# jac99/Egonn

Hardware: AMD Instinct MI355X
Metric: LiDAR scans/sec (descriptor extraction), 50k-pt clouds @ 0.1m voxel (higher is better)
Workload: dtype f32

## Files before the change

### egonn_amd/_lib.py

```python
from __future__ import annotations

import ctypes as C
import os
from typing import List, Optional, Sequence

import numpy as np
import torch

_HERE = os.path.dirname(os.path.abspath(__file__))
LIB_PATH = os.path.join(_HERE, "lib", "libegonn_hip.so")

QUANT_CARTESIAN, QUANT_POLAR = 0, 1
FLAG_DISABLE_GLOBAL, FLAG_DISABLE_LOCAL, FLAG_IGNORE_KP_REGRESSOR, FLAG_BF16 = 1, 2, 4, 8
FLAG_POOL_SPOC, FLAG_POOL_MAC = 16, 32
MINKFPN_SPLIT_TOPDOWN = 1
MINKFPN_BLOCKS = {'BasicBlock': 0, 'ECABasicBlock': 1}
MINKFPN_POOLING = {None: 0, 'GeM': 1, 'MAC': 2, 'SPoC': 3}

_P = C.c_void_p
_SIGS = [
    ("egonn_ctx_create", C.c_int, [C.POINTER(_P), C.c_int, C.c_int]),
    ("egonn_ctx_destroy", None, [_P]),
    ("egonn_last_error", C.c_char_p, []),
    ("egonn_debug_set_naive_conv", C.c_int, [_P, C.c_int]),
    ("egonn_debug_set_ksplit", C.c_int, [_P, C.c_int, C.c_int, C.c_int, C.c_int, C.c_int]),
    ("egonn_debug_set_resident", C.c_int, [_P, C.c_int, C.c_int]),
    ("egonn_debug_keep_level_features", C.c_int, [_P, C.c_int]),
    ("egonn_debug_set_trace", C.c_int, [_P]),
    ("egonn_prepare_maps", C.c_int, [_P, C.c_int, _P]),
    ("egonn_debug_rowgroup_tables", C.c_int, [_P, C.c_int, C.c_int, _P, _P, C.c_int64, C.POINTER(C.c_int64), _P]),
    ("egonn_debug_rowgroup_perm", C.c_int, [_P, C.c_int, C.c_int, _P, C.c_int64, C.POINTER(C.c_int64), _P]),
    ("egonn_debug_radix_sort_scratch_bytes", C.c_int64, [C.c_int64, C.c_int]),
    ("egonn_debug_radix_sort", C.c_int, [_P, _P, _P, _P, C.c_int64, C.c_int, _P, _P, C.c_int, C.c_int, C.c_int,
                                         C.POINTER(C.c_int32), _P, C.c_int64, _P]),
    ("egonn_voxelize", C.c_int, [_P, _P, C.POINTER(C.c_int64), C.c_int, C.c_int, C.POINTER(C.c_float), _P]),
    ("egonn_ctx_reserve", C.c_int, [_P, C.c_int64, C.c_int, C.POINTER(C.c_int64)]),
    ("egonn_voxelize_device", C.c_int, [_P, _P, C.c_int64, _P, C.c_int, C.c_int, C.POINTER(C.c_float), _P]),
    ("egonn_plan_status", C.c_int, [_P, _P]),
    ("egonn_ctx_set_exact_fp32", C.c_int, [_P, C.c_int]),
    ("egonn_ctx_set_operand_autoscale", C.c_int, [_P, C.c_int]),
    ("egonn_level_capacity", C.c_int, [_P, C.c_int, C.POINTER(C.c_int64)]),
    ("egonn_graph_begin", C.c_int, [_P]),
    ("egonn_graph_end", C.c_int, [_P, C.POINTER(_P)]),
    ("egonn_graph_launch", C.c_int, [_P, _P]),
    ("egonn_graph_destroy", None, [_P]),
    ("egonn_coords_set", C.c_int, [_P, _P, C.c_int64, C.c_int, _P]),
    ("egonn_level_count", C.c_int, [_P, C.c_int, C.POINTER(C.c_int64)]),
    ("egonn_level_batch_offsets", C.c_int, [_P, C.c_int, C.POINTER(C.c_int64)]),
    ("egonn_level_coords", C.c_int, [_P, C.c_int, _P, _P]),
    ("egonn_input_index", C.c_int, [_P, _P, _P]),
    ("egonn_conv", C.c_int, [_P, C.c_int, C.c_int, C.c_int, _P, C.c_int, _P, C.c_int, _P, _P, C.c_int, _P, _P]),
    ("egonn_conv_transpose", C.c_int, [_P, C.c_int, _P, C.c_int, _P, C.c_int, _P, _P]),
    ("egonn_sparse_conv", C.c_int, [_P, C.c_int, C.c_int, _P, C.c_int, _P, C.c_int, C.c_int, _P, _P, C.c_int, _P, _P, _P]),
    ("egonn_map_groups", C.c_int, [_P, C.c_int, C.c_int, C.POINTER(C.c_int64), C.POINTER(C.c_int64), _P]),
    ("egonn_global_avg_pool", C.c_int, [_P, C.c_int, _P, C.c_int, _P, _P]),
    ("egonn_bn_fold", C.c_int, [_P, _P, _P, _P, C.c_float, C.c_int, _P, _P, _P]),
    ("egonn_block_tail", C.c_int, [_P, C.c_int, _P, _P, C.c_int, _P, C.c_int, _P, _P]),
    ("egonn_gem", C.c_int, [_P, C.c_int, _P, C.c_int, _P, _P, _P]),
    ("egonn_global_max_pool", C.c_int, [_P, C.c_int, _P, C.c_int, _P, _P]),
    ("egonn_netvlad", C.c_int, [_P, C.c_int, _P, C.c_int, _P, _P, _P, _P, _P, _P, _P, _P, _P, _P, C.c_int, C.c_int, _P, _P]),
    ("egonn_netvlad_train_forward", C.c_int, [_P, C.c_int, _P, C.c_int, C.c_int, _P, _P, _P, _P, C.c_float, C.c_float, _P, _P,
                                              _P, C.c_int, _P, _P, _P, _P, _P, _P, _P]),
    ("egonn_netvlad_train_backward", C.c_int, [_P, C.c_int, _P, C.c_int, C.c_int, _P, _P, _P, _P, C.c_int, _P, _P, _P, _P, _P,
                                               _P, _P, _P, _P, _P, _P, _P]),
    ("egonn_global_max_pool_argmax", C.c_int, [_P, C.c_int, _P, C.c_int, _P, _P, _P]),
    ("egonn_global_max_pool_backward", C.c_int, [_P, C.c_int, _P, _P, C.c_int, _P, _P]),
    ("egonn_sigmoid_gate", C.c_int, [_P, _P, _P, C.c_int64, _P, _P, _P, _P]),
    ("egonn_add", C.c_int, [_P, _P, C.c_int64, _P, _P]),
    ("egonn_gather_input", C.c_int, [_P, _P, C.c_int, _P, _P]),
    ("egonn_model_create", C.c_int, [C.POINTER(_P)]),
    ("egonn_model_destroy", None, [_P]),
    ("egonn_model_set_tensor", C.c_int, [_P, C.c_char_p, _P, C.c_int, C.POINTER(C.c_int64)]),
    ("egonn_model_finalize", C.c_int, [_P, _P]),
    ("egonn_forward", C.c_int, [_P, _P, _P, C.c_int, C.POINTER(C.c_float), C.c_int, _P, _P, _P, _P, _P]),
    ("egonn_forward_level_features", C.c_int, [_P, C.c_int, _P, C.c_int, _P]),
    ("egonn_minkfpn_finalize", C.c_int, [_P, C.c_int, C.POINTER(C.c_int), C.POINTER(C.c_int), C.c_int, C.c_int, C.c_int, C.c_int, _P]),
    ("egonn_minkfpn_out_level", C.c_int, [C.c_int, C.c_int, C.POINTER(C.c_int)]),
    ("egonn_minkfpn_forward", C.c_int, [_P, _P, C.c_int, _P, _P, _P]),
    ("egonn_topdown_step", C.c_int, [_P, C.c_int, _P, _P, _P, _P, C.c_int, C.c_int, _P, _P]),
    ("egonn_select_keypoints", C.c_int, [_P, _P, _P, _P, C.c_int, _P, _P, _P, _P, _P]),
    ("egonn_topk_rows", C.c_int, [_P, _P, C.c_int, C.c_int, _P, _P, _P]),
    ("egonn_triplet_loss_scratch_floats", C.c_int64, [C.c_int]),
    ("egonn_triplet_loss", C.c_int, [_P, C.c_int, C.c_int, _P, _P, C.c_float, _P, _P, _P, _P, _P]),
    ("egonn_nn_search", C.c_int, [_P, C.c_int64, _P, _P, C.c_int64, _P, _P, _P]),
    ("egonn_matrix_min", C.c_int, [_P, C.c_int64, C.c_int64, _P, _P, _P, _P, _P]),
    ("egonn_softmax_cross_entropy", C.c_int, [_P, C.c_int64, C.c_int64, _P, _P, _P, _P, _P]),
    ("egonn_local_loss_scratch_bytes", C.c_int64, [C.c_int, C.c_int64, C.c_int64, C.c_int]),
    ("egonn_local_loss", C.c_int, [C.c_int, C.c_int64, C.c_int64, C.c_int64, C.c_int64, C.c_int] + [_P] * 13 +
                                  [C.POINTER(C.c_float)] + [_P] * 9 + [C.c_int64, _P]),
    ("egonn_dense", C.c_int, [_P, C.c_int64, C.c_int, _P, C.c_int, _P, C.c_int, C.c_int, _P, _P]),
    ("egonn_dense_pack_fragments", C.c_int, [_P, C.c_int, C.c_int, C.c_int, _P, _P]),
    ("egonn_dense_pack_fragments_host", C.c_int, [_P, C.c_int, C.c_int, C.c_int, _P]),
    ("egonn_debug_dense", C.c_int, [_P, C.c_int, C.c_int64, _P, C.c_int, C.c_int, _P, C.c_int, _P, _P, _P, _P, C.c_int, _P, C.c_int,
                                    _P, _P, C.c_int, _P, C.c_int, C.c_int, _P]),
    ("egonn_debug_dense_route", C.c_int, [C.c_int64, C.c_int, C.c_int, C.c_int, C.c_int, C.POINTER(C.c_int32)]),
    ("egonn_dense_backward_weight", C.c_int, [_P, C.c_int, _P, C.c_int, C.c_int64, _P, _P, C.c_int64, _P]),
    ("egonn_conv_backward_weight", C.c_int, [_P, C.c_int, C.c_int, C.c_int, C.c_int, _P, C.c_int, _P, C.c_int, _P, _P,
                                             C.c_int64, _P]),
    ("egonn_col_stats", C.c_int, [C.c_int, _P, _P, _P, _P, C.c_int64, C.c_int, _P, _P, C.c_int64, _P]),
    ("egonn_bn_train_finalize", C.c_int, [_P, _P, C.c_double, C.c_int, _P, _P, C.c_float, C.c_float, _P, _P, _P, _P]),
    ("egonn_bn_backward_finalize", C.c_int, [_P, _P, C.c_double, C.c_int, _P, _P, _P, _P, _P]),
    ("egonn_affine_act", C.c_int, [_P, _P, _P, C.c_int64, C.c_int, C.c_int, _P, _P]),
    ("egonn_affine3", C.c_int, [_P, _P, _P, _P, _P, _P, C.c_int64, C.c_int, _P, _P]),
    ("egonn_relu_backward", C.c_int, [_P, _P, C.c_int64, C.c_int, _P, _P]),
    ("egonn_contrastive_loss_scratch_floats", C.c_int64, [C.c_int]),
    ("egonn_contrastive_loss", C.c_int, [_P, C.c_int, C.c_int, _P, _P, C.c_float, C.c_float, _P, _P, _P, _P, _P]),
    ("egonn_se_gate", C.c_int, [_P, _P, _P, _P, _P, C.c_int, C.c_int, C.c_int, _P, _P, _P]),
    ("egonn_se_gate_backward", C.c_int, [_P, _P, _P, _P, _P, _P, C.c_int, C.c_int, C.c_int, _P, _P, _P, _P, _P, _P]),
    ("egonn_eca_gate", C.c_int, [_P, _P, C.c_int, C.c_int, C.c_int, _P, _P]),
    ("egonn_eca_gate_backward", C.c_int, [_P, _P, _P, _P, C.c_int, C.c_int, C.c_int, _P, _P, _P]),
    ("egonn_act_backward", C.c_int, [C.c_int, _P, _P, C.c_int64, C.c_int, _P, _P]),
    ("egonn_l2_normalize", C.c_int, [_P, _P, C.c_int64, C.c_int, _P, _P]),
    ("egonn_gate_residual", C.c_int, [_P, C.c_int, _P, _P, _P, C.c_int, C.c_int, _P, _P]),
    ("egonn_gate_residual_backward", C.c_int, [_P, C.c_int, _P, _P, _P, C.c_int, _P, _P, _P]),
    ("egonn_segment_sums", C.c_int, [_P, C.c_int, C.c_int, _P, _P, _P, _P, C.c_int, _P, _P, C.c_int64, _P]),
    ("egonn_segment_broadcast", C.c_int, [_P, C.c_int, _P, C.c_int, C.c_int, _P, _P]),
    ("egonn_gem_backward", C.c_int, [_P, C.c_int, _P, _P, _P, C.c_int, _P, _P]),
    ("egonn_filter_points_scratch_ints", C.c_int64, [C.c_int64]),
    ("egonn_filter_points", C.c_int, [_P, C.c_int64, C.c_int, _P, C.c_int, C.c_int, C.c_int, C.c_float, _P, _P, _P,
                                      C.c_int64, _P]),
    ("egonn_knn", C.c_int, [_P, C.c_int64, _P, C.c_int64, C.c_int, C.c_int, _P, _P, _P, C.c_int64, _P]),
    ("egonn_recall_counts", C.c_int, [_P, _P, _P, C.c_int64, C.c_int, C.c_int, _P, C.c_int, _P, _P]),
    ("egonn_registration_scratch_bytes", C.c_int64, [C.c_int, C.c_int, C.c_int]),
    ("egonn_match_mutual_scratch_bytes", C.c_int64, [C.c_int, C.c_int]),
    ("egonn_match_mutual", C.c_int, [_P, _P, _P, _P, C.c_int, C.c_int, C.c_int, _P, _P, _P, C.c_int64, _P]),
    ("egonn_ransac_pairs", C.c_int, [_P, _P, _P, _P, _P, _P, _P, C.c_int, C.c_int, C.c_int, C.c_uint64, C.c_double, _P,
                                     C.c_int64, _P, _P, _P]),
    ("egonn_registration_finish", C.c_int, [_P, _P, _P, _P, _P, _P, _P, C.c_int, C.c_int, C.c_int, C.c_uint64, C.c_double, _P,
                                            C.c_int64, _P, C.c_double, _P, _P, _P, _P, _P, _P, _P, _P, _P, _P, _P, _P]),
    ("egonn_voxel_downsample_scratch_bytes", C.c_int64, [C.c_int64, C.c_int]),
    ("egonn_voxel_downsample", C.c_int, [_P, C.c_int64, _P, C.c_int, C.c_double, C.POINTER(C.c_float), _P, _P, _P, _P, _P,
                                         C.c_int64, _P]),
    ("egonn_icp_scratch_bytes", C.c_int64, [C.c_int64, C.c_int64, C.c_int]),
    ("egonn_icp_pairs", C.c_int, [_P, C.c_int64, _P, _P, C.c_int64, _P, C.c_int, _P, C.c_double, C.c_int, C.c_double, C.c_double,
                                  _P, _P, _P, _P, _P, _P, _P, _P, _P, C.c_int64, _P]),
    ("egonn_estimate_normals_scratch_bytes", C.c_int64, [C.c_int64, C.c_int]),
    ("egonn_estimate_normals", C.c_int, [_P, C.c_int64, _P, C.c_int, C.c_int, _P, _P, _P, _P, _P, C.c_int64, _P]),
    ("egonn_icp_plane_scratch_bytes", C.c_int64, [C.c_int64, C.c_int64, C.c_int]),
    ("egonn_icp_plane_pairs", C.c_int, [_P, C.c_int64, _P, _P, C.c_int64, _P, _P, C.c_int, _P, C.c_double, C.c_int, C.c_double,
                                        C.c_double, _P, _P, _P, _P, _P, _P, _P, _P, _P, C.c_int64, _P]),
    ("egonn_augment_scratch_bytes", C.c_int64, [C.c_int64, C.c_int]),
    ("egonn_augment_points", C.c_int, [_P, C.c_int64, _P, C.c_int, _P, _P, _P, _P, _P, _P, _P, _P, _P, C.c_int64, _P]),
    ("egonn_scan_context", C.c_int, [_P, C.c_int64, _P, C.c_int, C.c_int, C.c_int, C.c_double, C.c_double, _P, _P, _P]),
    ("egonn_scan_context_ringkey", C.c_int, [_P, C.c_int64, C.c_int, C.c_int, _P, _P]),
    ("egonn_scan_context_distance", C.c_int, [_P, C.c_int64, _P, C.c_int64, C.c_int, C.c_int, _P, C.c_int, _P, _P, _P]),
    ("egonn_scan_context_rerank", C.c_int, [_P, _P, _P, C.c_int64, C.c_int, _P, _P, _P, _P]),
    ("egonn_radius_count", C.c_int, [_P, C.c_int64, _P, C.c_int64, C.POINTER(C.c_double), C.c_int, C.c_int, _P, _P]),
    ("egonn_radius_fill", C.c_int, [_P, C.c_int64, _P, C.c_int64, C.c_double, C.c_int, _P, _P, C.c_int64, _P, _P]),
    ("egonn_pair_masks", C.c_int, [_P, C.c_int, _P, _P, C.c_int64, _P, _P, C.c_int64, C.c_int64, _P, _P, _P, _P]),
    ("egonn_relative_poses", C.c_int, [_P, C.c_int64, _P, _P, C.c_int64, C.c_int, _P, _P, _P]),
    ("egonn_gather_clouds", C.c_int, [_P, C.c_int64, _P, C.c_int64, _P, C.c_int, _P, C.c_int64, _P, _P, _P]),
    ("egonn_match_candidates_scratch_bytes", C.c_int64, [C.c_int, C.c_int, C.c_int]),
    ("egonn_match_candidates", C.c_int, [_P, _P, _P, _P, _P, C.c_int, C.c_int, C.c_int, C.c_int, C.c_int, _P, _P, _P, _P,
                                         C.c_int64, _P]),
    ("egonn_gather_candidates", C.c_int, [_P, _P, _P, _P, _P, _P, C.c_int, C.c_int, C.c_int, C.c_int, _P, _P, _P, _P, _P, _P]),
    ("egonn_pick_candidates", C.c_int, [_P, C.c_int, C.c_int, C.c_int, _P, _P, _P, _P, _P, _P, _P, _P, C.c_int] + [_P] * 12),
    ("egonn_profile_enable", C.c_int, [_P, C.c_int, C.c_char_p]),
    ("egonn_profile_fetch", C.c_int, [_P, C.c_int, C.POINTER(C.c_int), C.c_char_p, C.POINTER(C.c_float),
                                      C.POINTER(C.c_double), C.POINTER(C.c_double), _P]),
]
EXPORTED_SYMBOLS = [s[0] for s in _SIGS]

_lib = None


def load() -> C.CDLL:
    global _lib
    if _lib is not None:
        return _lib
    if not os.path.exists(LIB_PATH):
        raise RuntimeError(
            f"egonn_amd: HIP library not found at {LIB_PATH}. Build it with "
            f"`python -c 'import __graft_entry__ as g; g.build()'` (hipcc --offload-arch=gfx950). "
            f"There is no CPU fallback.")
    lib = C.CDLL(LIB_PATH)
    for name, res, args in _SIGS:
        fn = getattr(lib, name)
        fn.restype = res
        fn.argtypes = args
    _lib = lib
    return lib


def _err(lib) -> str:
    msg = lib.egonn_last_error()
    return msg.decode() if msg else "unknown error"


class EgonnError(RuntimeError):

    def __init__(self, msg: str, code: int):
        super().__init__(msg)
        self.code = int(code)


class CapacityError(EgonnError):
    """status 5: the batch did not fit the capacities of egonn_ctx_reserve (the exact-size eager path still works)"""


class Fp16RangeError(EgonnError):
    """status 6: a kernel on the fp16-split pipe (fp32 sparse convolution or local heads) met an operand fp16 cannot hold
    (|x| >= 65520) or a non-finite input: the batch's outputs are invalid; Context.set_exact_fp32(True) and run it again
    (on the same plan: every forward clears this flag)"""


def check(rc: int):
    if rc != 0:
        cls = CapacityError if rc == 5 else (Fp16RangeError if rc == 6 else EgonnError)
        raise cls(f"libegonn_hip: {_err(load())} (code {rc})", rc)


def _stream() -> int:
    return torch.cuda.current_stream().cuda_stream


def _ptr(t: Optional[torch.Tensor]) -> Optional[int]:
    return None if t is None else t.data_ptr()


def call(device: torch.device, fn, *args):
    idx = device.index
    if idx is None or torch.cuda.current_device() == idx:
        rc = fn(*args, _stream())
    else:
        with torch.cuda.device(device):
            rc = fn(*args, _stream())
    if rc != 0:
        check(rc)


def _dev_f32(t: torch.Tensor, device) -> torch.Tensor:
    return t.to(device=device, dtype=torch.float32).contiguous()

# ... 425 lines not shown
            self._call(self.lib.egonn_sigmoid_gate, y.data_ptr(), t.data_ptr(), None, y.numel(), out.data_ptr(), None, None)
            return out
        g = _dev_f32(grad_out, self.device)
        dy, dt = torch.empty_like(y), torch.empty_like(y)
        self._call(self.lib.egonn_sigmoid_gate, y.data_ptr(), t.data_ptr(), g.data_ptr(), y.numel(), None, dy.data_ptr(),
                   dt.data_ptr())
        return dy, dt

    def dense_backward_weight(self, a, b):
        a, b = _dev_f32(a, self.device), _dev_f32(b, self.device)
        assert a.shape[0] == b.shape[0]
        ca, cb = a.shape[1], b.shape[1]
        out = torch.empty((ca, cb), dtype=torch.float32, device=self.device)
        sc = self.scratch(64 * ca * cb)
        self._call(self.lib.egonn_dense_backward_weight, a.data_ptr(), ca, b.data_ptr(), cb, a.shape[0], out.data_ptr(),
                   sc.data_ptr(), sc.numel())
        return out

    def conv_backward_weight(self, level_in, level_out, kernel_size, transposed, x, grad_out, kernel_shape):
        g = _dev_f32(grad_out, self.device)
        xx = None if x is None else _dev_f32(x, self.device)
        cin, cout = kernel_shape[-2], kernel_shape[-1]
        out = torch.empty(tuple(kernel_shape), dtype=torch.float32, device=self.device)
        sc = self.scratch(16 * out.numel())
        self._call(self.lib.egonn_conv_backward_weight, self.h, level_in, level_out, kernel_size, int(transposed), _ptr(xx),
                   cin, g.data_ptr(), cout, out.data_ptr(), sc.data_ptr(), sc.numel())
        return out

    def col_stats(self, mode: int, a, b=None, mask=None, mean=None):
        a = _dev_f32(a, self.device)
        n, c = a.shape
        out = torch.empty((2, c), dtype=torch.float64, device=self.device)
        sc = self.scratch(4 * c * max(1024, n // 512 + 2))
        self._call(self.lib.egonn_col_stats, mode, a.data_ptr(), _ptr(b), _ptr(mask), _ptr(mean), n, c, out.data_ptr(),
                   sc.data_ptr(), sc.numel())
        return out

    def affine_act(self, x, scale, shift, relu: bool):
        x = _dev_f32(x, self.device)
        out = torch.empty_like(x)
        self._call(self.lib.egonn_affine_act, x.data_ptr(), scale.data_ptr(), shift.data_ptr(), x.shape[0], x.shape[1],
                   int(relu), out.data_ptr())
        return out

    def affine3(self, g, mask, x, A, B, Cc):
        g, x = _dev_f32(g, self.device), _dev_f32(x, self.device)
        out = torch.empty_like(x)
        self._call(self.lib.egonn_affine3, g.data_ptr(), _ptr(mask), x.data_ptr(), A.data_ptr(), B.data_ptr(),
                   Cc.data_ptr(), x.shape[0], x.shape[1], out.data_ptr())
        return out

    def relu_backward(self, grad_out, out):
        g = _dev_f32(grad_out, self.device)
        dx = torch.empty_like(g)
        self._call(self.lib.egonn_relu_backward, g.data_ptr(), out.data_ptr(), g.shape[0], g.shape[1], dx.data_ptr())
        return dx

    def act_backward(self, act: int, grad_out, out):
        g = _dev_f32(grad_out, self.device)
        dx = torch.empty_like(g)
        self._call(self.lib.egonn_act_backward, act, g.data_ptr(), out.data_ptr(), g.shape[0], g.shape[1], dx.data_ptr())
        return dx

    def l2_normalize(self, x, grad_out=None):
        x = _dev_f32(x, self.device)
        g = None if grad_out is None else _dev_f32(grad_out, self.device)
        out = torch.empty_like(x)
        self._call(self.lib.egonn_l2_normalize, x.data_ptr(), _ptr(g), x.shape[0], x.shape[1], out.data_ptr())
        return out

    def gate_residual(self, level, x, gate, residual, relu: bool = True):
        x = _dev_f32(x, self.device)
        assert x.shape[0] == self.level_count(level)
        out = torch.empty_like(x)
        self._call(self.lib.egonn_gate_residual, self.h, level, x.data_ptr(), _ptr(gate), _ptr(residual), x.shape[1],
                   int(relu), out.data_ptr())
        return out

    def gate_residual_backward(self, level, grad_out, out, gate, want_residual: bool = True):
        g = _dev_f32(grad_out, self.device)
        dx = torch.empty_like(g)
        dres = torch.empty_like(g) if want_residual else None
        self._call(self.lib.egonn_gate_residual_backward, self.h, level, g.data_ptr(), _ptr(out), _ptr(gate), g.shape[1],
                   dx.data_ptr(), _ptr(dres))
        return dx, dres

    def segment_sums(self, level, mode, a, b=None, x2=None, p=None):
        a = _dev_f32(a, self.device)
        c = a.shape[1]
        out = torch.empty((self.batch_size, c), dtype=torch.float32, device=self.device)
        sc = self.scratch(32 * self.batch_size * c)
        self._call(self.lib.egonn_segment_sums, self.h, level, mode, a.data_ptr(), _ptr(b), _ptr(x2), _ptr(p), c,
                   out.data_ptr(), sc.data_ptr(), sc.numel())
        return out

    def segment_broadcast(self, level, v, mean: bool):
        v = _dev_f32(v, self.device)
        out = torch.empty((self.level_count(level), v.shape[1]), dtype=torch.float32, device=self.device)
        self._call(self.lib.egonn_segment_broadcast, self.h, level, v.data_ptr(), v.shape[1], int(mean), out.data_ptr())
        return out

    def gem_backward(self, level, x, coef, p):
        x, coef = _dev_f32(x, self.device), _dev_f32(coef, self.device)
        dx = torch.empty_like(x)
        self._call(self.lib.egonn_gem_backward, self.h, level, x.data_ptr(), coef.data_ptr(), p.data_ptr(), x.shape[1],
                   dx.data_ptr())
        return dx

    def eca_gate(self, mean, w):
        B, c = mean.shape
        gate = torch.empty_like(mean)
        self._call(self.lib.egonn_eca_gate, mean.data_ptr(), w.data_ptr(), w.numel(), B, c, gate.data_ptr())
        return gate

    def eca_gate_backward(self, grad_out, gate, mean, w):
        B, c = mean.shape
        dmean = torch.empty_like(mean)
        dw = torch.empty(w.numel(), dtype=torch.float32, device=mean.device)
        self._call(self.lib.egonn_eca_gate_backward, grad_out.data_ptr(), gate.data_ptr(), mean.data_ptr(), w.data_ptr(),
                   w.numel(), B, c, dmean.data_ptr(), dw.data_ptr())
        return dmean, dw

    def se_gate_backward(self, grad_out, gate, hid, mean, w1, w2):
        B, c = mean.shape
        h = w1.shape[0]
        dmean, dw1, dw2 = torch.empty_like(mean), torch.empty_like(w1), torch.empty_like(w2)
        db1 = torch.empty(h, dtype=torch.float32, device=mean.device)
        db2 = torch.empty(c, dtype=torch.float32, device=mean.device)
        self._call(self.lib.egonn_se_gate_backward, grad_out.data_ptr(), gate.data_ptr(), hid.data_ptr(), mean.data_ptr(),
                   w1.data_ptr(), w2.data_ptr(), B, c, h, dmean.data_ptr(), dw1.data_ptr(), db1.data_ptr(), dw2.data_ptr(),
                   db2.data_ptr())
        return dmean, dw1, db1, dw2, db2

    def bn_train_finalize(self, sums, shift, total: float, weight, bias, eps: float, momentum: float, running_mean=None,
                          running_var=None):
        c = weight.numel()
        out4 = torch.empty((4, c), dtype=torch.float32, device=sums.device)
        self._call(self.lib.egonn_bn_train_finalize, sums.data_ptr(), shift.data_ptr(), total, c, weight.data_ptr(),
                   bias.data_ptr(), float(eps), float(momentum), _ptr(running_mean), _ptr(running_var), out4.data_ptr())
        return out4

    def bn_backward_finalize(self, sums, sums_all, total: float, weight, mean, invstd):
        c = weight.numel()
        out5 = torch.empty((5, c), dtype=torch.float32, device=sums.device)
        self._call(self.lib.egonn_bn_backward_finalize, sums.data_ptr(), sums_all.data_ptr(), total, c, weight.data_ptr(),
                   mean.data_ptr(), invstd.data_ptr(), out5.data_ptr())
        return out5

    def forward_level_features(self, level: int, channels: int) -> torch.Tensor:
        out = torch.empty((self.level_count(level), channels), dtype=torch.float32, device=self.device)
        self._call(self.lib.egonn_forward_level_features, self.h, level, out.data_ptr(), channels)
        return out

    def select_keypoints(self, sigma: torch.Tensor, keypoints: torch.Tensor, descriptors: torch.Tensor, n_k: int):
        B = self.batch_size
        dev = self.device
        sel_kp = torch.empty((B, n_k, 3), dtype=torch.float32, device=dev)
        sel_desc = torch.empty((B, n_k, descriptors.shape[1]), dtype=torch.float32, device=dev)
        sel_rows = torch.empty((B, n_k), dtype=torch.int32, device=dev)
        sel_count = torch.empty((B,), dtype=torch.int32, device=dev)
        self._call(self.lib.egonn_select_keypoints, self.h, sigma.data_ptr(), keypoints.data_ptr(), descriptors.data_ptr(), n_k,
                   sel_kp.data_ptr(), sel_desc.data_ptr(), sel_rows.data_ptr(), sel_count.data_ptr())
        return sel_kp, sel_desc, sel_rows, sel_count

    def profile_enable(self, mode: int, filt: str = ""):
        check(self.lib.egonn_profile_enable(self.h, mode, filt.encode()))

    def profile_fetch(self, cap: int = 4096):
        n = C.c_int()
        names = C.create_string_buffer(cap * 64)
        ms = (C.c_float * cap)()
        by = (C.c_double * cap)()
        fl = (C.c_double * cap)()
        self._call(self.lib.egonn_profile_fetch, self.h, cap, C.byref(n), names, ms, by, fl)
        out = []
        for i in range(n.value):
            nm = names.raw[i * 64:(i + 1) * 64].split(b"\0", 1)[0].decode()
            out.append((nm, float(ms[i]), float(by[i]), float(fl[i])))
        return out


class ModelHandle:

    def __init__(self):
        self.lib = load()
        h = _P()
        check(self.lib.egonn_model_create(C.byref(h)))
        self.h = h
        self._keep = {}

    def __del__(self):
        try:
            if getattr(self, "h", None):
                self.lib.egonn_model_destroy(self.h)
                self.h = None
        except Exception:
            pass

    def set_tensor(self, key: str, t: torch.Tensor):
        assert t.is_cuda and t.dtype == torch.float32 and t.is_contiguous(), key
        shape = (C.c_int64 * max(t.dim(), 1))(*t.shape)
        check(self.lib.egonn_model_set_tensor(self.h, key.encode(), t.data_ptr(), t.dim(), shape))
        self._keep[key] = t

    def finalize(self):
        check(self.lib.egonn_model_finalize(self.h, _stream()))

    def finalize_minkfpn(self, planes: Sequence[int], layers: Sequence[int], num_top_down: int, feature_size: int, block: int,
                         pooling: int):
        n = len(planes)
        assert len(layers) == n
        check(self.lib.egonn_minkfpn_finalize(self.h, n, (C.c_int * max(n, 1))(*planes), (C.c_int * max(n, 1))(*layers),
                                              int(num_top_down), int(feature_size), int(block), int(pooling), _stream()))


def minkfpn_out_level(n_levels: int, num_top_down: int) -> int:
    lv = C.c_int()
    check(load().egonn_minkfpn_out_level(int(n_levels), int(num_top_down), C.byref(lv)))
    return lv.value
```

### egonn_amd/csrc/common.h

```cpp
#pragma once
#include <hip/hip_runtime.h>
#include <atomic>
#include <stdint.h>
#include <stdio.h>
#include <string.h>
#include <string>
#include <vector>

#define EGONN_MAX_LEVELS 10
#define EGONN_NUM_LEVELS 8
#define EGONN_MAX_BATCH 4096

#define API extern "C" __attribute__((visibility("default")))

namespace egonn {

void set_error(const char* fmt, ...);
#define EGONN_OK 0
#define EGONN_ERR_INVALID 1
#define EGONN_ERR_HIP 2
#define EGONN_ERR_RANGE 3
#define EGONN_ERR_STATE 4
#define EGONN_ERR_CAPACITY 5
#define EGONN_ERR_FP16_RANGE 6
// ... 27 lines not shown
__host__ __device__ static inline int64_t clipi(int64_t v, int64_t hi) { return v < 0 ? 0 : (v > hi ? hi : v); }

struct AttrOnce {
  std::atomic<uint64_t> done{0};
  static int dev() { int d = 0; (void)hipGetDevice(&d); return d & 63; }
  bool need() const { return !((done.load(std::memory_order_acquire) >> dev()) & 1ull); }
  void mark() { done.fetch_or(1ull << dev(), std::memory_order_release); }
};
static inline size_t align_up(size_t v, size_t a) { return (v + a - 1) / a * a; }

struct Arena {
  char* base = nullptr;
  size_t cap = 0;
  size_t off = 0;
  bool borrowed = false;
  static Arena view(void* span, size_t bytes) {
    Arena a;
    a.base = static_cast<char*>(span);
    a.cap = bytes;
    a.borrowed = true;
    return a;
  }
  int ensure(size_t bytes) {
    if (bytes <= cap) return EGONN_OK;
    EGONN_REQUIRE(!borrowed, EGONN_ERR_INVALID, "scratch span of %zu bytes is %zu bytes short of the %zu needed", cap, bytes - cap,
                  bytes);
    size_t want = align_up(bytes + bytes / 4, size_t(1) << 20);
    if (base) {
      HIP_CHECK(hipDeviceSynchronize());
      HIP_CHECK(hipFree(base));
      base = nullptr;
      cap = 0;
    }
    HIP_CHECK(hipMalloc(reinterpret_cast<void**>(&base), want));
    cap = want;
    off = 0;
    return EGONN_OK;
  }
  void reset() { off = 0; }
  template <typename T>
  T* alloc(size_t n) {
    size_t o = align_up(off, 256);
    size_t end = o + n * sizeof(T);
    if (end > cap) return nullptr;
    off = end;
    return reinterpret_cast<T*>(base + o);
  }
  void release() {
    if (borrowed) return;
    if (base) (void)hipFree(base);
    base = nullptr;
    cap = off = 0;
  }
};

__host__ __device__ static inline uint64_t part1by2(uint32_t v) {
  uint64_t x = v & 0xFFFFull;
  x = (x | (x << 16)) & 0x0000FF0000FFull;
  x = (x | (x << 8)) & 0x00F00F00F00Full;
  x = (x | (x << 4)) & 0x0C30C30C30C3ull;
  x = (x | (x << 2)) & 0x249249249249ull;
  return x;
}
__host__ __device__ static inline uint32_t compact1by2(uint64_t x) {
  x &= 0x249249249249ull;
  x = (x | (x >> 2)) & 0x0C30C30C30C3ull;
  x = (x | (x >> 4)) & 0x00F00F00F00Full;
  x = (x | (x >> 8)) & 0x0000FF0000FFull;
  x = (x | (x >> 16)) & 0xFFFFull;
  return (uint32_t)x;
}
__host__ __device__ static inline uint64_t morton3(uint32_t x, uint32_t y, uint32_t z) {
  return part1by2(x) | (part1by2(y) << 1) | (part1by2(z) << 2);
}

static constexpr int RG_MAX_JOBS = 24;
static constexpr int RG_MAX_WIN = 512;
struct RowGroups {
  int K = 0;
  int win = 0;
  int cap_groups = 0;
  int32_t* perm = nullptr;
  int32_t* snbr = nullptr;
  uint32_t* gmask = nullptr;
  int32_t* meta = nullptr;
  int32_t* order4 = nullptr;
  bool built = false;
};
struct RGBuild {
  RowGroups* rg;
  const int32_t* nbr;
  const int32_t* n_dev;
  const int32_t* boff;
  int32_t cap_rows = 0;
};
int rowgroup_build(const RGBuild* jobs, int njobs, int B, hipStream_t stream);

struct Level {
  int64_t n = 0;
  uint64_t* keys = nullptr;
  int32_t* parent = nullptr;
  int32_t* cstart = nullptr;
  uint64_t* mask = nullptr;
  int32_t* bstart = nullptr;
  int32_t* boff = nullptr;
  int32_t* nbr27 = nullptr;
  int32_t* nbr8 = nullptr;
  int32_t* nbrT = nullptr;
  RowGroups rg27, rg8, rgT;
};

struct Plan {
  bool valid = false;
  bool built_reserved = false;
  bool exact = false;
  int64_t cap_points = 0;
  int64_t* scan_off = nullptr;
  int batch = 0;
  int coord_bits = 16;
  int64_t n_input = 0;
  Level lv[EGONN_MAX_LEVELS];
  int64_t cap[EGONN_MAX_LEVELS] = {};
  int32_t* perm0 = nullptr;
  int32_t* g0 = nullptr;
  uint64_t* t2m = nullptr;
  int32_t* t2s = nullptr;
  std::vector<int32_t> boff_host[EGONN_NUM_LEVELS];
};

enum ProfKind { PK_CONV0 = 0, PK_K3 = 1, PK_K2S2 = 2, PK_TCONV = 3, PK_OTHER = 4 };
struct ProfRec {
  char name[64];
  int kind, level, K, cin, cout;
  int es;
  hipEvent_t e0, e1;
};
struct Profiler {
  int mode = 0;
  char filter[64] = "";
  std::vector<ProfRec> recs;
  std::vector<ProfRec> graph_recs;
  std::vector<hipEvent_t> pool;
  hipEvent_t get();
};

struct Switches {
  bool debug_sync;
  bool no_presplit;
  bool no_fused_down;
  bool no_fused_lateral;
  bool no_gated_k2s2;
  bool no_fused_ghead;
  bool no_split_heads;
  bool no_tail_split;
  bool no_task_order;
  bool flat_sort, sort_pairs;
  bool no_search67;
  bool no_dense_stream;
  int split_max_level;
  int split_max_level_k8;
  int split_cfg;
  int rg_first_pass;
  const char* ksplit[5];
};
const Switches& switches();

struct KsRule {
  int8_t kparts[2][EGONN_NUM_LEVELS];
  int8_t kw[2][EGONN_NUM_LEVELS];
  int8_t col_parts[EGONN_NUM_LEVELS];
};

static constexpr int SCONV_RESIDENT_DEFAULT = 6;

struct Ctx {
  Profiler prof;
  KsRule ks_rule;
  uint16_t* conv0_lut = nullptr;
  unsigned long long* dev_pairs = nullptr;
  int device = 0;
  int coord_bits = 16;
  int split_max_level = 5;
  float* ks_part = nullptr;
  size_t ks_part_floats = 0;
  const void* sort_prezeroed = nullptr;
  int resident_mask = SCONV_RESIDENT_DEFAULT;
  int resident_wgs = 0;
  int keep_level_features = 0;
  int operand_autoscale = 0;
  int conv_variant = 0;
  Arena plan_arena;
  Arena work_arena;
  Arena sort_arena;
  Plan plan;
  int32_t* host_counts = nullptr;
  int32_t* dev_counts = nullptr;
  int32_t* dev_flags = nullptr;
  int32_t* dev_fp16_flag = nullptr;
  bool reserved = false;
  int64_t reserve_points = 0;
  int reserve_batch = 0;
  int64_t reserve_cap[EGONN_MAX_LEVELS] = {};
  hipEvent_t ev0 = nullptr, ev1 = nullptr;
};

hipEvent_t* prof_kernel_events();
struct ProfScope {
  Ctx* ctx;
  hipStream_t st;
  int idx = -1;
  bool exact = false;
  bool in_graph = false;
  ProfScope(Ctx* c, hipStream_t s, const char* name, int kind, int level, int K, int cin, int cout, int es);
  ~ProfScope();
};

int ensure_level0_parent_table(Ctx* ctx, hipStream_t stream);
int ensure_rowgroups(Ctx* ctx, const int* kinds, const int* levels, int count, hipStream_t stream);
int rowgroup_cap_groups(const Plan& P, int level);

static constexpr int KP_MAX_N = 256;
static constexpr int KP_MAX_D = 256;
static constexpr int KP_MAX_PAIRS = 1 << 20;
static constexpr int REL_MAX_K = 1024;
int reg_check_shape(const char* who, int P, int n_max);
int rel_check_shape(const char* who, int Q, int k, int M, int n_max);

int radix_sort_pairs(Arena& ws, uint64_t* keys_in, uint32_t* vals_in, uint64_t* keys_out, uint32_t* vals_out,
                     int64_t n, int nbits, hipStream_t stream, const int64_t* n_dev = nullptr, uint64_t** keys_res = nullptr,
                     uint32_t** vals_res = nullptr);
size_t radix_sort_scratch_bytes(int64_t n);
int radix_sort_segments(Arena& ws, uint64_t* keys_in, uint32_t* vals_in, uint64_t* keys_out, uint32_t* vals_out, int64_t n,
                        const int64_t* off_dev, int B, int nbits, hipStream_t stream, uint64_t** keys_res, uint32_t** vals_res,
                        int idx_bits = 0, const void* prezeroed = nullptr);
size_t radix_sort_segments_scratch_bytes(int64_t n, int B);
int radix_sort_segments_layout(Arena& ws, int64_t n, int B, int32_t** tilehist, int32_t** scanhist);
int radix_sort_segments_passes(int nbits);
int radix_sort_segments_digits();

int plan_from_points(Ctx* ctx, const float* points, const int64_t* scan_offsets, int64_t n_cap, int offsets_on_device,
                     int B, int mode, const float* step, hipStream_t stream);
int plan_reserve(Ctx* ctx, int64_t max_points, int B, const int64_t* level_caps);
int plan_sync(Ctx* ctx, hipStream_t stream);
int plan_from_coords(Ctx* ctx, const int32_t* coords, int64_t n, int B, hipStream_t stream);
int plan_level_coords(Ctx* ctx, int level, int32_t* out, hipStream_t stream);
int count_map_pairs(Ctx* ctx, hipStream_t stream);

}
```

### egonn_amd/csrc/coords.hip

```cpp
#include "common.h"

#include <algorithm>
#include <stdarg.h>

namespace egonn {

static thread_local char g_err[1024] = "";
void set_error(const char* fmt, ...) {
  va_list ap;
  va_start(ap, fmt);
  vsnprintf(g_err, sizeof(g_err), fmt, ap);
  va_end(ap);
}
const char* last_error() { return g_err; }

const Switches& switches() {
  static const Switches sw = [] {
    auto on = [](const char* name) { return getenv(name) != nullptr; };
    auto num = [](const char* name, int unset) { const char* e = getenv(name); return e ? atoi(e) : unset; };
    const char* ds = getenv("EGONN_DEBUG_SYNC");
    return Switches{.debug_sync = ds && ds[0] == '1', .no_presplit = on("EGONN_NO_PRESPLIT"), .no_fused_down = on("EGONN_NO_FUSED_DOWN"),
                    .no_fused_lateral = on("EGONN_NO_FUSED_LATERAL"), .no_gated_k2s2 = on("EGONN_NO_GATED_K2S2"),
                    .no_fused_ghead = on("EGONN_NO_FUSED_GHEAD"), .no_split_heads = on("EGONN_NO_SPLIT_HEADS"),
                    .no_tail_split = on("EGONN_NO_TAIL_SPLIT"), .no_task_order = on("EGONN_NO_TASK_ORDER"),
                    .flat_sort = on("EGONN_FLAT_SORT"), .sort_pairs = on("EGONN_SORT_PAIRS"), .no_search67 = on("EGONN_NO_SEARCH67"),
                    .no_dense_stream = on("EGONN_NO_DENSE_STREAM"),
                    .split_max_level = num("EGONN_SPLIT_MAX_LEVEL", -1), .split_max_level_k8 = num("EGONN_SPLIT_MAX_LEVEL_K8", -1),
                    .split_cfg = num("EGONN_SPLIT_CFG", 0), .rg_first_pass = num("EGONN_RG_FIRST_PASS", 0),
                    .ksplit = {getenv("EGONN_KSPLIT"), getenv("EGONN_KSPLIT8"), getenv("EGONN_KSPLIT_KW"), getenv("EGONN_KSPLIT_KW8"),
                               getenv("EGONN_KSPLIT_PARTS")}};
  }();
  return sw;
}

hipEvent_t Profiler::get() {
  if (!pool.empty()) {
    hipEvent_t e = pool.back();
    pool.pop_back();
    return e;
  }
  hipEvent_t e = nullptr;
  (void)hipEventCreate(&e);
  return e;
}
ProfScope::ProfScope(Ctx* c, hipStream_t s, const char* name, int kind, int level, int K, int cin, int cout, int es)
    : ctx(c), st(s) {
  if (!c || c->prof.mode == 0) return;
  if (c->prof.mode >= 2 && !strstr(name, c->prof.filter)) return;
  hipStreamCaptureStatus cs = hipStreamCaptureStatusNone;
  (void)hipStreamIsCapturing(s, &cs);
  in_graph = cs == hipStreamCaptureStatusActive;
  if (in_graph && c->prof.mode != 3) return;
  ProfRec r;
  snprintf(r.name, sizeof(r.name), "%s", name);
  r.kind = kind; r.level = level; r.K = K; r.cin = cin; r.cout = cout; r.es = es;
  r.e0 = c->prof.get();
  r.e1 = c->prof.get();
  exact = c->prof.mode == 2 && (kind == PK_K3 || kind == PK_K2S2 || kind == PK_TCONV);
  if (exact) {
    prof_kernel_events()[0] = r.e0;
    prof_kernel_events()[1] = r.e1;
  } else {
    (void)hipEventRecord(r.e0, s);
  }
  std::vector<ProfRec>& dst = in_graph ? c->prof.graph_recs : c->prof.recs;
  idx = (int)dst.size();
  dst.push_back(r);
}
ProfScope::~ProfScope() {
  if (idx < 0) return;
  if (exact) {
    prof_kernel_events()[0] = prof_kernel_events()[1] = nullptr;
  } else {
    (void)hipEventRecord((in_graph ? ctx->prof.graph_recs : ctx->prof.recs)[idx].e1, st);
  }
}
hipEvent_t* prof_kernel_events() {
  static thread_local hipEvent_t ev[2] = {nullptr, nullptr};
  return ev;
}

struct QuantParams {
  int mode;
  float s0, s1, s2;
};

__device__ static inline void quantize_point(const QuantParams& qp, float x, float y, float z, int32_t& cx,
                                             int32_t& cy, int32_t& cz) {
  if (qp.mode == 0) {
    cx = (int32_t)floorf(qp.s0 == 1.0f ? x : __fdiv_rn(x, qp.s0));
    cy = (int32_t)floorf(qp.s0 == 1.0f ? y : __fdiv_rn(y, qp.s0));
    cz = (int32_t)floorf(qp.s0 == 1.0f ? z : __fdiv_rn(z, qp.s0));
  } else {
    const float at = (float)atan2((double)y, (double)x);
    const float theta = __fadd_rn(180.0f, __fdiv_rn(__fmul_rn(at, 180.0f), 3.14159265358979323846f));
    const float dist = sqrtf(__fadd_rn(__fmul_rn(x, x), __fmul_rn(y, y)));
    cx = (int32_t)floorf(__fdiv_rn(theta, qp.s0));
    cy = (int32_t)floorf(__fdiv_rn(dist, qp.s1));
    cz = (int32_t)floorf(__fdiv_rn(z, qp.s2));
  }
}

__device__ static inline bool encode_key(int32_t b, int32_t cx, int32_t cy, int32_t cz, int cb, uint64_t& key) {
  const int32_t bias = 1 << (cb - 1);
  const int32_t lim = 1 << cb;
  const int32_t ux = cx + bias, uy = cy + bias, uz = cz + bias;
  const bool ok = (ux >= 0) & (ux < lim) & (uy >= 0) & (uy < lim) & (uz >= 0) & (uz < lim) & (b >= 0);
  key = ((uint64_t)(uint32_t)b << (3 * cb)) | morton3((uint32_t)ux, (uint32_t)uy, (uint32_t)uz);
  return ok;
}

__global__ void points_to_keys_kernel(const float* __restrict__ pts, int64_t n_cap, const int64_t* __restrict__ scan_off,
                                      int B, QuantParams qp, int cb, uint64_t* __restrict__ keys,
                                      uint32_t* __restrict__ vals, int32_t* __restrict__ flags, int idx_bits,
                                      int64_t* __restrict__ off_copy, int32_t* __restrict__ zero_ptr, int zero_words) {
  const int64_t i = (int64_t)blockIdx.x * blockDim.x + threadIdx.x;
  const int64_t stride = (int64_t)gridDim.x * blockDim.x;
  if (off_copy)
    for (int64_t b = i; b <= B; b += stride) off_copy[b] = scan_off[b];
  for (int64_t w = i; w < zero_words; w += stride) zero_ptr[w] = 0;
  const int64_t nn = scan_off[B];
  if (i == 0 && nn > n_cap) atomicOr(flags, 2);
  for (int64_t b = i; b <= B; b += stride)
    if ((b == 0 && scan_off[0] != 0) || (b > 0 && scan_off[b] < scan_off[b - 1])) atomicOr(flags, 1);
  if (i >= (nn < n_cap ? nn : n_cap)) return;
  int lo = 0, hi = B;
  while (hi - lo > 1) {
    const int mid = (lo + hi) >> 1;
    if (scan_off[mid] <= i) lo = mid; else hi = mid;
  }
  const float x = pts[3 * i + 0], y = pts[3 * i + 1], z = pts[3 * i + 2];
  int32_t cx, cy, cz;
  quantize_point(qp, x, y, z, cx, cy, cz);
  uint64_t key;
  const bool finite = isfinite(x) & isfinite(y) & isfinite(z);
  if (!encode_key(lo, cx, cy, cz, cb, key) || !finite) {
    atomicOr(flags, 1);
    const int32_t hi = (1 << (cb - 1)) - 1, lo_c = -(1 << (cb - 1));
    const int32_t qx = finite ? min(max(cx, lo_c), hi) : 0, qy = finite ? min(max(cy, lo_c), hi) : 0,
                  qz = finite ? min(max(cz, lo_c), hi) : 0;
    encode_key(lo, qx, qy, qz, cb, key);
  }
  if (idx_bits > 0) {
    keys[i] = ((key & ((1ull << (3 * cb)) - 1)) << idx_bits) | (uint64_t)(i - scan_off[lo]);
  } else {
    keys[i] = key;
    vals[i] = (uint32_t)i;
  }
}

__global__ void coords_to_keys_kernel(const int32_t* __restrict__ c4, int64_t n, int cb, int Bmax,
                                      uint64_t* __restrict__ keys, uint32_t* __restrict__ vals,
                                      int32_t* __restrict__ flags) {
  const int64_t i = (int64_t)blockIdx.x * blockDim.x + threadIdx.x;
  if (i >= n) return;
  const int4 c = reinterpret_cast<const int4*>(c4)[i];
  uint64_t key;
  if (!encode_key(c.x, c.y, c.z, c.w, cb, key) || c.x >= Bmax) {
    atomicOr(flags, 1);
    key = ~0ull >> 1;
  }
  keys[i] = key;
  vals[i] = (uint32_t)i;
}

static constexpr int PYR_BLOCK = 256;
static constexpr int PYR_ROUNDS = 4;
static constexpr int PYR_TILE = PYR_BLOCK * PYR_ROUNDS;
static constexpr int NL = EGONN_MAX_LEVELS;

__device__ static inline int head_levels(const uint64_t* __restrict__ keys, int64_t i) {
  if (i == 0) return NL;
  const uint64_t d = keys[i] ^ keys[i - 1];
  if (d == 0) return 0;
  const int t = (63 - __clzll(d)) / 3;
  return (t >= NL - 1) ? NL : t + 1;
// ... 902 lines not shown
```

### egonn_amd/csrc/heads.hip

```cpp
#include <algorithm>

#include "common.h"
#include "kernels.h"
#include "rowmath.h"

namespace egonn {

__device__ static inline void keypoint_position(uint64_t key, int level, int cb, float ox, float oy, float oz, int mode,
                                                float s0, float s1, float s2, float* __restrict__ out3) {
  const int cbL = cb - level;
  const uint64_t mort = key & ((1ull << (3 * cbL)) - 1);
  const int32_t bias = 1 << (cb - 1);
  const float cx = (float)(((int32_t)compact1by2(mort) << level) - bias);
  const float cy = (float)(((int32_t)compact1by2(mort >> 1) << level) - bias);
  const float cz = (float)(((int32_t)compact1by2(mort >> 2) << level) - bias);
  const float stride = (float)(1 << level);
  const float px = __fadd_rn(__fmul_rn(__fadd_rn(cx, 0.5f), s0), __fdiv_rn(__fmul_rn(ox, __fmul_rn(stride, s0)), 2.f));
  const float py = __fadd_rn(__fmul_rn(__fadd_rn(cy, 0.5f), s1), __fdiv_rn(__fmul_rn(oy, __fmul_rn(stride, s1)), 2.f));
  const float pz = __fadd_rn(__fmul_rn(__fadd_rn(cz, 0.5f), s2), __fdiv_rn(__fmul_rn(oz, __fmul_rn(stride, s2)), 2.f));
  if (mode == 0) {
    out3[0] = px; out3[1] = py; out3[2] = pz;
  } else {
    const float theta = __fdiv_rn(__fmul_rn(3.14159265358979323846f, __fadd_rn(px, -180.f)), 180.f);
    out3[0] = cosf(theta) * py;
    out3[1] = sinf(theta) * py;
    out3[2] = pz;
  }
}

__global__ void keypoint_kernel(const uint64_t* __restrict__ keys, int64_t n, int level, int cb,
                                const float* __restrict__ offs, int mode, float s0, float s1, float s2, int ignore,
                                float* __restrict__ out, const int32_t* __restrict__ n_dev) {
  const int64_t i = (int64_t)blockIdx.x * blockDim.x + threadIdx.x;
  if (n_dev) n = min((int64_t)*n_dev, n);
  if (i >= n) return;
  const float kox = ignore ? 0.f : offs[3 * i + 0], koy = ignore ? 0.f : offs[3 * i + 1],
              koz = ignore ? 0.f : offs[3 * i + 2];
  keypoint_position(keys[i], level, cb, kox, koy, koz, mode, s0, s1, s2, out + 3 * i);
}
int keypoint_positions(const uint64_t* keys, int64_t n, int level, int cb, const float* offsets, int mode,
                       const float* step, int ignore_offsets, float* out, hipStream_t stream, const int32_t* n_dev) {
  if (n == 0) return EGONN_OK;
  const float s0 = step[0], s1 = mode ? step[1] : step[0], s2 = mode ? step[2] : step[0];
  hipLaunchKernelGGL(keypoint_kernel, dim3((unsigned)cdiv(n, 256)), dim3(256), 0, stream, keys, n, level, cb, offsets,
                     mode, s0, s1, s2, ignore_offsets, out, n_dev);
  HIP_CHECK(hipGetLastError());
  return EGONN_OK;
}

struct LocalHeadsArgs {
  const float* x;
  const float *lw, *lres;
  const float *dw0, *db0, *dw1, *db1;
  const float *kw0, *kb0, *kw1, *kb1;
  const float *sw0, *sb0, *sw1, *sb1;
  const uint64_t* keys;
  const int32_t* n_dev;
  float *out_desc, *out_kp, *out_sigma;
  int64_t n;
  int level, cb, mode, ignore_offsets;
  int in_bf16;
  float s0, s1, s2;
};
template <int CIN, int NT>
__device__ static inline void stage_frags(const float* __restrict__ W, int rows_w, f32x4* __restrict__ dst, int tid, int nthreads) {
  constexpr int T = CIN / 16;
  for (int i = tid; i < NT * T * 64; i += nthreads) {
    const int lane = i & 63, ft = i >> 6;
    const int nt = ft / T, t = ft - nt * T;
    const int unit = 16 * nt + (lane & 15);
    f32x4 v = {0.f, 0.f, 0.f, 0.f};
    if (unit < rows_w) v = *reinterpret_cast<const f32x4*>(W + (int64_t)unit * CIN + 16 * t + 4 * (lane >> 4));
    dst[i] = v;
  }
}
template <int CIN, int NT>
__device__ static inline void mlp_layer(const f32x4* __restrict__ frags, const f32x4* __restrict__ in, int lane,
                                        f32x4* __restrict__ out) {
  constexpr int T = CIN / 16;
#pragma unroll
  for (int nt = 0; nt < NT; ++nt) {
    f32x4 acc = {0.f, 0.f, 0.f, 0.f};
#pragma unroll
    for (int t = 0; t < T; ++t) {
      const f32x4 wf = frags[(nt * T + t) * 64 + lane];
#pragma unroll
      for (int u = 0; u < 4; ++u) acc = __builtin_amdgcn_mfma_f32_16x16x4f32(wf[u], in[t][u], acc, 0, 0, 0);
    }
    out[nt] = acc;
    __builtin_amdgcn_sched_barrier(0);
  }
}
template <int CIN, int NT>
__device__ static inline void stage_frags_t(const float* __restrict__ W, int cout, f32x4* __restrict__ dst, int tid, int nthreads) {
  constexpr int T = CIN / 16;
  for (int i = tid; i < NT * T * 64; i += nthreads) {
    const int lane = i & 63, ft = i >> 6;
    const int nt = ft / T, t = ft - nt * T;
    const float* wp = W + (int64_t)(16 * t + 4 * (lane >> 4)) * cout + 16 * nt + (lane & 15);
    dst[i] = (f32x4){wp[0], wp[cout], wp[2 * (int64_t)cout], wp[3 * (int64_t)cout]};
  }
}
constexpr int LH_F_DW0 = 0, LH_F_DW1 = LH_F_DW0 + 6 * 4, LH_F_KW0 = LH_F_DW1 + 8 * 6, LH_F_KW1 = LH_F_KW0 + 2 * 4,
              LH_F_SW0 = LH_F_KW1 + 1 * 2, LH_F_SW1 = LH_F_SW0 + 2 * 4, LH_FRAGS = LH_F_SW1 + 1 * 2;
__global__ __launch_bounds__(LH_WAVES * 64) void local_heads_kernel(const LocalHeadsArgs p) {
  extern __shared__ __attribute__((aligned(16))) f32x4 lh_frags[];
  const int tid = threadIdx.x, lane = tid & 63, wave = tid >> 6;
  const int l15 = lane & 15, g4 = lane >> 4;
  stage_frags<64, 6>(p.dw0, 96, lh_frags + LH_F_DW0 * 64, tid, LH_WAVES * 64);
  stage_frags<96, 8>(p.dw1, 128, lh_frags + LH_F_DW1 * 64, tid, LH_WAVES * 64);
  stage_frags<64, 2>(p.kw0, 32, lh_frags + LH_F_KW0 * 64, tid, LH_WAVES * 64);
  stage_frags<32, 1>(p.kw1, 3, lh_frags + LH_F_KW1 * 64, tid, LH_WAVES * 64);
  stage_frags<64, 2>(p.sw0, 32, lh_frags + LH_F_SW0 * 64, tid, LH_WAVES * 64);
  stage_frags<32, 1>(p.sw1, 1, lh_frags + LH_F_SW1 * 64, tid, LH_WAVES * 64);
  if (p.lw) stage_frags_t<64, 4>(p.lw, 64, lh_frags + LH_FRAGS * 64, tid, LH_WAVES * 64);
  __syncthreads();
  int64_t n = p.n;
  if (p.n_dev) n = min((int64_t)*p.n_dev, n);
  const int64_t ntiles = (n + 15) >> 4;
  for (int64_t tile = (int64_t)blockIdx.x * LH_WAVES + wave; tile < ntiles; tile += (int64_t)gridDim.x * LH_WAVES) {
    const int64_t row = tile * 16 + l15;
    const bool ok = row < n;
    f32x4 x[4];
    auto load4 = [&](const float* base, int t) -> f32x4 {
      if (!ok) return (f32x4){0.f, 0.f, 0.f, 0.f};
      if (p.in_bf16) {
        const uint2 h = *reinterpret_cast<const uint2*>(reinterpret_cast<const uint16_t*>(base) + row * 64 + 16 * t + 4 * g4);
        return (f32x4){bf2f(h.x & 0xFFFFu), bf2f(h.x >> 16), bf2f(h.y & 0xFFFFu), bf2f(h.y >> 16)};
      }
      return *reinterpret_cast<const f32x4*>(base + row * 64 + 16 * t + 4 * g4);
    };
#pragma unroll
    for (int t = 0; t < 4; ++t) x[t] = load4(p.x, t);
    if (p.lw) {
      f32x4 r[4], l[4];
#pragma unroll
      for (int t = 0; t < 4; ++t) r[t] = load4(p.lres, t);
      mlp_layer<64, 4>(lh_frags + LH_FRAGS * 64, x, lane, l);
#pragma unroll
      for (int t = 0; t < 4; ++t) x[t] = l[t] + r[t];
    }
    {
      f32x4 h[6], o[8];
      mlp_layer<64, 6>(lh_frags + LH_F_DW0 * 64, x, lane, h);
#pragma unroll
      for (int nt = 0; nt < 6; ++nt) {
        const f32x4 b = *reinterpret_cast<const f32x4*>(p.db0 + 16 * nt + 4 * g4);
#pragma unroll
        for (int r = 0; r < 4; ++r) h[nt][r] = fmaxf(h[nt][r] + b[r], 0.f);
      }
      mlp_layer<96, 8>(lh_frags + LH_F_DW1 * 64, h, lane, o);
      float ss = 0.f;
#pragma unroll
      for (int nt = 0; nt < 8; ++nt) {
        const f32x4 b = *reinterpret_cast<const f32x4*>(p.db1 + 16 * nt + 4 * g4);
#pragma unroll
        for (int r = 0; r < 4; ++r) {
          o[nt][r] += b[r];
          ss += o[nt][r] * o[nt][r];
        }
      }
      ss += __shfl_xor(ss, 16, 64);
      ss += __shfl_xor(ss, 32, 64);
      const float inv = 1.f / fmaxf(sqrtf(ss), 1e-12f);
      if (ok) {
#pragma unroll
        for (int nt = 0; nt < 8; ++nt)
          *reinterpret_cast<f32x4*>(p.out_desc + row * 128 + 16 * nt + 4 * g4) = o[nt] * inv;
      }
    }
    {
      f32x4 h[2], o[1];
      mlp_layer<64, 2>(lh_frags + LH_F_KW0 * 64, x, lane, h);
#pragma unroll
      for (int nt = 0; nt < 2; ++nt) {
        const f32x4 b = *reinterpret_cast<const f32x4*>(p.kb0 + 16 * nt + 4 * g4);
#pragma unroll
        for (int r = 0; r < 4; ++r) h[nt][r] = fmaxf(h[nt][r] + b[r], 0.f);
      }
      mlp_layer<32, 1>(lh_frags + LH_F_KW1 * 64, h, lane, o);
      if (ok && g4 == 0) {
        const float ox = p.ignore_offsets ? 0.f : tanhf(o[0][0] + p.kb1[0]);
        const float oy = p.ignore_offsets ? 0.f : tanhf(o[0][1] + p.kb1[1]);
        const float oz = p.ignore_offsets ? 0.f : tanhf(o[0][2] + p.kb1[2]);
        keypoint_position(p.keys[row], p.level, p.cb, ox, oy, oz, p.mode, p.s0, p.s1, p.s2, p.out_kp + row * 3);
      }
    }
    {
      f32x4 h[2], o[1];
      mlp_layer<64, 2>(lh_frags + LH_F_SW0 * 64, x, lane, h);
#pragma unroll
      for (int nt = 0; nt < 2; ++nt) {
        const f32x4 b = *reinterpret_cast<const f32x4*>(p.sb0 + 16 * nt + 4 * g4);
#pragma unroll
        for (int r = 0; r < 4; ++r) h[nt][r] = fmaxf(h[nt][r] + b[r], 0.f);
      }
      mlp_layer<32, 1>(lh_frags + LH_F_SW1 * 64, h, lane, o);
      if (ok && g4 == 0) p.out_sigma[row] = apply_act(o[0][0] + p.sb1[0], ACT_SOFTPLUS);
    }
  }
}
typedef _Float16 lh_f16x8 __attribute__((ext_vector_type(8)));
typedef _Float16 lh_f16x2 __attribute__((ext_vector_type(2)));
typedef float lh_f32x2 __attribute__((ext_vector_type(2)));
__host__ __device__ static inline int lh_chan(int g, int e) { return e < 4 ? 4 * g + e : 16 + 4 * g + (e - 4); }
constexpr int LHS_DW0 = 0, LHS_DW1 = LHS_DW0 + 6 * 2, LHS_KW0 = LHS_DW1 + 8 * 3, LHS_KW1 = LHS_KW0 + 2 * 2, LHS_SW0 = LHS_KW1 + 1 * 1,
              LHS_SW1 = LHS_SW0 + 2 * 2, LHS_FRAGS = LHS_SW1 + 1 * 1;
struct LhsMat { int cin, nout, nt, first; };
__constant__ LhsMat lhs_mats[6] = {{64, 96, 6, LHS_DW0}, {96, 128, 8, LHS_DW1}, {64, 32, 2, LHS_KW0}, {32, 3, 1, LHS_KW1},
                                   {64, 32, 2, LHS_SW0}, {32, 1, 1, LHS_SW1}};
__global__ void lhs_absmax_kernel(const float* const* __restrict__ W, uint32_t* __restrict__ trailer) {
  const int mi = blockIdx.x;
  const LhsMat M = lhs_mats[mi];
  const float* w = W[mi];
  float m = 0.f;
  for (int i = threadIdx.x; i < M.cin * M.nout; i += blockDim.x) {
    const float v = fabsf(w[i]);
    m = (v == v && v < INFINITY) ? fmaxf(m, v) : m;
  }
#pragma unroll
  for (int o = 32; o > 0; o >>= 1) m = fmaxf(m, __shfl_xor(m, o, 64));
  if ((threadIdx.x & 63) == 0) atomicMax(trailer + 8 + mi, __float_as_uint(m));
}
__device__ static inline float lhs_scale_of(uint32_t maxbits) {
  const int e = (int)(maxbits >> 23) - 127;
  const int se = min(max(13 - e, -100), 100);
  return __uint_as_float((uint32_t)(se + 127) << 23);
}
__global__ void lhs_pack_kernel(const float* const* __restrict__ W, uint16_t* __restrict__ out, uint32_t* __restrict__ trailer) {
  const int mi = blockIdx.y;
  const LhsMat M = lhs_mats[mi];
  const int KB = M.cin / 32;
  const int t = blockIdx.x * blockDim.x + threadIdx.x;
  const float sc = lhs_scale_of(trailer[8 + mi]);
  if (t == 0) reinterpret_cast<float*>(trailer)[mi] = 1.f / sc;
  if (t >= M.nt * KB * 2 * 64 * 8) return;
  int r = t;
  const int e = r & 7; r >>= 3;
  const int lane = r & 63; r >>= 6;
  const int part = r & 1; r >>= 1;
  const int kb = r % KB, nt = r / KB;
  const int unit = 16 * nt + (lane & 15), k = 32 * kb + lh_chan(lane >> 4, e);
  const float v = unit < M.nout ? sc * W[mi][(int64_t)unit * M.cin + k] : 0.f;
  const _Float16 hi = (_Float16)v;
  const _Float16 lo = (_Float16)(v - (float)hi);
  out[(int64_t)M.first * 2 * 512 + t] = __builtin_bit_cast(uint16_t, part == 0 ? hi : lo);
}
size_t local_heads_pack_bytes() { return (size_t)LHS_FRAGS * 2048 + 64; }
int local_heads_pack(const float* const* w6_dev , void* out, hipStream_t stream) {
  uint32_t* trailer = reinterpret_cast<uint32_t*>(reinterpret_cast<char*>(out) + (size_t)LHS_FRAGS * 2048);
  HIP_CHECK(hipMemsetAsync(trailer, 0, 64, stream));
  hipLaunchKernelGGL(lhs_absmax_kernel, dim3(6), dim3(256), 0, stream, w6_dev, trailer);
  hipLaunchKernelGGL(lhs_pack_kernel, dim3((8 * 3 * 2 * 64 * 8 + 255) / 256, 6), dim3(256), 0, stream, w6_dev,
                     reinterpret_cast<uint16_t*>(out), trailer);
  HIP_CHECK(hipGetLastError());
  return EGONN_OK;
}
__device__ static inline void lhs_split8(const f32x4& a0, const f32x4& a1, lh_f16x8& hi, lh_f16x8& lo) {
#pragma unroll
  for (int q = 0; q < 4; ++q) {
    const float x0 = q < 2 ? a0[2 * q] : a1[2 * q - 4], x1 = q < 2 ? a0[2 * q + 1] : a1[2 * q - 3];
    const lh_f16x2 h = __builtin_convertvector((lh_f32x2){x0, x1}, lh_f16x2);
    const lh_f32x2 hf = __builtin_convertvector(h, lh_f32x2);
    const lh_f16x2 l = __builtin_convertvector((lh_f32x2){x0 - hf[0], x1 - hf[1]}, lh_f16x2);
    hi[2 * q] = h[0]; hi[2 * q + 1] = h[1];
    lo[2 * q] = l[0]; lo[2 * q + 1] = l[1];
  }
}
template <int CIN, int NT>
__device__ static inline void lhs_layer(const f32x4* __restrict__ frags , const f32x4* __restrict__ in, int lane,
                                        float winv, f32x4* __restrict__ out) {
  constexpr int KB = CIN / 32;
  lh_f16x8 ah[KB], al[KB];
#pragma unroll
  for (int kb = 0; kb < KB; ++kb) lhs_split8(in[2 * kb], in[2 * kb + 1], ah[kb], al[kb]);
#pragma unroll
  for (int nt = 0; nt < NT; ++nt) {
    f32x4 acc = {0.f, 0.f, 0.f, 0.f};
#pragma unroll
    for (int kb = 0; kb < KB; ++kb) {
      const lh_f16x8 wh = __builtin_bit_cast(lh_f16x8, frags[((nt * KB + kb) * 2) * 64 + lane]);
      const lh_f16x8 wl = __builtin_bit_cast(lh_f16x8, frags[((nt * KB + kb) * 2 + 1) * 64 + lane]);
      acc = __builtin_amdgcn_mfma_f32_16x16x32_f16(wl, ah[kb], acc, 0, 0, 0);
      acc = __builtin_amdgcn_mfma_f32_16x16x32_f16(wh, al[kb], acc, 0, 0, 0);
      acc = __builtin_amdgcn_mfma_f32_16x16x32_f16(wh, ah[kb], acc, 0, 0, 0);
    }
    out[nt] = acc * winv;
    __builtin_amdgcn_sched_barrier(0);
  }
}
struct LocalHeadsSplitArgs {
  LocalHeadsArgs a;
  const void* pack;
  int32_t* flags;
};
__global__ __launch_bounds__(LH_WAVES * 64) void local_heads_split_kernel(const LocalHeadsSplitArgs q) {
  const LocalHeadsArgs& p = q.a;
  extern __shared__ __attribute__((aligned(16))) f32x4 lh_frags[];
  const int tid = threadIdx.x, lane = tid & 63, wave = tid >> 6;
  const int l15 = lane & 15, g4 = lane >> 4;
  {
    const f32x4* src = reinterpret_cast<const f32x4*>(q.pack);
    for (int i = tid; i < LHS_FRAGS * 2 * 64; i += LH_WAVES * 64) lh_frags[i] = src[i];
  }
  f32x4* const lat = lh_frags + LHS_FRAGS * 2 * 64;
  if (p.lw) stage_frags_t<64, 4>(p.lw, 64, lat, tid, LH_WAVES * 64);
  const float* winv = reinterpret_cast<const float*>(reinterpret_cast<const char*>(q.pack) + (size_t)LHS_FRAGS * 2048);
  const float wi0 = winv[0], wi1 = winv[1], wi2 = winv[2], wi3 = winv[3], wi4 = winv[4], wi5 = winv[5];
  __syncthreads();
  int64_t n = p.n;
  if (p.n_dev) n = min((int64_t)*p.n_dev, n);
  const int64_t ntiles = (n + 15) >> 4;
  for (int64_t tile = (int64_t)blockIdx.x * LH_WAVES + wave; tile < ntiles; tile += (int64_t)gridDim.x * LH_WAVES) {
    const int64_t row = tile * 16 + l15;
    const bool ok = row < n;
    f32x4 x[4];
    auto load4 = [&](const float* base, int t) -> f32x4 {
      if (!ok) return (f32x4){0.f, 0.f, 0.f, 0.f};
      if (p.in_bf16) {
        const uint2 h = *reinterpret_cast<const uint2*>(reinterpret_cast<const uint16_t*>(base) + row * 64 + 16 * t + 4 * g4);
        return (f32x4){bf2f(h.x & 0xFFFFu), bf2f(h.x >> 16), bf2f(h.y & 0xFFFFu), bf2f(h.y >> 16)};
      }
      return *reinterpret_cast<const f32x4*>(base + row * 64 + 16 * t + 4 * g4);
    };
#pragma unroll
    for (int t = 0; t < 4; ++t) x[t] = load4(p.x, t);
    if (p.lw) {
      f32x4 r[4], l[4];
#pragma unroll
      for (int t = 0; t < 4; ++t) r[t] = load4(p.lres, t);
      mlp_layer<64, 4>(lat, x, lane, l);
#pragma unroll
      for (int t = 0; t < 4; ++t) x[t] = l[t] + r[t];
    }
    float guard = 0.f;
    bool outside = false;
#pragma unroll
    for (int t = 0; t < 4; ++t)
#pragma unroll
      for (int r = 0; r < 4; ++r) outside |= !(fabsf(x[t][r]) < 65520.f);
    {
      f32x4 h[6], o[8];
      lhs_layer<64, 6>(lh_frags + LHS_DW0 * 2 * 64, x, lane, wi0, h);
#pragma unroll
      for (int nt = 0; nt < 6; ++nt) {
        const f32x4 b = *reinterpret_cast<const f32x4*>(p.db0 + 16 * nt + 4 * g4);
#pragma unroll
        for (int r = 0; r < 4; ++r) h[nt][r] = fmaxf(h[nt][r] + b[r], 0.f);
      }
      lhs_layer<96, 8>(lh_frags + LHS_DW1 * 2 * 64, h, lane, wi1, o);
      float ss = 0.f;
#pragma unroll
      for (int nt = 0; nt < 8; ++nt) {
        const f32x4 b = *reinterpret_cast<const f32x4*>(p.db1 + 16 * nt + 4 * g4);
#pragma unroll
        for (int r = 0; r < 4; ++r) {
          o[nt][r] += b[r];
          ss += o[nt][r] * o[nt][r];
        }
      }
      ss += __shfl_xor(ss, 16, 64);
      ss += __shfl_xor(ss, 32, 64);
      guard += ss - ss;
      const float inv = 1.f / fmaxf(sqrtf(ss), 1e-12f);
      if (ok) {
#pragma unroll
        for (int nt = 0; nt < 8; ++nt)
          *reinterpret_cast<f32x4*>(p.out_desc + row * 128 + 16 * nt + 4 * g4) = o[nt] * inv;
      }
    }
    {
      f32x4 h[2], o[1];
      lhs_layer<64, 2>(lh_frags + LHS_KW0 * 2 * 64, x, lane, wi2, h);
#pragma unroll
      for (int nt = 0; nt < 2; ++nt) {
        const f32x4 b = *reinterpret_cast<const f32x4*>(p.kb0 + 16 * nt + 4 * g4);
#pragma unroll
        for (int r = 0; r < 4; ++r) h[nt][r] = fmaxf(h[nt][r] + b[r], 0.f);
      }
      lhs_layer<32, 1>(lh_frags + LHS_KW1 * 2 * 64, h, lane, wi3, o);
      if (ok && g4 == 0) {
        guard += (o[0][0] - o[0][0]) + (o[0][1] - o[0][1]) + (o[0][2] - o[0][2]);
        const float ox = p.ignore_offsets ? 0.f : tanhf(o[0][0] + p.kb1[0]);
        const float oy = p.ignore_offsets ? 0.f : tanhf(o[0][1] + p.kb1[1]);
        const float oz = p.ignore_offsets ? 0.f : tanhf(o[0][2] + p.kb1[2]);
        keypoint_position(p.keys[row], p.level, p.cb, ox, oy, oz, p.mode, p.s0, p.s1, p.s2, p.out_kp + row * 3);
      }
    }
    {
      f32x4 h[2], o[1];
      lhs_layer<64, 2>(lh_frags + LHS_SW0 * 2 * 64, x, lane, wi4, h);
#pragma unroll
      for (int nt = 0; nt < 2; ++nt) {
        const f32x4 b = *reinterpret_cast<const f32x4*>(p.sb0 + 16 * nt + 4 * g4);
#pragma unroll
        for (int r = 0; r < 4; ++r) h[nt][r] = fmaxf(h[nt][r] + b[r], 0.f);
      }
      lhs_layer<32, 1>(lh_frags + LHS_SW1 * 2 * 64, h, lane, wi5, o);
      if (ok && g4 == 0) {
        guard += o[0][0] - o[0][0];
        p.out_sigma[row] = apply_act(o[0][0] + p.sb1[0], ACT_SOFTPLUS);
      }
    }
    if (ok && (outside || guard != 0.f) && q.flags) atomicOr(q.flags, 8);
  }
}

int local_heads_forward(const float* x, int64_t n, const int32_t* n_dev, const float* const* w ,
                        const uint64_t* keys, int level, int cb, int mode, const float* step, int ignore_offsets,
                        float* out_desc, float* out_kp, float* out_sigma, hipStream_t stream, const float* lateral_w,
                        const float* lateral_res, int in_bf16, const void* split_pack, int32_t* flags) {
  if (n == 0) return EGONN_OK;
  EGONN_REQUIRE((lateral_w == nullptr) == (lateral_res == nullptr), EGONN_ERR_INVALID, "local heads: lateral kernel and residual go together");
  LocalHeadsArgs a;
  a.x = x; a.n = n; a.n_dev = n_dev;
  a.lw = lateral_w; a.lres = lateral_res;
  a.in_bf16 = in_bf16 ? 1 : 0;
  EGONN_REQUIRE(!in_bf16 || lateral_w, EGONN_ERR_INVALID, "local heads: bf16 input rows only through the fused lateral");
  a.dw0 = w[0]; a.db0 = w[1]; a.dw1 = w[2]; a.db1 = w[3];
  a.kw0 = w[4]; a.kb0 = w[5]; a.kw1 = w[6]; a.kb1 = w[7];
  a.sw0 = w[8]; a.sb0 = w[9]; a.sw1 = w[10]; a.sb1 = w[11];
  a.keys = keys; a.level = level; a.cb = cb; a.mode = mode; a.ignore_offsets = ignore_offsets;
  a.s0 = step[0]; a.s1 = mode ? step[1] : step[0]; a.s2 = mode ? step[2] : step[0];
  a.out_desc = out_desc; a.out_kp = out_kp; a.out_sigma = out_sigma;
  const int64_t tiles = cdiv(n, 16);
  const size_t lds = (size_t)(LH_FRAGS + (lateral_w ? 16 : 0)) * 64 * sizeof(f32x4);
  static AttrOnce attr_done;
  if (attr_done.need()) {
    HIP_CHECK(hipFuncSetAttribute(reinterpret_cast<const void*>(&local_heads_kernel), hipFuncAttributeMaxDynamicSharedMemorySize, 160 * 1024));
    attr_done.mark(); 
  }
  const unsigned grid = (unsigned)std::min<int64_t>(cdiv(tiles, LH_WAVES), 256);
  if (split_pack) {
    static AttrOnce attr2;
    if (attr2.need()) {
      HIP_CHECK(hipFuncSetAttribute(reinterpret_cast<const void*>(&local_heads_split_kernel), hipFuncAttributeMaxDynamicSharedMemorySize, 160 * 1024));
      attr2.mark();
    }
    LocalHeadsSplitArgs q;
    q.a = a; q.pack = split_pack; q.flags = flags;
    const size_t lds2 = (size_t)(LHS_FRAGS * 2 + (lateral_w ? 16 : 0)) * 64 * sizeof(f32x4);
    hipLaunchKernelGGL(local_heads_split_kernel, dim3(grid), dim3(LH_WAVES * 64), lds2, stream, q);
    HIP_CHECK(hipGetLastError());
    return EGONN_OK;
  }
  hipLaunchKernelGGL(local_heads_kernel, dim3(grid), dim3(LH_WAVES * 64), lds, stream, a);
  HIP_CHECK(hipGetLastError());
  return EGONN_OK;
}

__device__ static inline uint32_t sigma_bits(float v) {
  const uint32_t u = __float_as_uint(v);
  return (u & 0x80000000u) ? ~u : (u | 0x80000000u);
}
constexpr int TK_THREADS = 1024, TK_BINS = 2048, TK_CACHE = 8;
__global__ __launch_bounds__(TK_THREADS) void select_topk_kernel(const float* __restrict__ sigma, const int32_t* __restrict__ boff,
                                                                 int k, int S, const float* __restrict__ kp,
                                                                 const float* __restrict__ desc, int dc,
                                                                 int32_t* __restrict__ sel_rows, int32_t* __restrict__ sel_count,
                                                                 float* __restrict__ out_kp, float* __restrict__ out_desc) {
  extern __shared__ __attribute__((aligned(16))) unsigned long long skeys[];
  __shared__ uint32_t s_hist[TK_BINS];
  __shared__ uint32_t s_wave[TK_THREADS / 64];
  __shared__ uint32_t s_pick[3];
  __shared__ uint32_t s_n;
  const int b = blockIdx.x, tid = threadIdx.x, lane = tid & 63, wave = tid >> 6;
  const int32_t r0 = boff[b], nb = boff[b + 1] - r0;
  const int kk = min(k, nb);
  uint32_t sb[TK_CACHE];
#pragma unroll
  for (int i = 0; i < TK_CACHE; ++i) {
    const int r = i * TK_THREADS + tid;
    sb[i] = r < nb ? sigma_bits(sigma[r0 + r]) : 0xFFFFFFFFu;
  }
  auto key_of = [&](uint32_t bits, int r) { return ((unsigned long long)bits << 32) | (unsigned)r; };
  unsigned long long T = 0;
  if (kk > 0) {
    unsigned long long prefix = 0;
    uint32_t need = (uint32_t)kk;
    const int shifts[6] = {53, 42, 31, 20, 9, 0};
#pragma unroll 1
    for (int p = 0; p < 6; ++p) {
      const int sh = shifts[p], bits = p == 5 ? 9 : 11;
      const uint32_t dmask = (1u << bits) - 1;
      for (int i = tid; i < TK_BINS; i += TK_THREADS) s_hist[i] = 0;
      __syncthreads();
      auto count = [&](uint32_t sbits, int r) {
        const unsigned long long key = key_of(sbits, r);
        if (p == 0 || (key >> (sh + bits)) == prefix) atomicAdd(&s_hist[(uint32_t)(key >> sh) & dmask], 1u);
      };
#pragma unroll
      for (int i = 0; i < TK_CACHE; ++i) {
        const int r = i * TK_THREADS + tid;
        if (r < nb) count(sb[i], r);
      }
      for (int r = TK_CACHE * TK_THREADS + tid; r < nb; r += TK_THREADS) count(sigma_bits(sigma[r0 + r]), r);
      __syncthreads();
      const uint32_t h0 = s_hist[2 * tid], h1 = s_hist[2 * tid + 1];
      uint32_t inc = h0 + h1;
#pragma unroll
      for (int d = 1; d < 64; d <<= 1) {
        const uint32_t o = __shfl_up(inc, d, 64);
        if (lane >= d) inc += o;
      }
      if (lane == 63) s_wave[wave] = inc;
      __syncthreads();
      uint32_t ex = inc - (h0 + h1);
      for (int w = 0; w < wave; ++w) ex += s_wave[w];
      if (ex < need && need <= ex + h0) {
        s_pick[0] = 2 * tid; s_pick[1] = ex; s_pick[2] = h0;
      } else if (ex + h0 < need && need <= ex + h0 + h1) {
        s_pick[0] = 2 * tid + 1; s_pick[1] = ex + h0; s_pick[2] = h1;
      }
      __syncthreads();
      const uint32_t digit = s_pick[0], below = s_pick[1], inbin = s_pick[2];
      prefix = (prefix << bits) | digit;
      need -= below;
      if (inbin == need || sh == 0) {
        T = sh ? ((prefix << sh) | ((1ull << sh) - 1)) : prefix;
        break;
      }
    }
  }
  if (tid == 0) s_n = 0;
  for (int i = tid; i < S; i += TK_THREADS) skeys[i] = ~0ull;
  __syncthreads();
  if (kk > 0) {
    auto take = [&](uint32_t sbits, int r) {
      const unsigned long long key = key_of(sbits, r);
      if (key <= T) skeys[atomicAdd(&s_n, 1u)] = key;
    };
#pragma unroll
    for (int i = 0; i < TK_CACHE; ++i) {
      const int r = i * TK_THREADS + tid;
      if (r < nb) take(sb[i], r);
    }
    for (int r = TK_CACHE * TK_THREADS + tid; r < nb; r += TK_THREADS) take(sigma_bits(sigma[r0 + r]), r);
  }
  __syncthreads();
  if (k <= 512) {
    unsigned long long* sorted = skeys + S;
    if (tid < kk) {
      const unsigned long long mine = skeys[tid];
      int rank = 0;
      for (int j = 0; j < kk; ++j) rank += skeys[j] < mine ? 1 : 0;
      sorted[rank] = mine;
    }
    __syncthreads();
    if (tid < kk) skeys[tid] = sorted[tid];
    __syncthreads();
  } else {
    for (int k2 = 2; k2 <= S; k2 <<= 1)
      for (int j2 = k2 >> 1; j2 > 0; j2 >>= 1) {
        for (int e = tid; e < S / 2; e += TK_THREADS) {
          const int i = ((e & ~(j2 - 1)) << 1) | (e & (j2 - 1));
          const int q = i | j2;
          const bool up = (i & k2) == 0;
          const unsigned long long x = skeys[i], y = skeys[q];
          if ((x > y) == up) { skeys[i] = y; skeys[q] = x; }
        }
        __syncthreads();
      }
  }
  for (int i = tid; i < k; i += TK_THREADS) sel_rows[(int64_t)b * k + i] = (i < kk) ? r0 + (int32_t)(skeys[i] & 0xFFFFFFFFu) : -1;
  if (tid == 0) sel_count[b] = kk;
  if (out_desc) {
    if ((dc & 3) == 0) {
      const int q4 = dc >> 2;
      for (int t = tid; t < k * q4; t += TK_THREADS) {
        const int i = t / q4, c = t - i * q4;
        float4 v = make_float4(0.f, 0.f, 0.f, 0.f);
        if (i < kk) v = *reinterpret_cast<const float4*>(desc + (int64_t)(r0 + (int32_t)(skeys[i] & 0xFFFFFFFFu)) * dc + 4 * c);
        *reinterpret_cast<float4*>(out_desc + ((int64_t)b * k + i) * dc + 4 * c) = v;
      }
    } else {
      for (int64_t t = tid; t < (int64_t)k * dc; t += TK_THREADS) {
        const int i = (int)(t / dc), c = (int)(t - (int64_t)i * dc);
        out_desc[((int64_t)b * k + i) * dc + c] = (i < kk) ? desc[(int64_t)(r0 + (int32_t)(skeys[i] & 0xFFFFFFFFu)) * dc + c] : 0.f;
      }
    }
    for (int t = tid; t < k * 3; t += TK_THREADS) {
      const int i = t / 3, c = t - i * 3;
      out_kp[((int64_t)b * k + i) * 3 + c] = (i < kk) ? kp[(int64_t)(r0 + (int32_t)(skeys[i] & 0xFFFFFFFFu)) * 3 + c] : 0.f;
    }
  }
}
int select_topk(const float* sigma, const int32_t* boff_dev, int B, int k, const float* kp, const float* desc, int dc,
                int32_t* sel_rows, int32_t* sel_count, float* out_kp, float* out_desc, hipStream_t stream) {
  EGONN_REQUIRE(k >= 1 && k <= 8192, EGONN_ERR_INVALID, "select_keypoints: n_k=%d outside [1, 8192]", k);
  int S = 64;
  while (S < k) S <<= 1;
  const size_t lds = (size_t)(S + (k <= 512 ? k : 0)) * sizeof(unsigned long long);
  static AttrOnce attr_done;
  if (attr_done.need()) {
    HIP_CHECK(hipFuncSetAttribute(reinterpret_cast<const void*>(&select_topk_kernel), hipFuncAttributeMaxDynamicSharedMemorySize,
                                  128 * 1024));
    attr_done.mark(); 
  }
  hipLaunchKernelGGL(select_topk_kernel, dim3(B), dim3(TK_THREADS), lds, stream, sigma, boff_dev, k, S, kp, desc, dc, sel_rows,
// ... 7 lines not shown
```

### egonn_amd/csrc/kernels.h

```cpp
#pragma once
#include "common.h"

namespace egonn {

const char* last_error();

bool sconv_rg_supported(int cin, int cout);
int pack_rg_weights(const float* W, int K, int cin, int cout, int bf16, int flip, int transpose, void* out,
                    hipStream_t stream);
extern unsigned long long* g_sconv_trace;
struct PackedKernel {
  const void* rg32 = nullptr;
  const void* rg16 = nullptr;
  const void* split = nullptr;
};
struct ConvCall {
  int kind = 0, level = 0;
  const void* in = nullptr; void* out = nullptr;
  int cin = 0, cout = 0, bf16 = 0;
  const float *scale = nullptr, *shift = nullptr;
  int relu = 0;
  float* psum = nullptr;
  const PackedKernel* packed = nullptr;
  const float* W = nullptr; float* scratch = nullptr; size_t scratch_floats = 0;
  int split_io = 0;
  const float *in2 = nullptr, *gate = nullptr;
  const float* residual = nullptr;
};
enum SconvRoute {
  ROUTE_PLAIN,
  ROUTE_SPLIT,
  ROUTE_TAIL_SPLIT,
  ROUTE_WG,
  ROUTE_DMA,
  ROUTE_RG
};
SconvRoute sconv_route(const Ctx* ctx, int kind, int level, int cin, int cout, int bf16);
bool sconv_split_arithmetic(const Ctx* ctx);
const char* sconv_kernel_name(const Ctx* ctx, int kind, int level, int cin, int cout, int bf16);
struct SconvLaunch {
  SconvRoute route = ROUTE_RG;
  const RowGroups* rg = nullptr;
  int64_t n_in_cap = 0;
  int64_t groups_hint = 0;
  const void* Wp = nullptr;
  int variant = 0;
  bool small = false;
  int32_t* flags = nullptr;
  int B = 0;
  int kparts = 1, kw = 0, col_parts = 0;
  int resident = 0, resident_wgs = 0;
  float* part = nullptr; size_t part_floats = 0;
  uint32_t* in_absmax = nullptr; int64_t in_elems = 0;
};
int sconv_rg_forward(const ConvCall& c, const SconvLaunch& l, hipStream_t stream);
int sconv_map(Ctx* ctx, const ConvCall& c, hipStream_t stream);
bool sconv_split_supported(int cin, int cout);
int pack_split_weights(const float* W, int K, int cin, int cout, int flip, int transpose, void* out, hipStream_t stream);
size_t split_weights_bytes(int K, int cin, int cout);
int sconv_split_forward(const ConvCall& c, const SconvLaunch& l, hipStream_t stream);
size_t sconv_split_part_floats(const RowGroups& rg, int cout, int kparts);
void sconv_ksplit_rule(const Ctx* ctx, int kind, int level, int* kparts, int* col_parts, int* kw);
void sconv_ksplit_defaults(KsRule* r);
size_t sconv_ksplit_scratch_floats(const Ctx* ctx);
int sconv_resident_bit(int kind, int level, int cin, int cout, bool gated);
static constexpr size_t SCONV_SCRATCH_FLOATS = (size_t)2 << 20;
int sconv_naive(const float* in, const int32_t* nbr, const float* W, const float* scale, const float* shift, int relu,
                float* out, int64_t n_out, int K, int cin, int cout, hipStream_t stream);
int conv0_lut_init(Ctx* ctx);
int conv0_k5_forward(Ctx* ctx, const float* feat, const float* W, int cout, const float* scale,
                     const float* shift, int relu, void* out, int out_bf16, hipStream_t stream, const void* wpk = nullptr);
int conv0_pack_unit(const float* W, void* wpk, hipStream_t stream);

enum Act { ACT_NONE = 0, ACT_RELU = 1, ACT_TANH = 2, ACT_SOFTPLUS = 3, ACT_SIGMOID = 4 };
struct DenseCall {
  const void* in = nullptr; int in_bf16 = 0;
  int64_t n = 0;
  const int32_t* n_dev = nullptr;
  int cin = 0, cout = 0;
  const float* W = nullptr;
  int w_out_in = 0;
  const float* wfrag = nullptr;
  const float* bias = nullptr;
  const float *scale = nullptr, *shift = nullptr;
  int act = 0;
  const void* residual = nullptr; int res_bf16 = 0;
  const float* gate = nullptr;
  const int32_t* boff = nullptr;
  int B = 0;
  void* out = nullptr; int out_bf16 = 0;
  int form = -1;
};
enum DenseRoute {
  DENSE_INVALID = -1,
  DENSE_NONE = 0,
  DENSE_STREAM,
  DENSE_LDS,
  DENSE_SMALL,
  DENSE_TILE,
  DENSE_PLAIN
};
struct DenseLaunch {
  DenseRoute route = DENSE_NONE;
  unsigned gx = 0, gy = 0;
  size_t lds = 0;
  int colblk = 0;
};
DenseRoute dense_route(int64_t n, int cin, int cout, int form);
DenseLaunch dense_launch(int64_t n, int cin, int cout, int form, int gate_scans);
int dense_forward(const DenseCall& c, hipStream_t stream);
bool dense_gate_fusable(int64_t n, int cin, int cout);
bool dense_group3_rows(int64_t n);
int dense_small_group3(const float* const* in, const int64_t* n, const int32_t* const* n_dev, const float* const* W, float* const* out,
                       hipStream_t stream);
int dense_pack_frags(const float* W, int w_out_in, int cin, int cout, float* out, hipStream_t stream);

int bn_fold(const float* w, const float* b, const float* rm, const float* rv, float eps, int c, float* scale,
            float* shift, hipStream_t stream);
int gather_rows(const float* in, const int32_t* perm, int64_t n, int c, float* out, hipStream_t stream,
                const int32_t* n_dev = nullptr);
static constexpr int SEG_CHUNKS = 32;
int segment_partial_sums(const float* in, const int32_t* boff, int B, int c, int pow_mode, const float* p,
                         float* partial, hipStream_t stream);
int eca_apply(const float* x, const float* res, const float* partial, const int32_t* boff, int B, int64_t n, int c,
              const float* wconv, int ksize, float* out, hipStream_t stream);
int eca_gate_groups(const float* psum, const RowGroups& rg, const int32_t* boff, int B, int c, const float* wconv, int ksize,
                    float* gate, hipStream_t stream);
int eca_apply_gate(const void* x, const void* res, const float* gate, const int32_t* boff, int B, int64_t n, int c,
                   void* out, int bf16, hipStream_t stream);
int convert_bf16_to_f32(const void* in, int64_t n, float* out, hipStream_t stream);
int gem_finish(const float* partial, const int32_t* boff, int B, int c, const float* p, float* out,
               hipStream_t stream);
int pool_finish(const float* partial, const int32_t* boff, int B, int c, int mode, float* out, hipStream_t stream);
int l2_normalize_rows(float* x, int64_t n, int c, hipStream_t stream, const int32_t* n_dev = nullptr);
int add_act(const float* a, const float* b, int64_t n, int relu, float* out, hipStream_t stream);

constexpr int LH_WAVES = 8;
int keypoint_positions(const uint64_t* keys, int64_t n, int level, int cb, const float* offsets, int mode,
                       const float* step, int ignore_offsets, float* out, hipStream_t stream, const int32_t* n_dev = nullptr);
int local_heads_forward(const float* x, int64_t n, const int32_t* n_dev, const float* const* w, const uint64_t* keys,
                        int level, int cb, int mode, const float* step, int ignore_offsets, float* out_desc, float* out_kp,
                        float* out_sigma, hipStream_t stream, const float* lateral_w = nullptr, const float* lateral_res = nullptr,
                        int in_bf16 = 0, const void* split_pack = nullptr, int32_t* flags = nullptr);
size_t local_heads_pack_bytes();
int local_heads_pack(const float* const* w6_dev, void* out, hipStream_t stream);
int select_topk(const float* sigma, const int32_t* boff_dev, int B, int k, const float* kp, const float* desc, int dc,
                int32_t* sel_rows , int32_t* sel_count , float* out_kp, float* out_desc, hipStream_t stream);

static constexpr int NV_K = 64;
static constexpr int NV_MAX_CHUNKS = 32;
static constexpr int NV_CHUNK_ROWS = 128;
__host__ __device__ static inline int nv_chunks(int32_t len) {
  if (len <= 0) return 0;
  const int n = (len + NV_CHUNK_ROWS - 1) / NV_CHUNK_ROWS;
  return n < NV_MAX_CHUNKS ? n : NV_MAX_CHUNKS;
}
size_t netvlad_workspace_floats(int B, int C, int D);
void netvlad_workspace_carve(float* ws, int B, int C, float** part, float** vraw, float** sq, float** pp);
int netvlad_forward(const float* x, const int32_t* boff, int B, int C, const float* wc, const float* w2, const float* sc1,
                    const float* sh1, const float* H, int D, const float* sc2, const float* sh2, const float* wg,
                    const float* scg, const float* shg, int gating, float* out, float* ws, hipStream_t stream);

constexpr int LL_CLOUD_CHUNK = 1024;
constexpr int LL_STATS = 16;

}
```

### egonn_amd/csrc/model.h

```cpp
#pragma once
#include <map>
#include <string>
#include <vector>

#include "../../include/egonn_hip.h"
#include "common.h"
#include "kernels.h"

struct egonn_ctx : public egonn::Ctx {
  hipStream_t plan_stream = nullptr;

  void* level_feat[EGONN_NUM_LEVELS] = {};
  int level_ch[EGONN_NUM_LEVELS] = {};
  int level_bf16 = 0;
  bool from_points = false;
};

#define REQUIRE_PLAN(c)                                                                               \
  EGONN_REQUIRE((c) && (c)->plan.valid, EGONN_ERR_STATE, "no coordinate plan (call egonn_voxelize / " \
                                                         "egonn_coords_set first)")
#define REQUIRE_LEVEL(c, level)                                                                              \
  REQUIRE_PLAN(c);                                                                                           \
  HIP_CHECK(hipSetDevice((c)->device));                                                                      \
  EGONN_REQUIRE((level) >= 0 && (level) < EGONN_NUM_LEVELS, EGONN_ERR_INVALID, "level %d out of range", (level))

#define DBG_SYNC(...)                                                 \
  do {                                                                \
    if (switches().debug_sync) {                                      \
      fprintf(stderr, "[egonn] " __VA_ARGS__);                        \
      fprintf(stderr, "\n");                                          \
      fflush(stderr);                                                 \
      HIP_CHECK(hipStreamSynchronize(st));                            \
    }                                                                 \
  } while (0)

#define WALLOC(T, var, count)                                                      \
  T* var = A->alloc<T>((size_t)(count));                                           \
  EGONN_REQUIRE(var != nullptr, EGONN_ERR_STATE, "work arena too small (" #var ")")

namespace egonn {

int claim_work(egonn_ctx* c, size_t bytes, bool with_ksplit, Arena** A);

struct TensorRef {
  const float* p = nullptr;
  std::vector<int64_t> shape;
};

struct BnRef {
  const float *w = nullptr, *b = nullptr, *rm = nullptr, *rv = nullptr;
  float *scale = nullptr, *shift = nullptr;
  int c = 0;
};

struct BlockRef {
  const float *conv1 = nullptr, *conv2 = nullptr, *down = nullptr, *eca = nullptr;
  BnRef n1, n2, dn;
  int cin = 0, cout = 0, eca_k = 0;
};

struct MlpRef {
  const float *w0 = nullptr, *b0 = nullptr, *w1 = nullptr, *b1 = nullptr;
  int cin = 0, mid = 0, cout = 0;
};

struct ModelStore {
  enum Form { RG32, RG16, SPLIT, DENSE };
  struct Pack { Form form; const float* w; int K, ci, co; size_t off; const void** dst; };
  std::vector<BnRef*> bns;
  std::vector<Pack> packs;
  size_t bn_bytes = 0, pack_bytes = 0;
  char *folded = nullptr, *packed = nullptr;
  size_t folded_cap = 0, packed_cap = 0;

  void begin();
  void add_bn(BnRef* bn);
  void add_pack(Form form, const float* w, int K, int ci, int co, const void** dst);
  void add_kernel(const float* w, int K, int ci, int co, bool bf16, PackedKernel* dst);
  int commit(hipStream_t st);
  void release();
};

struct MinkFpnModel;
void minkfpn_model_free(MinkFpnModel* f);
void minkfpn_model_invalidate(MinkFpnModel* f);

}

struct egonn_model {
  std::map<std::string, egonn::TensorRef> t;
  bool ready = false;
  egonn::ModelStore store;
  const float* conv0 = nullptr;
  egonn::BnRef bn[8];
  const float* convs[8] = {};
  egonn::BlockRef blk[8];
  const float *g1x1[8] = {}, *gt[8] = {}, *l1x1[8] = {}, *lt[8] = {};
  const float* gem_p = nullptr;
  egonn::MlpRef gdec, ldec, kp, sg;
  void* conv0_unit = nullptr;
  void* lh_pack = nullptr;
  const float** lh_ptrs = nullptr;
  egonn::PackedKernel pk_convs[8], pk_c1[8], pk_c2[8], pk_gt[8], pk_lt[8];
  const void *pk_down[8] = {}, *pk_l1x1[8] = {};
  egonn::MinkFpnModel* fpn = nullptr;
};

namespace egonn {

int get_tensor(egonn_model* m, const std::string& key, std::initializer_list<int64_t> want, const float** out);
int get_bn(egonn_model* m, const std::string& prefix, int c, BnRef* bn, ModelStore* store);
int get_block(egonn_model* m, const std::string& prefix, int ci, int co, bool eca, BlockRef* b, ModelStore* store);
int eca_ksize(int c);
int conv_layer(egonn_ctx* c, hipStream_t st, const ConvCall& cc, const char* what);
ConvCall conv_call(int kind, int level, const void* in, const PackedKernel& pk, int cin, int cout, int bf16, const BnRef* bn, int relu,
                   void* out);
int ensure_graph_rowgroups(egonn_ctx* c, int L, const int* tlevels, int nt, hipStream_t st);
int block_convs(egonn_ctx* c, hipStream_t st, Arena* A, int level, const BlockRef& b, const PackedKernel& pk1, const PackedKernel& pk2,
                int bf16, const void* in, float* psum, void** t2);
DenseCall down_call(const BlockRef& b, const void* in, int bf16, int64_t n, const int32_t* n_dev, const void* wfrag);
int block_tail(const float* x, const float* res, const int32_t* boff, int B, int64_t n, int ch, const float* eca, int eca_k,
               float* partial, float* out, hipStream_t st);
enum Pooling { POOL_GEM = 1, POOL_MAC = 2, POOL_SPOC = 3 };
int global_pool(Pooling method, const float* x, const int32_t* boff, int B, int C, const float* p, float* partial, float* out,
                hipStream_t st);

bool topdown_split_supported(int C, int Cl);
int topdown_split_forward(Ctx* ctx, int level_out, const float* x_coarse, const void* sp_tconv, const float* x_lateral,
                          const void* sp_lateral, int C, int Cl, float* out, hipStream_t stream);

}
```

### egonn_amd/csrc/model.hip

```cpp
#include "model.h"

using namespace egonn;

namespace {

const int PLANES[7] = {32, 64, 64, 128, 128, 128, 128};
const int GLOBAL_CH = 128, GLOBAL_DIM = 256, LOCAL_CH = 64, LOCAL_DIM = 128;

}

API const char* egonn_last_error(void) { return last_error(); }

API int egonn_debug_set_naive_conv(egonn_ctx* c, int on) {
  EGONN_REQUIRE(c, EGONN_ERR_INVALID, "debug_set_naive_conv: null context");
  if (on >= 1000) { c->conv_variant = on; return EGONN_OK; }
  c->conv_variant = (on == 1) ? 3 : (on == 2 ? 1 : (on == 4 ? 2 : (on == 8 ? 4 : (on == 16 ? 5 : (on == 32 ? 6 : (on == 128 ? 9 : 0))))));
  return EGONN_OK;
}

API int egonn_debug_set_ksplit(egonn_ctx* c, int map_class, int level, int kparts, int kw, int col_parts) {
  EGONN_REQUIRE(c && (map_class == 0 || map_class == 1) && level >= 0 && level < EGONN_NUM_LEVELS, EGONN_ERR_INVALID,
                "debug_set_ksplit: bad argument");
  EGONN_REQUIRE(kparts <= 27 && kw <= 4 && col_parts <= 4, EGONN_ERR_INVALID, "debug_set_ksplit: kparts <= 27, kw <= 4, col_parts <= 4");
  if (kparts >= 0) c->ks_rule.kparts[map_class][level] = (int8_t)std::max(kparts, 1);
// ... 597 lines not shown
  auto dense = [&](const float* w, int ci, int co, const void** dst) {
    *dst = nullptr;
    if (ci % 16 == 0 && co % 16 == 0) S.add_pack(ModelStore::DENSE, w, 1, ci, co, dst);
  };
  EGONN_TRY(get_tensor(m, "trunk.convs.0.kernel", {125, 1, 32}, &m->conv0));
  EGONN_TRY(get_bn(m, "trunk.bn.0", 32, &m->bn[0], &S));
  int inpl = PLANES[0];
  for (int i = 1; i <= 7; ++i) {
    const std::string si = std::to_string(i);
    const int cout = PLANES[i - 1];
    EGONN_TRY(get_tensor(m, "trunk.convs." + si + ".kernel", {8, inpl, inpl}, &m->convs[i]));
    EGONN_TRY(get_bn(m, "trunk.bn." + si, inpl, &m->bn[i], &S));
    BlockRef& b = m->blk[i];
    EGONN_TRY(get_block(m, "trunk.blocks." + si + ".0", inpl, cout, true, &b, &S));
    S.add_kernel(m->convs[i], 8, inpl, inpl, true, &m->pk_convs[i]);
    S.add_kernel(b.conv1, 27, inpl, cout, true, &m->pk_c1[i]);
    S.add_kernel(b.conv2, 27, cout, cout, true, &m->pk_c2[i]);
    m->pk_down[i] = nullptr;
    if (b.down) dense(b.down, inpl, cout, &m->pk_down[i]);
    inpl = cout;
  }
  for (int l : {5, 6, 7})
    EGONN_TRY(get_tensor(m, "global_head.conv1x1." + std::to_string(l) + ".kernel", {PLANES[l - 1], GLOBAL_CH}, &m->g1x1[l]));
  for (int l : {6, 7}) {
    EGONN_TRY(get_tensor(m, "global_head.tconv." + std::to_string(l) + ".kernel", {8, GLOBAL_CH, GLOBAL_CH}, &m->gt[l]));
    S.add_kernel(m->gt[l], 8, GLOBAL_CH, GLOBAL_CH, true, &m->pk_gt[l]);
  }
  for (int l : {3, 4}) {
    EGONN_TRY(get_tensor(m, "local_head.conv1x1." + std::to_string(l) + ".kernel", {PLANES[l - 1], LOCAL_CH}, &m->l1x1[l]));
    dense(m->l1x1[l], PLANES[l - 1], LOCAL_CH, &m->pk_l1x1[l]);
  }
  EGONN_TRY(get_tensor(m, "local_head.tconv.4.kernel", {8, LOCAL_CH, LOCAL_CH}, &m->lt[4]));
  S.add_kernel(m->lt[4], 8, LOCAL_CH, LOCAL_CH, true, &m->pk_lt[4]);
  m->gem_p = nullptr;
  if (m->t.count("global_pooling.pooling.p")) EGONN_TRY(get_tensor(m, "global_pooling.pooling.p", {1}, &m->gem_p));
  EGONN_TRY(get_mlp(m, "global_descriptor_decoder", GLOBAL_CH, GLOBAL_DIM + (GLOBAL_CH - GLOBAL_DIM) / 2, GLOBAL_DIM, &m->gdec));
  EGONN_TRY(get_mlp(m, "local_descriptor_decoder", LOCAL_CH, LOCAL_DIM + (LOCAL_CH - LOCAL_DIM) / 2, LOCAL_DIM, &m->ldec));
  EGONN_TRY(get_mlp(m, "local_keypoint_regressor", LOCAL_CH, LOCAL_CH / 2, 3, &m->kp));
  EGONN_TRY(get_mlp(m, "local_sigma_regressor", LOCAL_CH, LOCAL_CH / 2, 1, &m->sg));

  EGONN_TRY(S.commit(st));
  if (!m->conv0_unit) HIP_CHECK(hipMalloc(&m->conv0_unit, 2 * 4 * 3 * 64 * 16));
  EGONN_TRY(conv0_pack_unit(m->conv0, m->conv0_unit, st));
  if (m->ldec.cin == 64 && m->ldec.mid == 96 && m->ldec.cout == 128 && m->kp.mid == 32 && m->sg.mid == 32 && m->kp.cin == 64 &&
      m->sg.cin == 64) {
    if (!m->lh_pack) HIP_CHECK(hipMalloc(&m->lh_pack, local_heads_pack_bytes()));
    if (!m->lh_ptrs) HIP_CHECK(hipMalloc(reinterpret_cast<void**>(&m->lh_ptrs), 6 * sizeof(float*)));
    const float* hp[6] = {m->ldec.w0, m->ldec.w1, m->kp.w0, m->kp.w1, m->sg.w0, m->sg.w1};
    HIP_CHECK(hipMemcpyAsync(m->lh_ptrs, hp, sizeof(hp), hipMemcpyHostToDevice, st));
    HIP_CHECK(hipStreamSynchronize(st));
    EGONN_TRY(local_heads_pack(m->lh_ptrs, m->lh_pack, st));
  }
  m->ready = true;
  return EGONN_OK;
}

namespace {

int run_mlp(const MlpRef& r, const float* x, int64_t n, int act_out, float* hidden, float* out, hipStream_t st,
            const int32_t* n_dev) {
  EGONN_TRY(dense_forward({.in = x, .n = n, .n_dev = n_dev, .cin = r.cin, .cout = r.mid, .W = r.w0, .w_out_in = 1, .bias = r.b0,
                           .act = ACT_RELU, .out = hidden},
                          st));
  return dense_forward({.in = hidden, .n = n, .n_dev = n_dev, .cin = r.mid, .cout = r.cout, .W = r.w1, .w_out_in = 1, .bias = r.b1,
                        .act = act_out, .out = out},
                       st);
}

}

namespace egonn {

int claim_work(egonn_ctx* c, size_t bytes, bool with_ksplit, Arena** A) {
  for (int l = 0; l < EGONN_NUM_LEVELS; ++l) c->level_feat[l] = nullptr;
  c->ks_part = nullptr;
  c->ks_part_floats = 0;
  EGONN_TRY(c->work_arena.ensure(bytes));
  c->work_arena.reset();
  *A = &c->work_arena;
  const size_t ks = with_ksplit ? sconv_ksplit_scratch_floats(c) : 0;
  if (ks) {
    c->ks_part = (*A)->alloc<float>(ks);
    EGONN_REQUIRE(c->ks_part, EGONN_ERR_STATE, "work arena too small (ks_part)");
    c->ks_part_floats = ks;
  }
  return EGONN_OK;
}

int conv_layer(egonn_ctx* c, hipStream_t st, const ConvCall& cc, const char* what) {
  static const int pk[3] = {PK_K3, PK_K2S2, PK_TCONV};
  char tag[64];
  snprintf(tag, sizeof(tag), "%s<%d,%d>/L%d/%s", sconv_kernel_name(c, cc.kind, cc.level, cc.cin, cc.cout, cc.bf16), cc.cin, cc.cout,
           cc.level, what);
  ProfScope ps(c, st, tag, pk[cc.kind], cc.level, cc.kind == 0 ? 27 : 8, cc.cin, cc.cout, cc.bf16 ? 2 : 4);
  return sconv_map(c, cc, st);
}
ConvCall conv_call(int kind, int level, const void* in, const PackedKernel& pk, int cin, int cout, int bf16, const BnRef* bn, int relu,
                   void* out) {
  return ConvCall{.kind = kind, .level = level, .in = in, .out = out, .cin = cin, .cout = cout, .bf16 = bf16,
                  .scale = bn ? bn->scale : nullptr, .shift = bn ? bn->shift : nullptr, .relu = relu, .packed = &pk};
}

int ensure_graph_rowgroups(egonn_ctx* c, int L, const int* tlevels, int nt, hipStream_t st) {
  int kinds[RG_MAX_JOBS], levels[RG_MAX_JOBS], n = 0;
  for (int l = 1; l <= L; ++l) { kinds[n] = 0; levels[n++] = l; }
  for (int l = 1; l <= L; ++l) { kinds[n] = 1; levels[n++] = l; }
  for (int i = 0; i < nt; ++i) { kinds[n] = 2; levels[n++] = tlevels[i]; }
  return ensure_rowgroups(c, kinds, levels, n, st);
}

int block_convs(egonn_ctx* c, hipStream_t st, Arena* A, int level, const BlockRef& b, const PackedKernel& pk1, const PackedKernel& pk2,
                int bf16, const void* in, float* psum, void** t2_out) {
  const size_t bytes = (size_t)c->plan.cap[level] * b.cout * (bf16 ? 2 : 4);
  WALLOC(char, t1, bytes);
  WALLOC(char, t2, bytes);
  const bool t1_split = !switches().no_presplit && sconv_route(c, 0, level, b.cin, b.cout, bf16) == ROUTE_SPLIT &&
                        sconv_route(c, 0, level, b.cout, b.cout, bf16) == ROUTE_SPLIT;
  ConvCall c1 = conv_call(0, level, in, pk1, b.cin, b.cout, bf16, &b.n1, 1, t1);
  c1.split_io = t1_split ? 2 : 0;
  EGONN_TRY(conv_layer(c, st, c1, "k3.conv1"));
  ConvCall c2 = conv_call(0, level, t1, pk2, b.cout, b.cout, bf16, &b.n2, 0, t2);
  c2.split_io = t1_split ? 1 : 0;
  c2.psum = psum;
  EGONN_TRY(conv_layer(c, st, c2, "k3.conv2"));
  *t2_out = t2;
  return EGONN_OK;
}

DenseCall down_call(const BlockRef& b, const void* in, int bf16, int64_t n, const int32_t* n_dev, const void* wfrag) {
  return DenseCall{.in = in, .in_bf16 = bf16, .n = n, .n_dev = n_dev, .cin = b.cin, .cout = b.cout, .W = b.down,
                   .wfrag = static_cast<const float*>(wfrag), .scale = b.dn.scale, .shift = b.dn.shift, .out_bf16 = bf16};
}

int global_pool(Pooling method, const float* x, const int32_t* boff, int B, int C, const float* p, float* partial, float* out,
                hipStream_t st) {
  if (method == POOL_GEM) {
    EGONN_TRY(segment_partial_sums(x, boff, B, C, 1, p, partial, st));
    return gem_finish(partial, boff, B, C, p, out, st);
  }
  const int mode = method == POOL_MAC ? 2 : 0;
  EGONN_TRY(segment_partial_sums(x, boff, B, C, mode, nullptr, partial, st));
  return pool_finish(partial, boff, B, C, mode, out, st);
}

int block_tail(const float* x, const float* res, const int32_t* boff, int B, int64_t n, int ch, const float* eca, int eca_k,
               float* partial, float* out, hipStream_t st) {
  if (!eca) return add_act(x, res, n * ch, 1, out, st);
  EGONN_TRY(segment_partial_sums(x, boff, B, ch, 0, nullptr, partial, st));
  return eca_apply(x, res, partial, boff, B, n, ch, eca, eca_k, out, st);
}

}

API int egonn_forward(egonn_ctx* c, egonn_model* m, const float* features, int quant_mode, const float* step, int flags,
                      float* out_global, float* out_desc, float* out_kp, float* out_sigma, void* stream) {
  REQUIRE_PLAN(c);
  EGONN_REQUIRE(m && m->ready, EGONN_ERR_STATE, "model not finalized (call egonn_model_finalize)");
  EGONN_REQUIRE(step, EGONN_ERR_INVALID, "forward: null argument");
  HIP_CHECK(hipSetDevice(c->device));
  hipStream_t st = (hipStream_t)stream;
  Plan& P = c->plan;
  const int B = P.batch;
  const int32_t* cnt = c->dev_counts;
  const int bf16 = (flags & EGONN_FLAG_BF16) ? 1 : 0;
  const size_t es = bf16 ? 2 : 4;
  const bool do_global = !(flags & EGONN_FLAG_DISABLE_GLOBAL);
  const bool do_local = !(flags & EGONN_FLAG_DISABLE_LOCAL);
  EGONN_REQUIRE(!do_global || out_global, EGONN_ERR_INVALID, "forward: out_global is null");
  EGONN_REQUIRE(!do_local || (out_desc && out_kp && out_sigma), EGONN_ERR_INVALID, "forward: local outputs are null");
  HIP_CHECK(hipMemsetAsync(c->dev_fp16_flag, 0, sizeof(int32_t), st));

  {
    const int tlevels[3] = {6, 5, 3};
    EGONN_TRY(ensure_graph_rowgroups(c, 7, tlevels + (do_global ? 0 : 2), (do_global ? 2 : 0) + (do_local ? 1 : 0), st));
    DBG_SYNC("row groups");
  }

  size_t need = (size_t)P.cap[0] * (1 + 32) * 4;
  for (int i = 1; i <= 7; ++i) need += (size_t)P.cap[i] * 128 * 4 * 6 + (size_t)P.lv[i].rg27.cap_groups * 128 * 4;
  need += (size_t)P.cap[5] * (192 + 256 + 128 * 2) * 4 + (size_t)P.cap[3] * (96 + 32 + 32 + 3 + 64 * 2) * 4;
  need += (size_t)B * SEG_CHUNKS * 256 * 4 * 10 + (size_t)P.cap[3] * 32 + (4u << 20);
  need += sconv_ksplit_scratch_floats(c) * 4 + 4096;
  Arena* A;
  EGONN_TRY(claim_work(c, need, true, &A));

  const int64_t n0 = P.cap[0];
  const float* f0 = features;
  if (features && !c->from_points) {
    WALLOC(float, fg, n0);
    EGONN_TRY(gather_rows(features, P.perm0, n0, 1, fg, st, cnt));
    f0 = fg;
  }
  WALLOC(char, x0, n0 * 32 * es);
  {
    ProfScope ps(c, st, "conv0_k5_kernel/L0", PK_CONV0, 0, 125, 1, 32, (int)es);
    EGONN_TRY(conv0_k5_forward(c, f0, m->conv0, 32, m->bn[0].scale, m->bn[0].shift, 1, x0, bf16, st, m->conv0_unit));
  }
  DBG_SYNC("conv0");
  const void* x[8] = {x0};
  c->level_feat[0] = x0;
  c->level_ch[0] = 32;
  c->level_bf16 = bf16;
  auto local_head = [&](hipStream_t st) -> int {
    const int64_t n3 = P.cap[3], n4 = P.cap[4];
    WALLOC(char, l4, n4 * LOCAL_CH * es);
    EGONN_TRY(dense_forward({.in = x[4], .in_bf16 = bf16, .n = n4, .n_dev = cnt + 4, .cin = 128, .cout = LOCAL_CH, .W = m->l1x1[4],
                             .wfrag = static_cast<const float*>(m->pk_l1x1[4]), .out = l4, .out_bf16 = bf16},
                            st));
    WALLOC(char, u3, n3 * LOCAL_CH * es);
    EGONN_TRY(conv_layer(c, st, conv_call(2, 3, l4, m->pk_lt[4], LOCAL_CH, LOCAL_CH, bf16, nullptr, 0, u3), "tconv"));
    EGONN_REQUIRE(m->ldec.cin == 64 && m->ldec.mid == 96 && m->ldec.cout == 128 && m->kp.mid == 32 && m->sg.mid == 32,
                  EGONN_ERR_STATE, "local heads: unexpected layer sizes");
    const float* hw[12] = {m->ldec.w0, m->ldec.b0, m->ldec.w1, m->ldec.b1, m->kp.w0, m->kp.b0, m->kp.w1, m->kp.b1,
                           m->sg.w0, m->sg.b0, m->sg.w1, m->sg.b1};
    const void* lh_pack = (!switches().no_split_heads && sconv_split_arithmetic(c)) ? m->lh_pack : nullptr;
    if (!switches().no_fused_lateral && LOCAL_CH == 64) {
      EGONN_TRY(local_heads_forward(reinterpret_cast<const float*>(x[3]), n3, cnt + 3, hw, P.lv[3].keys, 3, P.coord_bits, quant_mode,
                                    step, (flags & EGONN_FLAG_IGNORE_KP_REGRESSOR) ? 1 : 0, out_desc, out_kp, out_sigma, st,
                                    m->l1x1[3], reinterpret_cast<const float*>(u3), bf16, lh_pack, c->dev_fp16_flag));
      return EGONN_OK;
    }
    WALLOC(float, l3, n3 * LOCAL_CH);
    EGONN_TRY(dense_forward({.in = x[3], .in_bf16 = bf16, .n = n3, .n_dev = cnt + 3, .cin = 64, .cout = LOCAL_CH, .W = m->l1x1[3],
                             .wfrag = static_cast<const float*>(m->pk_l1x1[3]), .residual = u3, .res_bf16 = bf16, .out = l3},
                            st));
    EGONN_TRY(local_heads_forward(l3, n3, cnt + 3, hw, P.lv[3].keys, 3, P.coord_bits, quant_mode, step,
                                  (flags & EGONN_FLAG_IGNORE_KP_REGRESSOR) ? 1 : 0, out_desc, out_kp, out_sigma, st, nullptr, nullptr, 0,
                                  lh_pack, c->dev_fp16_flag));
    return EGONN_OK;
  };
  const float *gated_t2 = nullptr, *gated_res = nullptr, *gated_gate = nullptr;
  for (int i = 1; i <= 7; ++i) {
    const BlockRef& b = m->blk[i];
    const Level& L = P.lv[i];
    const int64_t n = P.cap[i];
    WALLOC(char, y, n * b.cin * es);
    {
      ConvCall cc = conv_call(1, i, x[i - 1], m->pk_convs[i], b.cin, b.cin, bf16, &m->bn[i], 1, y);
      if (gated_t2 && i == 2) {
        cc.in = gated_t2;
        cc.in2 = gated_res;
        cc.gate = gated_gate;
      }
      EGONN_TRY(conv_layer(c, st, cc, "k2s2"));
    }
    DBG_SYNC("L%d k2s2", i);
    WALLOC(float, psum, (size_t)L.rg27.cap_groups * b.cout);
    void* t2 = nullptr;
    EGONN_TRY(block_convs(c, st, A, i, b, m->pk_c1[i], m->pk_c2[i], bf16, y, psum, &t2));
    WALLOC(float, gate, (size_t)B * b.cout);
    DBG_SYNC("L%d convs", i);
    EGONN_TRY(eca_gate_groups(psum, L.rg27, L.boff, B, b.cout, b.eca, b.eca_k, gate, st));
    DBG_SYNC("L%d eca gate", i);
    const void* res = y;
    if (i == 1 && !switches().no_gated_k2s2 && !c->keep_level_features && !bf16 && !b.down && c->conv_variant == 0 && b.cout == 32 &&
        m->blk[2].cin == 32 && sconv_route(c, 1, 2, 32, 32, 0) == ROUTE_SPLIT) {
      gated_t2 = reinterpret_cast<const float*>(t2);
      gated_res = reinterpret_cast<const float*>(y);
      gated_gate = gate;
      x[i] = nullptr;
      c->level_feat[i] = nullptr;
      c->level_ch[i] = b.cout;
      continue;
    }
    WALLOC(char, xo, n * b.cout * es);
    const DenseCall down = down_call(b, y, bf16, n, cnt + i, m->pk_down[i]);
    if (b.down && !switches().no_fused_down && dense_gate_fusable(n, b.cin, b.cout)) {
      DenseCall dc = down;
      dc.residual = t2; dc.res_bf16 = bf16;
      dc.gate = gate; dc.boff = L.boff; dc.B = B;
      dc.out = xo;
      EGONN_TRY(dense_forward(dc, st));
    } else {
      if (b.down) {
        WALLOC(char, rd, n * b.cout * es);
        DenseCall dc = down;
        dc.out = rd;
        EGONN_TRY(dense_forward(dc, st));
        res = rd;
      }
      EGONN_TRY(eca_apply_gate(t2, res, gate, L.boff, B, n, b.cout, xo, bf16, st));
    }
    DBG_SYNC("L%d eca apply", i);
    x[i] = xo;
    c->level_feat[i] = xo;
    c->level_ch[i] = b.cout;
  }
  if (do_local) EGONN_TRY(local_head(st));
  DBG_SYNC("local head");

  void* g5_fused = nullptr;
  if (do_global && !switches().no_fused_ghead && !bf16 && c->conv_variant == 0 && dense_group3_rows(P.cap[5]) &&
      dense_group3_rows(P.cap[6]) && dense_group3_rows(P.cap[7])) {
    WALLOC(float, l7, P.cap[7] * GLOBAL_CH);
    WALLOC(float, l6, P.cap[6] * GLOBAL_CH);
    WALLOC(float, l5, P.cap[5] * GLOBAL_CH);
    WALLOC(float, g6f, P.cap[6] * GLOBAL_CH);
    WALLOC(float, g5f, P.cap[5] * GLOBAL_CH);
    const float* gin[3] = {reinterpret_cast<const float*>(x[7]), reinterpret_cast<const float*>(x[6]), reinterpret_cast<const float*>(x[5])};
    const int64_t gn[3] = {P.cap[7], P.cap[6], P.cap[5]};
    const int32_t* gnd[3] = {cnt + 7, cnt + 6, cnt + 5};
    const float* gw[3] = {m->g1x1[7], m->g1x1[6], m->g1x1[5]};
    float* gout[3] = {l7, l6, l5};
    EGONN_TRY(dense_small_group3(gin, gn, gnd, gw, gout, st));
    for (int lv = 6; lv >= 5; --lv) {
      ConvCall cc = conv_call(2, lv, lv == 6 ? l7 : g6f, m->pk_gt[lv + 1], GLOBAL_CH, GLOBAL_CH, 0, nullptr, 0, lv == 6 ? g6f : g5f);
      cc.residual = lv == 6 ? l6 : l5;
      EGONN_TRY(conv_layer(c, st, cc, "tconv"));
    }
    g5_fused = g5f;
    DBG_SYNC("global head (fused)");
  }
  if (do_global) {
    const float* g5 = reinterpret_cast<const float*>(g5_fused);
    if (!g5) {
    auto lateral = [&](int l, const void* up, void* out, int out_bf16) {
      return dense_forward({.in = x[l], .in_bf16 = bf16, .n = P.cap[l], .n_dev = cnt + l, .cin = 128, .cout = GLOBAL_CH, .W = m->g1x1[l],
                            .residual = up, .res_bf16 = up ? bf16 : 0, .out = out, .out_bf16 = out_bf16},
                           st);
    };
    WALLOC(char, g7, P.cap[7] * GLOBAL_CH * es);
    EGONN_TRY(lateral(7, nullptr, g7, bf16));
    WALLOC(char, u6, P.cap[6] * GLOBAL_CH * es);
    EGONN_TRY(conv_layer(c, st, conv_call(2, 6, g7, m->pk_gt[7], GLOBAL_CH, GLOBAL_CH, bf16, nullptr, 0, u6), "tconv"));
    WALLOC(char, g6, P.cap[6] * GLOBAL_CH * es);
    EGONN_TRY(lateral(6, u6, g6, bf16));
    WALLOC(char, u5, P.cap[5] * GLOBAL_CH * es);
    EGONN_TRY(conv_layer(c, st, conv_call(2, 5, g6, m->pk_gt[6], GLOBAL_CH, GLOBAL_CH, bf16, nullptr, 0, u5), "tconv"));
    WALLOC(float, g5u, P.cap[5] * GLOBAL_CH);
    EGONN_TRY(lateral(5, u5, g5u, 0));
    g5 = g5u;
    DBG_SYNC("global head");
    }
    WALLOC(float, gh, P.cap[5] * m->gdec.mid);
    WALLOC(float, gd, P.cap[5] * GLOBAL_DIM);
    EGONN_TRY(run_mlp(m->gdec, g5, P.cap[5], ACT_NONE, gh, gd, st, cnt + 5));
    WALLOC(float, gp, (size_t)B * SEG_CHUNKS * GLOBAL_DIM);
    const Pooling pool = (flags & EGONN_FLAG_POOL_MAC) ? POOL_MAC : (flags & EGONN_FLAG_POOL_SPOC) ? POOL_SPOC : POOL_GEM;
    EGONN_REQUIRE(pool != POOL_GEM || m->gem_p, EGONN_ERR_STATE, "forward: GeM pooling needs the tensor 'global_pooling.pooling.p'");
    EGONN_TRY(global_pool(pool, gd, P.lv[5].boff, B, GLOBAL_DIM, m->gem_p, gp, out_global, st));
  }

  DBG_SYNC("global decoder + pooling");
  return EGONN_OK;
}

API int egonn_forward_level_features(egonn_ctx* c, int level, float* out, int channels, void* stream) {
  REQUIRE_PLAN(c);
  EGONN_REQUIRE(level >= 0 && level < EGONN_NUM_LEVELS && c->level_feat[level], EGONN_ERR_STATE,
                "no features for level %d (run egonn_forward first; level 1 of fp32 maps is materialised only after "
                "egonn_debug_keep_level_features(ctx, 1))", level);
  EGONN_REQUIRE(channels == c->level_ch[level], EGONN_ERR_INVALID, "level %d has %d channels, caller expects %d", level,
                c->level_ch[level], channels);
  const int64_t cnt = c->plan.lv[level].n * channels;
  if (c->level_bf16) return convert_bf16_to_f32(c->level_feat[level], cnt, out, (hipStream_t)stream);
  HIP_CHECK(hipMemcpyAsync(out, c->level_feat[level], sizeof(float) * cnt, hipMemcpyDeviceToDevice, (hipStream_t)stream));
  return EGONN_OK;
}

API int egonn_select_keypoints(egonn_ctx* c, const float* sigma, const float* keypoints, const float* descriptors,
                               int n_k, float* sel_kp, float* sel_desc, int32_t* sel_rows, int32_t* sel_count,
                               void* stream) {
  REQUIRE_PLAN(c);
  EGONN_REQUIRE(sigma && keypoints && descriptors && sel_kp && sel_desc && sel_rows && sel_count, EGONN_ERR_INVALID,
                "select_keypoints: null argument");
  HIP_CHECK(hipSetDevice(c->device));
  return select_topk(sigma, c->plan.lv[3].boff, c->plan.batch, n_k, keypoints, descriptors, LOCAL_DIM, sel_rows, sel_count,
                     sel_kp, sel_desc, (hipStream_t)stream);
}


API int egonn_topk_rows(const float* sigma, const int32_t* row_offsets, int batch_size, int n_k, int32_t* sel_rows,
                        int32_t* sel_count, void* stream) {
  EGONN_REQUIRE(sigma && row_offsets && sel_rows && sel_count && batch_size >= 1, EGONN_ERR_INVALID, "topk_rows: bad argument");
  return select_topk(sigma, row_offsets, batch_size, n_k, nullptr, nullptr, 0, sel_rows, sel_count, nullptr, nullptr,
                     (hipStream_t)stream);
}

API int egonn_profile_enable(egonn_ctx* c, int mode, const char* filter) {
  EGONN_REQUIRE(c && mode >= 0 && mode <= 3, EGONN_ERR_INVALID, "profile_enable: bad argument");
  c->prof.mode = mode;
  snprintf(c->prof.filter, sizeof(c->prof.filter), "%s", filter ? filter : "");
  return EGONN_OK;
}

API int egonn_profile_fetch(egonn_ctx* c, int cap, int* n, char* names, float* ms, double* bytes, double* flops,
                            void* stream) {
  EGONN_REQUIRE(c && n && names && ms && bytes && flops, EGONN_ERR_INVALID, "profile_fetch: null argument");
  HIP_CHECK(hipSetDevice(c->device));
  Plan& P = c->plan;
  if (P.valid) {
    if (P.built_reserved) P.exact = false;
    EGONN_TRY(plan_sync(c, (hipStream_t)stream));
    EGONN_TRY(count_map_pairs(c, (hipStream_t)stream));
  }
  HIP_CHECK(hipStreamSynchronize((hipStream_t)stream));
  unsigned long long pairs[16];
  HIP_CHECK(hipMemcpy(pairs, c->dev_pairs, sizeof(pairs), hipMemcpyDeviceToHost));
  int w = 0;
  std::vector<ProfRec> all(c->prof.recs);
  all.insert(all.end(), c->prof.graph_recs.begin(), c->prof.graph_recs.end());
  const size_t n_plain = c->prof.recs.size();
  size_t ri = 0;
  for (auto& r : all) {
    const bool plain = ri++ < n_plain;
    float t = 0.f;
    if (hipEventSynchronize(r.e1) != hipSuccess || hipEventElapsedTime(&t, r.e0, r.e1) != hipSuccess) {
      (void)hipGetLastError();
      if (plain) { c->prof.pool.push_back(r.e0); c->prof.pool.push_back(r.e1); }
      continue;
    }
    if (w < cap) {
      const double n_out = (double)P.lv[r.level].n;
      double Pn = 0;
      switch (r.kind) {
        case PK_CONV0: Pn = (double)pairs[0]; break;
        case PK_K3: Pn = (double)pairs[r.level]; break;
        case PK_K2S2: Pn = (double)P.lv[r.level - 1].n; break;
        case PK_TCONV: Pn = n_out; break;
        default: Pn = n_out; break;
      }
      snprintf(names + (size_t)w * 64, 64, "%s", r.name);
      ms[w] = t;
      bytes[w] = Pn * r.cin * r.es + n_out * r.cout * r.es + (double)r.K * r.cin * r.cout * r.es + 8.0 * Pn;
      flops[w] = 2.0 * Pn * r.cin * r.cout;
      ++w;
    }
    if (plain) { c->prof.pool.push_back(r.e0); c->prof.pool.push_back(r.e1); }
  }
  c->prof.recs.clear();
  *n = w;
  return EGONN_OK;
}
```

### egonn_amd/evaluator.py

```python
from __future__ import annotations

from typing import Dict, List, Sequence

import numpy as np
import torch

from . import _lib
from .model import MinkGL
from .minkloc import _MinkLocBase


class DescriptorExtractor:
    def __init__(self, model: MinkGL, n_k: int = 128, ignore_keypoint_saliency: bool = False):
        self.model = model
        self.n_k = n_k
        self.quantizer = model.quantizer
        self.ignore_keypoint_saliency = ignore_keypoint_saliency

    @torch.no_grad()
    def compute_embedding(self, pc, model: MinkGL = None):
        model = model or self.model
        pc = pc if isinstance(pc, torch.Tensor) else torch.as_tensor(np.asarray(pc), dtype=torch.float32)
        out = self.extract([pc], model=model)
        n = int(out['count'][0].item())
        global_embedding = out['global'].cpu().numpy()
        return global_embedding, out['keypoints'][0, :n].cpu(), out['descriptors'][0, :n].cpu()

    def get_keypoints_idxes(self, sigmas: torch.Tensor, n_k: int):
        n = sigmas.shape[0]
        if self.ignore_keypoint_saliency:
            return torch.randperm(n)[:min(n_k, n)]
        ctx = self.model.context()
        dev = ctx.device
        sg = sigmas.detach().to(device=dev, dtype=torch.float32).reshape(-1).contiguous()
        rows = torch.empty((1, n_k), dtype=torch.int32, device=dev)
        cnt = torch.empty((1,), dtype=torch.int32, device=dev)
        boff = torch.tensor([0, n], dtype=torch.int32, device=dev)
        _lib.call(dev, ctx.lib.egonn_topk_rows, sg.data_ptr(), boff.data_ptr(), 1, n_k, rows.data_ptr(), cnt.data_ptr())
        return rows[0, :int(cnt[0].item())].long().cpu()

    @torch.no_grad()
    def extract(self, scans: Sequence[torch.Tensor], model: MinkGL = None) -> Dict[str, torch.Tensor]:
        model = model or self.model
        ctx = model.context()
        dev = ctx.device
        pts = [torch.as_tensor(s, dtype=torch.float32).to(dev) for s in scans]
        offsets = [0]
        for p in pts:
            offsets.append(offsets[-1] + p.shape[0])
        allpts = pts[0].contiguous() if len(pts) == 1 else torch.cat(pts, dim=0)
        out = self.extract_packed(allpts, offsets, model)
        try:
            ctx.plan_status()
        except _lib.Fp16RangeError:
            ctx.set_exact_fp32(True)
            try:
                y = model._forward_on_plan(ctx, None)
                d, k, s = model._last_local
                if self.ignore_keypoint_saliency:
                    s = torch.rand_like(s)
                sel_kp, sel_desc, rows, cnt = ctx.select_keypoints(s, k, d, self.n_k)
                ctx.plan_status()
            finally:
                ctx.set_exact_fp32(False)
            out = {'global': y['global'], 'keypoints': sel_kp, 'descriptors': sel_desc, 'count': cnt, 'rows': rows}
        return out

    @torch.no_grad()
    def extract_packed(self, points: torch.Tensor, offsets: List[int], model: MinkGL = None, slot: int = 0):
        model = model or self.model
        ctx = model.context(slot)
        q = self.quantizer
        ctx.voxelize(points, offsets, q.mode, q.step)
        y = model._forward_on_plan(ctx, None)
        d, k, s = model._last_local
        if self.ignore_keypoint_saliency:
            s = torch.rand_like(s)
        sel_kp, sel_desc, rows, cnt = ctx.select_keypoints(s, k, d, self.n_k)
        return {'global': y['global'], 'keypoints': sel_kp, 'descriptors': sel_desc, 'count': cnt, 'rows': rows}

    @torch.no_grad()
    def calibrate(self, points: torch.Tensor, offsets: List[int], margin: float = 1.3):
        ctx = self.model.context(0)
        q = self.quantizer
        ctx.voxelize(points, offsets, q.mode, q.step)
        return [int(ctx.level_count(l) * margin) + 1024 for l in range(8)]

    def graph(self, batch_size: int, max_points: int, level_capacity=None, slot: int = 0, stream=None):
        return GraphExtractor(self, batch_size, max_points, level_capacity, slot, stream)

    @torch.no_grad()
    def extract_stream(self, batches, n_streams: int = 2, model: MinkGL = None):
        model = model or self.model
        dev = model.context(0).device
        model._sync_weights()
        if getattr(self, '_streams', None) is None or len(self._streams) != n_streams:
            self._streams = [torch.cuda.Stream(device=dev) for _ in range(n_streams)]
        torch.cuda.current_stream(dev).synchronize()
        for i, (points, offsets) in enumerate(batches):
            slot = i % n_streams
            with torch.cuda.stream(self._streams[slot]):
                yield self.extract_packed(points, offsets, model, slot=slot)

    def _ones(self, n, dev):
        buf = getattr(self, '_ones_buf', None)
        if buf is None or buf.shape[0] < n or buf.device != dev:
            buf = torch.ones((max(n, 1) * 5 // 4 + 1024, 1), dtype=torch.float32, device=dev)
            torch.cuda.synchronize(dev)
            self._ones_buf = buf
        return buf[:n]


class GraphExtractor:

    def __init__(self, extractor: DescriptorExtractor, batch_size: int, max_points: int, level_capacity=None, slot: int = 0,
                 stream=None):
        self.ex = extractor
        model = extractor.model
        self.model = model
        self.ctx = model.context(slot)
        self.B = int(batch_size)
        self.max_points = int(max_points)
        ctx, dev = self.ctx, self.ctx.device
        model._sync_weights()
        ctx.reserve(self.max_points, self.B, level_capacity)
        self.points = torch.zeros((self.max_points, 3), dtype=torch.float32, device=dev)
        self.offsets = torch.zeros((self.B + 1,), dtype=torch.int64, device=dev)
        self._host_off = torch.zeros((self.B + 1,), dtype=torch.int64).pin_memory()
        self._off_copied = None
        self.stream = stream if stream is not None else torch.cuda.Stream(device=dev)
        self.graph = None
        self.out = None

    def _enqueue(self):
        ctx, model, q = self.ctx, self.model, self.ex.quantizer
        ctx.voxelize_device(self.points, self.offsets, self.B, q.mode, q.step)
        if self.out is None:
            dev = ctx.device
            cap3 = ctx.level_capacity(3)
            n_k = self.ex.n_k
            self.out = {
                'global': torch.zeros((self.B, model.global_descriptor_size), dtype=torch.float32, device=dev),
                'all_descriptors': torch.zeros((cap3, model.local_descriptor_size), dtype=torch.float32, device=dev),
                'all_keypoints': torch.zeros((cap3, 3), dtype=torch.float32, device=dev),
                'all_sigma': torch.zeros((cap3, 1), dtype=torch.float32, device=dev),
                'keypoints': torch.zeros((self.B, n_k, 3), dtype=torch.float32, device=dev),
                'descriptors': torch.zeros((self.B, n_k, model.local_descriptor_size), dtype=torch.float32, device=dev),
                'rows': torch.zeros((self.B, n_k), dtype=torch.int32, device=dev),
                'count': torch.zeros((self.B,), dtype=torch.int32, device=dev),
            }
        o = self.out
        model._forward_on_plan(ctx, None, outputs=(o['global'], o['all_descriptors'], o['all_keypoints'], o['all_sigma']))
        _lib.call(ctx.device, ctx.lib.egonn_select_keypoints, ctx.h, o['all_sigma'].data_ptr(), o['all_keypoints'].data_ptr(),
                  o['all_descriptors'].data_ptr(), self.ex.n_k, o['keypoints'].data_ptr(), o['descriptors'].data_ptr(),
                  o['rows'].data_ptr(), o['count'].data_ptr())

    def _load(self, points: torch.Tensor, offsets):
        n = int(offsets[-1])
        if n > self.max_points or len(offsets) != self.B + 1:
            raise ValueError(f"batch of {n} points / {len(offsets) - 1} scans does not fit the reservation "
                             f"({self.max_points} points, {self.B} scans)")
        if self._off_copied is not None:
            self._off_copied.synchronize()
        cur = torch.cuda.current_stream(self.ctx.device) if not hasattr(self, "_caller_stream") else self._caller_stream
        if cur != self.stream:
            self.stream.wait_stream(cur)
            if points.is_cuda:
                points.record_stream(self.stream)
        self._host_off.copy_(torch.as_tensor(list(offsets), dtype=torch.int64))
        self.points[:n].copy_(points[:n], non_blocking=True)
        self.offsets.copy_(self._host_off, non_blocking=True)
        self._off_copied = torch.cuda.Event()
        self._off_copied.record(self.stream)

    @torch.no_grad()
    def run(self, points: torch.Tensor, offsets):
        ctx = self.ctx
        self._caller_stream = torch.cuda.current_stream(ctx.device)
        with torch.cuda.stream(self.stream):
            self._load(points, offsets)
            if self.graph is None:
                self._enqueue()
                self.stream.synchronize()
                ctx.plan_status()
                g = _lib._P()
                _lib.check(ctx.lib.egonn_graph_begin(self.stream.cuda_stream))
                try:
                    self._enqueue()
                finally:
                    rc = ctx.lib.egonn_graph_end(self.stream.cuda_stream, _lib.C.byref(g))
                _lib.check(rc)
                self.graph = g
            _lib.check(ctx.lib.egonn_graph_launch(self.graph, self.stream.cuda_stream))
        return self.out

    def replay(self):
        _lib.check(self.ctx.lib.egonn_graph_launch(self.graph, self.stream.cuda_stream))
        return self.out

    def status(self):
        with torch.cuda.stream(self.stream):
            self.ctx.plan_status()

    def __del__(self):
        try:
            if getattr(self, 'graph', None):
                self.ctx.lib.egonn_graph_destroy(self.graph)
                self.graph = None
        except Exception:
            pass


class GlobalExtractor:

    def __init__(self, model, quantizer=None):
        if isinstance(model, _MinkLocBase):
            model.minkfpn_spec()
            self.dim = model.feature_size
        elif isinstance(model, MinkGL):
            self.dim = model.global_descriptor_size
        else:
            raise NotImplementedError(f"GlobalExtractor: {type(model).__name__} is neither a MinkLoc-type model nor MinkGL")
        self.model = model
        self.quantizer = quantizer if quantizer is not None else getattr(model, 'quantizer', None)
        if self.quantizer is None:
            raise ValueError("GlobalExtractor: the model carries no quantizer (model_factory attaches one): pass quantizer=")

    def _forward(self, ctx: _lib.Context, out: Dict[str, torch.Tensor]):
        m = self.model
        if isinstance(m, MinkGL):
            if 'map' in out:
                raise NotImplementedError("GlobalExtractor: the feature map is an output of the MinkLoc-type models only")
            m._forward_on_plan(ctx, None, disable_local_head=True, outputs=(out['global'], None, None, None))
        else:
            m.forward_on_plan(ctx, outputs=(out['global'], out.get('map')))
        return out

    def _outputs(self, ctx: _lib.Context, batch_size: int, want_map: bool):
        out = {'global': torch.empty((batch_size, self.dim), dtype=torch.float32, device=ctx.device)}
        if want_map:
            if isinstance(self.model, MinkGL):
                raise NotImplementedError("GlobalExtractor: the feature map is an output of the MinkLoc-type models only")
            out['map'] = torch.empty((ctx.level_capacity(self.model.out_level), self.dim), dtype=torch.float32, device=ctx.device)
        return out

    @torch.no_grad()
    def extract(self, scans: Sequence[torch.Tensor], want_map: bool = False) -> Dict[str, torch.Tensor]:
        dev = self.model.context().device
        pts = [torch.as_tensor(s, dtype=torch.float32).to(dev) for s in scans]
        offsets = [0]
        for p in pts:
            offsets.append(offsets[-1] + p.shape[0])
        allpts = pts[0].contiguous() if len(pts) == 1 else torch.cat(pts, dim=0)
        return self.extract_checked(allpts, offsets, want_map=want_map)

    @torch.no_grad()
    def extract_checked(self, points: torch.Tensor, offsets: List[int], slot: int = 0, want_map: bool = False):
        ctx = self.model.context(slot)
        out = self.extract_packed(points, offsets, slot, want_map=want_map)
        try:
            ctx.plan_status()
        except _lib.Fp16RangeError:
            ctx.set_exact_fp32(True)
            try:
                out = self._forward(ctx, out)
                ctx.plan_status()
            finally:
                ctx.set_exact_fp32(False)
        return out

    @torch.no_grad()
    def extract_packed(self, points: torch.Tensor, offsets: List[int], slot: int = 0, want_map: bool = False):
        ctx = self.model.context(slot)
        q = self.quantizer
        ctx.voxelize(points, offsets, q.mode, q.step)
        return self._forward(ctx, self._outputs(ctx, len(offsets) - 1, want_map))

    @torch.no_grad()
    def calibrate(self, points: torch.Tensor, offsets: List[int], margin: float = 1.3):
        ctx = self.model.context(0)
        q = self.quantizer
        ctx.voxelize(points, offsets, q.mode, q.step)
        return [int(ctx.level_count(l) * margin) + 1024 for l in range(8)]

    def graph(self, batch_size: int, max_points: int, level_capacity=None, slot: int = 0, stream=None, want_map: bool = False):
        return GlobalGraphExtractor(self, batch_size, max_points, level_capacity, slot, stream, want_map)

    @torch.no_grad()
    def extract_stream(self, batches, n_streams: int = 2):
        dev = self.model.context(0).device
        self.model._sync_weights()
        if getattr(self, '_streams', None) is None or len(self._streams) != n_streams:
            self._streams = [torch.cuda.Stream(device=dev) for _ in range(n_streams)]
        torch.cuda.current_stream(dev).synchronize()
        for i, (points, offsets) in enumerate(batches):
            slot = i % n_streams
            with torch.cuda.stream(self._streams[slot]):
                yield self.extract_packed(points, offsets, slot=slot)


class GlobalGraphExtractor(GraphExtractor):

    def __init__(self, extractor: GlobalExtractor, batch_size: int, max_points: int, level_capacity=None, slot: int = 0,
                 stream=None, want_map: bool = False):
        super().__init__(extractor, batch_size, max_points, level_capacity, slot, stream)
        self.want_map = want_map

    def _enqueue(self):
# ... 6 lines not shown
```

### egonn_amd/model.py

```python
from __future__ import annotations

from typing import Dict, List

import numpy as np
import torch
import torch.nn as nn

from . import _lib
from .quantization import Quantizer

PLANES = [32, 64, 64, 128, 128, 128, 128]
GLOBAL_LEVELS, GLOBAL_CH, GLOBAL_DIM = [5, 6, 7], 128, 256
LOCAL_LEVELS, LOCAL_CH, LOCAL_DIM = [3, 4], 64, 128


class SparseConv(nn.Module):

    def __init__(self, cin, cout, kernel_size, transpose=False):
        super().__init__()
        kv = kernel_size ** 3
        self.kernel_size, self.transpose = kernel_size, transpose
        shape = (cin, cout) if kv == 1 else (kv, cin, cout)
        self.kernel = nn.Parameter(torch.empty(*shape))
        with torch.no_grad():
# ... 232 lines not shown
        assert coords.dim() == 2 and coords.shape[1] == 4 and feats.shape[0] == coords.shape[0]
        bs = batch.get('batch_size', None)
        if bs is None:
            bs = int(coords[:, 0].max().item()) + 1
        ctx.coords_set(coords, bs)
        return ctx, feats


class MinkGL(PlanModule):

    def __init__(self, trunk: MinkTrunk, local_head: MinkHead = None, local_descriptor_size: int = None,
                 local_normalize: bool = True, global_head: MinkHead = None, global_descriptor_size: int = None,
                 global_pool_method: str = 'GeM', global_normalize: bool = False, quantizer: Quantizer = None):
        assert quantizer is not None
        super().__init__()
        self.trunk = trunk
        self.global_head = global_head
        if global_pool_method not in ('GeM', 'MAC', 'SPoC'):
            raise NotImplementedError(f'global pooling method {global_pool_method!r}: the MinkGL (egonn) path implements '
                                      f'GeM, MAC and SPoC; NetVLAD pooling is available in MinkLoc only')
        self.global_pool_method = global_pool_method
        self.global_channels = global_head.out_channels
        self.global_pooling = PoolingWrapper(global_pool_method, self.global_channels, self.global_channels)
        self.global_normalize = global_normalize
        self.global_descriptor_size = global_descriptor_size
        self.global_descriptor_decoder = DescriptorDecoder(self.global_channels, global_descriptor_size,
                                                           normalize=False)
        self.local_head = local_head
        if local_head is not None:
            self.local_descriptor_size = local_descriptor_size
            self.local_normalize = local_normalize
            n = local_head.out_channels
            self.local_keypoint_regressor = KeypointRegressor(n, reduction=2)
            self.local_sigma_regressor = SigmaRegressor(n, reduction=2)
            self.local_descriptor_decoder = DescriptorDecoder(n, local_descriptor_size, normalize=local_normalize)
        self.quantizer = quantizer
        self.ignore_keypoint_regressor = False
        if global_normalize or (local_head is not None and not local_normalize) or local_head is None:
            raise NotImplementedError("the MI355X path implements the 'egonn' configuration "
                                      "(global_normalize=False, local_normalize=True, with local head)")
        self._handle = None
        self._registered = None

    def _float_state(self):
        for k, v in self.state_dict(keep_vars=True).items():
            if v.dtype == torch.float32:
                yield k, v

    def _sync_weights(self):
        sig = tuple((k, v.data_ptr(), v._version) for k, v in self.state_dict(keep_vars=True).items())
        if self._handle is not None and sig == self._registered:
            return
        if self._handle is None:
            self._handle = _lib.ModelHandle()
        for k, v in self._float_state():
            t = v.detach()
            if not t.is_contiguous():
                raise RuntimeError(f"parameter {k} is not contiguous")
            self._handle.set_tensor(k, t)
        self._handle.finalize()
        self._registered = sig

    def forward(self, batch: Dict[str, torch.Tensor], disable_global_head: bool = False,
                disable_local_head: bool = False, context_slot: int = 0):
        assert batch['features'].dim() == 2 and batch['features'].shape[1] == 1
        ctx, feats = self._plan(batch, context_slot)
        if self.training:
            return self._forward_train(ctx, feats, disable_global_head, disable_local_head)
        return self._forward_on_plan(ctx, feats, disable_global_head, disable_local_head)

    precision = 'fp32'

    sync_bn_group = None

    def _forward_train(self, ctx: _lib.Context, feats: torch.Tensor, disable_global_head: bool,
                       disable_local_head: bool = False):
        from . import train
        if not bool((feats == 1).all()):
            raise NotImplementedError("train mode supports the reference's all-ones input features only")
        y = {}
        ctx.prepare_maps(with_level0_transpose=True)
        levels = train.trunk_forward(self, ctx, self.sync_bn_group)
        if not disable_global_head:
            g = train.global_branch(self, ctx, self.sync_bn_group, levels)
            assert g.dim() == 2 and g.shape[1] == self.global_descriptor_size
            y['global'] = g
        if self.local_head is not None and not disable_local_head:
            lvl, desc, kp_off, sigma = train.local_branch(self, ctx, levels)
            coords = ctx.level_coords(lvl)
            stride = [2 ** lvl] * 3
            if self.ignore_keypoint_regressor:
                kp_off = torch.zeros_like(kp_off)
            kp_pos = self.quantizer.keypoint_position(coords[:, 1:], stride, kp_off)
            off = ctx.level_batch_offsets(lvl)
            B = ctx.batch_size
            y['descriptors'] = [desc[off[b]:off[b + 1]] for b in range(B)]
            y['keypoints'] = [kp_pos[off[b]:off[b + 1]] for b in range(B)]
            y['sigma'] = [sigma[off[b]:off[b + 1]] for b in range(B)]
        return y

    def _forward_on_plan(self, ctx: _lib.Context, feats: torch.Tensor, disable_global_head=False,
                         disable_local_head=False, outputs=None):
        self._sync_weights()
        dev = ctx.device
        B = ctx.batch_size
        lvl = min(LOCAL_LEVELS)
        if outputs is not None:
            out_g, out_d, out_k, out_s = outputs
            self._egonn_forward(ctx, feats, disable_global_head, disable_local_head, outputs)
            self._last_local = (out_d, out_k, out_s)
            return {'global': out_g, 'descriptors': out_d, 'keypoints': out_k, 'sigma': out_s}
        n3 = ctx.level_count(lvl)
        out_g = out_d = out_k = out_s = None
        if not disable_global_head:
            out_g = torch.empty((B, self.global_descriptor_size), dtype=torch.float32, device=dev)
        if not disable_local_head:
            out_d = torch.empty((n3, self.local_descriptor_size), dtype=torch.float32, device=dev)
            out_k = torch.empty((n3, 3), dtype=torch.float32, device=dev)
            out_s = torch.empty((n3, 1), dtype=torch.float32, device=dev)
        self._egonn_forward(ctx, feats, disable_global_head, disable_local_head, (out_g, out_d, out_k, out_s))
        y = {}
        if out_g is not None:
            assert out_g.dim() == 2 and out_g.shape[1] == self.global_descriptor_size
            y['global'] = out_g
        if out_d is not None:
            off = ctx.level_batch_offsets(lvl)
            y['descriptors'] = [out_d[off[b]:off[b + 1]] for b in range(B)]
            y['keypoints'] = [out_k[off[b]:off[b + 1]] for b in range(B)]
            y['sigma'] = [out_s[off[b]:off[b + 1]] for b in range(B)]
            self._last_local = (out_d, out_k, out_s)
        return y

    def _flags(self, disable_global_head, disable_local_head):
        flags = 0
        if disable_global_head:
            flags |= _lib.FLAG_DISABLE_GLOBAL
        if disable_local_head:
            flags |= _lib.FLAG_DISABLE_LOCAL
        if self.ignore_keypoint_regressor:
            flags |= _lib.FLAG_IGNORE_KP_REGRESSOR
        if self.precision == 'bf16':
            flags |= _lib.FLAG_BF16
        elif self.precision != 'fp32':
            raise ValueError(f"precision {self.precision!r}: 'fp32' or 'bf16'")
        flags |= {'GeM': 0, 'SPoC': _lib.FLAG_POOL_SPOC, 'MAC': _lib.FLAG_POOL_MAC}[self.global_pool_method]
        return flags

    def _egonn_forward(self, ctx, feats, disable_global_head, disable_local_head, outputs):
        q = self.quantizer
        step = (_lib.C.c_float * 3)(*([float(s) for s in q.step] + [0.0, 0.0])[:3])
        _lib.call(ctx.device, ctx.lib.egonn_forward, ctx.h, self._handle.h, _lib._ptr(feats), q.mode, step,
                  self._flags(disable_global_head, disable_local_head), *[_lib._ptr(t) for t in outputs])

    def keypoint_coords(self) -> List[torch.Tensor]:
        ctx = self.context()
        lvl = min(LOCAL_LEVELS)
        c = ctx.level_coords(lvl)
        off = ctx.level_batch_offsets(lvl)
        return [c[off[b]:off[b + 1]] for b in range(ctx.batch_size)]

    def print_info(self):
        print(f'Model class: {type(self).__name__}')
        n_params = sum(p.nelement() for p in self.parameters())
        n_trunk = sum(p.nelement() for p in self.trunk.parameters())
        print(f"# parameters - total: {n_params/1000:.1f}   trunk: {n_trunk/1000:.1f} [k]")
        if self.local_head is not None:
            n_local_head = sum(p.nelement() for p in self.local_head.parameters())
            n_kr = sum(p.nelement() for p in self.local_keypoint_regressor.parameters())
            n_kd = sum(p.nelement() for p in self.local_descriptor_decoder.parameters())
            n_sr = sum(p.nelement() for p in self.local_sigma_regressor.parameters())
            print(f'kp. head: {n_local_head/1000:.1f}   kp. regressor {n_kr/1000:.1f}   '
                  f'kp. descriptor {n_kd / 1000:.1f}   [k] kp. saliency regresor {n_sr/1000:.1f} [k]')
            print(f'# channels in the local map: {self.local_head.out_channels}   keypoint descriptor size: '
                  f'{self.local_descriptor_size}')
        n_gh = sum(p.nelement() for p in self.global_head.parameters())
        print(f'global descriptor head: {n_gh/1000:.1f} [k]   pool method: {self.global_pool_method}')
        print(f'# channels in the global map: {self.global_channels}   global descriptor size: '
              f'{self.global_descriptor_size}')


def create_egonn_model(model_params):
    if model_params.model != 'egonn':
        raise NotImplementedError(f'Unknown model: {model_params.model}')
    global_in_channels = [PLANES[i - 1] for i in GLOBAL_LEVELS]
    head_global = MinkHead(GLOBAL_LEVELS, global_in_channels, GLOBAL_CH)
    local_in_channels = [PLANES[i - 1] for i in LOCAL_LEVELS]
    head_local = MinkHead(LOCAL_LEVELS, local_in_channels, LOCAL_CH)
    trunk = MinkTrunk(in_channels=1, planes=PLANES, conv0_kernel_size=5)
    return MinkGL(trunk, local_head=head_local, local_descriptor_size=LOCAL_DIM, local_normalize=True,
                  global_head=head_global, global_descriptor_size=GLOBAL_DIM, global_pool_method='GeM',
                  global_normalize=False, quantizer=model_params.quantizer)


def model_factory(model_params):
    if model_params.model == 'MinkLoc':
        from .minkloc import MinkLoc
        m = MinkLoc(in_channels=1, feature_size=model_params.feature_size, output_dim=model_params.output_dim,
                    planes=model_params.planes, layers=model_params.layers,
                    num_top_down=model_params.num_top_down, conv0_kernel_size=model_params.conv0_kernel_size,
                    block=model_params.block, pooling_method=model_params.pooling)
        m.quantizer = model_params.quantizer
        return m
    if model_params.model == 'MinkLoc3D':
        from .minkloc import MinkLoc3D
        m = MinkLoc3D()
        m.quantizer = model_params.quantizer
        return m
    if 'egonn' in model_params.model:
        return create_egonn_model(model_params)
    raise NotImplementedError('Model not implemented: {}'.format(model_params.model))
```

### include/egonn_hip.h

```cpp
#ifndef EGONN_HIP_H
#define EGONN_HIP_H

#include <stdint.h>

#ifdef __cplusplus
extern "C" {
#endif

typedef struct egonn_ctx egonn_ctx;
typedef struct egonn_model egonn_model;

enum { EGONN_QUANT_CARTESIAN = 0, EGONN_QUANT_POLAR = 1 };
enum { EGONN_STATUS_OK = 0, EGONN_STATUS_INVALID = 1, EGONN_STATUS_HIP = 2, EGONN_STATUS_RANGE = 3, EGONN_STATUS_STATE = 4,
       EGONN_STATUS_CAPACITY = 5,
       EGONN_STATUS_FP16_RANGE = 6 };
enum { EGONN_FLAG_DISABLE_GLOBAL = 1, EGONN_FLAG_DISABLE_LOCAL = 2, EGONN_FLAG_IGNORE_KP_REGRESSOR = 4,
       EGONN_FLAG_BF16 = 8,
       EGONN_FLAG_POOL_SPOC = 16, EGONN_FLAG_POOL_MAC = 32 };

int egonn_ctx_create(egonn_ctx** ctx, int device, int coord_bits);
void egonn_ctx_destroy(egonn_ctx* ctx);
const char* egonn_last_error(void);
int egonn_debug_set_naive_conv(egonn_ctx* ctx, int on);
int egonn_debug_set_ksplit(egonn_ctx* ctx, int map_class, int level, int kparts, int kw, int col_parts);
int egonn_debug_set_resident(egonn_ctx* ctx, int mask, int max_workgroups);
int egonn_debug_keep_level_features(egonn_ctx* ctx, int on);
int egonn_debug_set_trace(void* device_buffer);
int egonn_debug_rowgroup_tables(egonn_ctx* ctx, int map_kind, int level_out, uint32_t* gmask_out, int32_t* snbr_out,
                                int64_t capacity_groups, int64_t* n_groups, void* stream);
int egonn_debug_rowgroup_perm(egonn_ctx* ctx, int map_kind, int level_out, int32_t* perm_out, int64_t capacity_groups,
                              int64_t* n_groups, void* stream);
int64_t egonn_debug_radix_sort_scratch_bytes(int64_t n, int n_segments);
int egonn_debug_radix_sort(uint64_t* keys_in, uint32_t* vals_in, uint64_t* keys_out, uint32_t* vals_out, int64_t n, int nbits,
                           const int64_t* n_dev, const int64_t* seg_offsets, int n_segments, int idx_bits, int either_pair,
                           int32_t* result_pair, void* scratch, int64_t scratch_bytes, void* stream);

int egonn_voxelize(egonn_ctx* ctx, const float* points, const int64_t* scan_offsets, int batch_size, int quant_mode,
                   const float* step, void* stream);
int egonn_ctx_reserve(egonn_ctx* ctx, int64_t max_points, int batch_size, const int64_t* level_capacity);
int egonn_voxelize_device(egonn_ctx* ctx, const float* points, int64_t n_rows, const int64_t* scan_offsets_dev,
                          int batch_size, int quant_mode, const float* step, void* stream);
int egonn_plan_status(egonn_ctx* ctx, void* stream);
int egonn_ctx_set_exact_fp32(egonn_ctx* ctx, int on);
int egonn_ctx_set_operand_autoscale(egonn_ctx* ctx, int on);
int egonn_level_capacity(egonn_ctx* ctx, int level, int64_t* capacity);
typedef struct egonn_graph egonn_graph;
int egonn_graph_begin(void* stream);
int egonn_graph_end(void* stream, egonn_graph** graph);
int egonn_graph_launch(egonn_graph* graph, void* stream);
void egonn_graph_destroy(egonn_graph* graph);
int egonn_coords_set(egonn_ctx* ctx, const int32_t* coords, int64_t n, int batch_size, void* stream);

int egonn_level_count(egonn_ctx* ctx, int level, int64_t* n_rows);
int egonn_level_batch_offsets(egonn_ctx* ctx, int level, int64_t* offsets );
int egonn_level_coords(egonn_ctx* ctx, int level, int32_t* out, void* stream);
int egonn_input_index(egonn_ctx* ctx, int64_t* out , void* stream);

int egonn_conv(egonn_ctx* ctx, int level_in, int level_out, int kernel_size, const float* in, int cin,
               const float* kernel, int cout, const float* scale, const float* shift, int relu, float* out,
               void* stream);
int egonn_conv_transpose(egonn_ctx* ctx, int level_in, const float* in, int cin, const float* kernel, int cout,
                         float* out, void* stream);
int egonn_sparse_conv(egonn_ctx* ctx, int map_kind, int level_out, const void* in, int cin, const float* kernel, int cout,
                      int bf16, const float* scale, const float* shift, int relu, void* out, float* group_sums,
                      void* stream);
int egonn_prepare_maps(egonn_ctx* ctx, int with_level0_transpose, void* stream);
int egonn_map_groups(egonn_ctx* ctx, int map_kind, int level_out, int64_t* n_groups, int64_t* first_group, void* stream);
int egonn_global_avg_pool(egonn_ctx* ctx, int level, const float* in, int channels, float* out, void* stream);

int egonn_bn_fold(const float* weight, const float* bias, const float* running_mean, const float* running_var,
                  float eps, int channels, float* scale, float* shift, void* stream);
int egonn_block_tail(egonn_ctx* ctx, int level, const float* x, const float* residual, int channels,
                     const float* eca_weight, int eca_ksize, float* out, void* stream);
int egonn_add(const float* a, const float* b, int64_t n, float* out, void* stream);
int egonn_gather_input(egonn_ctx* ctx, const float* features, int channels, float* out, void* stream);
int egonn_gem(egonn_ctx* ctx, int level, const float* x, int channels, const float* p, float* out, void* stream);
int egonn_global_max_pool(egonn_ctx* ctx, int level, const float* in, int channels, float* out, void* stream);
int egonn_netvlad(egonn_ctx* ctx, int level, const float* x, int channels, const float* cluster_weights,
                  const float* cluster_weights2, const float* bn1_scale, const float* bn1_shift,
                  const float* hidden1_weights, const float* bn2_scale, const float* bn2_shift,
                  const float* gating_weights, const float* gate_scale, const float* gate_shift, int out_dim, int gating,
                  float* out, void* stream);
int egonn_netvlad_train_forward(egonn_ctx* ctx, int level, const float* x, int channels, int nmax,
                                const float* cluster_weights, const float* cluster_weights2, const float* bn1_weight,
                                const float* bn1_bias, float bn1_eps, float bn1_momentum, float* bn1_running_mean,
                                float* bn1_running_var, const float* hidden1_weights, int out_dim, float* out, float* save_z,
                                float* save_bn1, float* save_v, float* save_sq, float* save_asum, void* stream);
int egonn_netvlad_train_backward(egonn_ctx* ctx, int level, const float* x, int channels, int nmax,
                                 const float* cluster_weights, const float* cluster_weights2, const float* bn1_weight,
                                 const float* hidden1_weights, int out_dim, const float* grad_out, const float* save_z,
                                 const float* save_bn1, const float* save_v, const float* save_sq, const float* save_asum,
                                 float* grad_x, float* grad_cluster_weights, float* grad_cluster_weights2, float* out_bn1,
                                 float* grad_hidden1_weights, void* stream);
int egonn_global_max_pool_argmax(egonn_ctx* ctx, int level, const float* in, int channels, float* out, int32_t* out_rows,
                                 void* stream);
int egonn_global_max_pool_backward(egonn_ctx* ctx, int level, const float* grad_out, const int32_t* rows, int channels,
                                   float* grad_in, void* stream);
int egonn_sigmoid_gate(const float* y, const float* t, const float* grad_out, int64_t n, float* out, float* grad_y,
                       float* grad_t, void* stream);

int egonn_model_create(egonn_model** model);
void egonn_model_destroy(egonn_model* model);
int egonn_model_set_tensor(egonn_model* model, const char* key, const float* data, int ndim, const int64_t* shape);
int egonn_model_finalize(egonn_model* model, void* stream);

int egonn_forward(egonn_ctx* ctx, egonn_model* model, const float* features, int quant_mode, const float* step,
                  int flags, float* out_global, float* out_descriptors, float* out_keypoints, float* out_sigma,
                  void* stream);
int egonn_forward_level_features(egonn_ctx* ctx, int level, float* out, int channels, void* stream);

int egonn_minkfpn_finalize(egonn_model* model, int n_levels, const int* planes, const int* layers, int num_top_down,
                           int feature_size, int block, int pooling, void* stream);
int egonn_minkfpn_out_level(int n_levels, int num_top_down, int* level);
enum { EGONN_MINKFPN_SPLIT_TOPDOWN = 1 };
int egonn_minkfpn_forward(egonn_ctx* ctx, egonn_model* model, int flags, float* out_global, float* out_map, void* stream);
int egonn_topdown_step(egonn_ctx* ctx, int level_out, const float* x_coarse, const float* w_tconv, const float* x_lateral,
                       const float* w_lateral, int C, int Cl, float* out, void* stream);

int egonn_select_keypoints(egonn_ctx* ctx, const float* sigma, const float* keypoints, const float* descriptors,
                           int n_k, float* sel_keypoints, float* sel_descriptors, int32_t* sel_rows,
                           int32_t* sel_count, void* stream);

int egonn_topk_rows(const float* sigma, const int32_t* row_offsets, int batch_size, int n_k, int32_t* sel_rows,
                    int32_t* sel_count, void* stream);

int64_t egonn_triplet_loss_scratch_floats(int n);
int egonn_triplet_loss(const float* embeddings, int n, int d, const uint8_t* positives_mask,
                       const uint8_t* negatives_mask, float margin, float* out_stats, int32_t* out_triplets,
                       float* out_grad, float* scratch, void* stream);

int64_t egonn_contrastive_loss_scratch_floats(int n);
int egonn_contrastive_loss(const float* embeddings, int n, int d, const uint8_t* positives_mask,
                           const uint8_t* negatives_mask, float pos_margin, float neg_margin, float* out_stats,
                           int32_t* out_triplets, float* out_grad, float* scratch, void* stream);

int egonn_nn_search(const float* a, int64_t n, const float* transform, const float* b, int64_t m, float* out_dist,
                    int32_t* out_index, void* stream);
int egonn_matrix_min(const float* d, int64_t n, int64_t m, float* row_min, int32_t* row_index, float* col_min,
                     int32_t* col_index, void* stream);
int egonn_softmax_cross_entropy(const float* logits, int64_t n, int64_t m, const int32_t* target, float* out_loss,
                                int32_t* out_argmax, float* out_dlogits, void* stream);

#define EGONN_LOCAL_LOSS_STATS 16
enum { EGONN_LL_LOSS = 0, EGONN_LL_KP_PER_CLOUD = 1, EGONN_LL_REPEATABILITY = 2, EGONN_LL_CHAMFER_PURE = 3,
       EGONN_LL_CHAMFER_WEIGHTED = 4, EGONN_LL_MEAN_SIGMA = 5, EGONN_LL_LOSS_CHAMFER = 6, EGONN_LL_LOSS_P2P = 7,
       EGONN_LL_KEYPOINT_LOSS = 8, EGONN_LL_CORRESPONDENCE_LOSS = 9, EGONN_LL_MATCHING_KEYPOINTS = 10,
       EGONN_LL_MATCHING_DESCRIPTORS = 11, EGONN_LL_POS_SIMILARITY = 12, EGONN_LL_NEG_SIMILARITY = 13  };
int64_t egonn_local_loss_scratch_bytes(int pairs, int64_t n_kp1, int64_t n_kp2, int dim);
int egonn_local_loss(int pairs, int64_t n_cloud1, int64_t n_cloud2, int64_t n_kp1, int64_t n_kp2, int dim,
                     const float* clouds1, const int32_t* cloud_off1, const float* clouds2, const int32_t* cloud_off2,
                     const float* kp1, const float* sigma1, const float* desc1, const int32_t* kp_off1,
                     const float* kp2, const float* sigma2, const float* desc2, const int32_t* kp_off2,
                     const float* transforms, const float* params, float* out_pair, float* out_batch,
                     float* g_kp1, float* g_sigma1, float* g_desc1, float* g_kp2, float* g_sigma2, float* g_desc2,
                     void* scratch, int64_t scratch_bytes, void* stream);

enum { EGONN_ACT_NONE = 0, EGONN_ACT_RELU = 1, EGONN_ACT_TANH = 2, EGONN_ACT_SOFTPLUS = 3, EGONN_ACT_SIGMOID = 4 };
int egonn_dense(const float* x, int64_t n, int cin, const float* weight, int weight_out_in, const float* bias, int cout,
                int act, float* out, void* stream);
int egonn_dense_pack_fragments(const float* weight, int weight_out_in, int cin, int cout, float* packed, void* stream);
int egonn_dense_pack_fragments_host(const float* weight, int weight_out_in, int cin, int cout, float* packed);
int egonn_debug_dense(const void* in, int in_bf16, int64_t rows_capacity, const int32_t* n_dev, int cin, int cout, const float* weight,
                      int weight_out_in, const float* packed, const float* bias, const float* scale, const float* shift, int act,
                      const void* residual, int res_bf16, const float* gate, const int32_t* boff, int B, void* out, int out_bf16,
                      int form, void* stream);
int egonn_debug_dense_route(int64_t rows, int cin, int cout, int form, int gate_scans, int32_t out[5]);
int egonn_dense_backward_weight(const float* a, int ca, const float* b, int cb, int64_t n, float* out, float* scratch,
                                int64_t scratch_floats, void* stream);
int egonn_conv_backward_weight(egonn_ctx* ctx, int level_in, int level_out, int kernel_size, int transposed,
                               const float* in, int cin, const float* grad_out, int cout, float* grad_kernel,
                               float* scratch, int64_t scratch_floats, void* stream);
int egonn_col_stats(int mode, const float* a, const float* b, const float* mask, const float* mean, int64_t n, int c,
                    double* out, float* scratch, int64_t scratch_floats, void* stream);
int egonn_bn_train_finalize(const double* sums, const float* shift_point, double count, int c, const float* weight,
                            const float* bias, float eps, float momentum, float* running_mean, float* running_var,
                            float* out_mean_invstd_scale_shift, void* stream);
int egonn_bn_backward_finalize(const double* local_sums, const double* global_sums, double count, int c, const float* weight,
                               const float* mean, const float* invstd, float* out_abc_dgamma_dbeta, void* stream);
int egonn_affine_act(const float* x, const float* scale, const float* shift, int64_t n, int c, int relu, float* out,
                     void* stream);
int egonn_affine3(const float* g, const float* mask, const float* x, const float* A, const float* B, const float* C,
                  int64_t n, int c, float* out, void* stream);
int egonn_relu_backward(const float* grad_out, const float* out, int64_t n, int c, float* grad_in, void* stream);
int egonn_act_backward(int act, const float* grad_out, const float* out, int64_t n, int c, float* grad_in, void* stream);
int egonn_l2_normalize(const float* x, const float* grad_out, int64_t n, int c, float* out, void* stream);
int egonn_eca_gate(const float* mean, const float* conv_weight, int kernel_size, int batch_size, int channels, float* gate,
                   void* stream);
int egonn_eca_gate_backward(const float* grad_gate, const float* gate, const float* mean, const float* conv_weight,
                            int kernel_size, int batch_size, int channels, float* grad_mean, float* grad_weight,
                            void* stream);
int egonn_se_gate(const float* mean, const float* w1, const float* b1, const float* w2, const float* b2, int batch_size,
                  int channels, int hidden, float* gate, float* hidden_out, void* stream);
int egonn_se_gate_backward(const float* grad_gate, const float* gate, const float* hidden_act, const float* mean,
                           const float* w1, const float* w2, int batch_size, int channels, int hidden, float* grad_mean,
                           float* grad_w1, float* grad_b1, float* grad_w2, float* grad_b2, void* stream);
int egonn_gate_residual(egonn_ctx* ctx, int level, const float* x, const float* gate, const float* residual, int channels,
                        int relu, float* out, void* stream);
int egonn_gate_residual_backward(egonn_ctx* ctx, int level, const float* grad_out, const float* out, const float* gate,
                                 int channels, float* grad_x, float* grad_residual, void* stream);
int egonn_segment_sums(egonn_ctx* ctx, int level, int mode, const float* a, const float* b, const float* x2,
                       const float* p, int channels, float* out, float* scratch, int64_t scratch_floats, void* stream);
int egonn_segment_broadcast(egonn_ctx* ctx, int level, const float* v, int channels, int mean, float* out, void* stream);
int egonn_gem_backward(egonn_ctx* ctx, int level, const float* x, const float* coef, const float* p, int channels,
                       float* grad_x, void* stream);

int64_t egonn_filter_points_scratch_ints(int64_t n);
int egonn_filter_points(const float* raw, int64_t n, int floats_per_point, const int64_t* scan_offsets, int batch_size,
                        int remove_zero_points, int remove_ground_plane, float ground_plane_level, float* out_points,
                        int64_t* out_scan_offsets, int32_t* scratch, int64_t scratch_ints, void* stream);

int egonn_knn(const float* query, int64_t n_query, const float* database, int64_t n_database, int dim, int k,
              int32_t* out_index, float* out_distance, float* scratch, int64_t scratch_floats, void* stream);
int egonn_recall_counts(const int32_t* nn_index, const float* query_positions, const float* map_positions,
                        int64_t n_query, int k, int position_dim, const float* radius, int n_radius,
                        int32_t* out_true_positives, void* stream);

enum { EGONN_REG_STATUS_CLIPPED = 1,
       EGONN_REG_STATUS_FEW_CORR = 2,
       EGONN_REG_STATUS_NO_MODEL = 4,
       EGONN_REG_STATUS_BAD_INDEX = 8 };
int64_t egonn_registration_scratch_bytes(int n_pairs, int n_max, int n_hypotheses);
int64_t egonn_match_mutual_scratch_bytes(int n_pairs, int n_max);
int egonn_match_mutual(const float* feat1, const float* feat2, const int32_t* n1, const int32_t* n2, int n_pairs, int n_max,
                       int dim, int32_t* corr, int32_t* n_corr, void* scratch, int64_t scratch_bytes, void* stream);
int egonn_ransac_pairs(const float* kp1, const float* kp2, const int32_t* n1, const int32_t* n2, const int32_t* corr,
                       const int32_t* n_corr, const int32_t* pair_id, int n_pairs, int n_max, int n_hypotheses, uint64_t seed,
                       double dist_th, void* scratch, int64_t scratch_bytes, int32_t* hyp_count, double* hyp_err2, void* stream);
int egonn_registration_finish(const float* kp1, const float* kp2, const int32_t* n1, const int32_t* n2, const int32_t* corr,
                              const int32_t* n_corr, const int32_t* pair_id, int n_pairs, int n_max, int n_hypotheses,
                              uint64_t seed, double dist_th, const void* scratch, int64_t scratch_bytes, const double* T_gt,
                              double repeat_th, double* T, int32_t* inliers, double* fitness, double* inlier_rmse,
                              int32_t* corr_set, int32_t* best_t, double* rte, double* rre, int32_t* success,
                              double* repeatability, int32_t* status, void* stream);

enum { EGONN_ICP_STATUS_FEW_CORR = 1,
       EGONN_ICP_STATUS_MAX_ITER = 2,
       EGONN_ICP_STATUS_EMPTY = 4,
       EGONN_ICP_STATUS_RANGE = 8 };
int64_t egonn_voxel_downsample_scratch_bytes(int64_t n, int n_clouds);
int egonn_voxel_downsample(const float* points, int64_t n, const int64_t* offsets, int n_clouds, double voxel_size,
                           const float* crop, double* out_points, int64_t* out_offsets, int32_t* out_counts, int32_t* status,
                           void* scratch, int64_t scratch_bytes, void* stream);
int64_t egonn_icp_scratch_bytes(int64_t n_src, int64_t n_tgt, int n_pairs);
int egonn_icp_pairs(const double* src, int64_t n_src, const int64_t* src_offsets, const double* tgt, int64_t n_tgt,
                    const int64_t* tgt_offsets, int n_pairs, const double* T_init, double max_dist, int max_iteration,
                    double eps_fitness, double eps_rmse, double* T, double* fitness, double* inlier_rmse, int32_t* iterations,
                    int32_t* status, double* T_trace, double* eval_trace, int32_t* corr, void* scratch, int64_t scratch_bytes,
                    void* stream);

enum { EGONN_ICP_STATUS_SINGULAR = 16 };
enum { EGONN_NORMALS_STATUS_FEW_POINTS = 1,
       EGONN_NORMALS_STATUS_RANGE = 2 };
int64_t egonn_estimate_normals_scratch_bytes(int64_t n, int n_clouds);
int egonn_estimate_normals(const double* points, int64_t n, const int64_t* offsets, int n_clouds, int knn, double* normals,
                           int32_t* status, int32_t* neighbors, double* eigenvalues, void* scratch, int64_t scratch_bytes,
                           void* stream);
int64_t egonn_icp_plane_scratch_bytes(int64_t n_src, int64_t n_tgt, int n_pairs);
int egonn_icp_plane_pairs(const double* src, int64_t n_src, const int64_t* src_offsets, const double* tgt, int64_t n_tgt,
                          const int64_t* tgt_offsets, const double* tgt_normals, int n_pairs, const double* T_init, double max_dist,
                          int max_iteration, double eps_fitness, double eps_rmse, double* T, double* fitness, double* inlier_rmse,
                          int32_t* iterations, int32_t* status, double* T_trace, double* eval_trace, int32_t* corr, void* scratch,
                          int64_t scratch_bytes, void* stream);

enum { EGONN_AUG_JITTER = 1, EGONN_AUG_REMOVE_POINTS = 2, EGONN_AUG_TRANSLATE = 4, EGONN_AUG_ROTATE = 8, EGONN_AUG_BLOCK = 16,
       EGONN_AUG_SET_ROTATE = 32, EGONN_AUG_FLIP = 64, EGONN_AUG_RIGID = 128, EGONN_AUG_JITTER_CLIP = 256, EGONN_AUG_ALL = 511 };
enum { EGONN_AUG_STATUS_BAD_ID = 1 };
typedef struct egonn_augment_params {
  uint64_t seed;
  uint32_t draw;
  uint32_t set_id;
  uint32_t stages;
  uint32_t reserved;
  double sigma, clip;
  double r_min, r_max;
// ... 64 lines not shown
```

Baseline: 22850.

## Compute sigma first, then decode descriptors and keypoints only for selected rows

New measurement: 22800. Within noise of the previous version (-0.2%).

```diff
diff --git a/egonn_amd/_lib.py b/egonn_amd/_lib.py
--- a/egonn_amd/_lib.py
+++ b/egonn_amd/_lib.py
@@ -79,6 +79,8 @@
     ("egonn_minkfpn_forward", C.c_int, [_P, _P, C.c_int, _P, _P, _P]),
     ("egonn_topdown_step", C.c_int, [_P, C.c_int, _P, _P, _P, _P, C.c_int, C.c_int, _P, _P]),
     ("egonn_select_keypoints", C.c_int, [_P, _P, _P, _P, C.c_int, _P, _P, _P, _P, _P]),
+    ("egonn_extract", C.c_int, [_P, _P, _P, C.c_int, C.POINTER(C.c_float), C.c_int, _P, C.c_int, _P, _P, _P, _P, _P]),
+    ("egonn_debug_set_keypoint_first", C.c_int, [_P, C.c_int]),
     ("egonn_topk_rows", C.c_int, [_P, _P, C.c_int, C.c_int, _P, _P, _P]),
     ("egonn_triplet_loss_scratch_floats", C.c_int64, [C.c_int]),
     ("egonn_triplet_loss", C.c_int, [_P, C.c_int, C.c_int, _P, _P, C.c_float, _P, _P, _P, _P, _P]),
@@ -810,6 +812,9 @@
         self._call(self.lib.egonn_forward_level_features, self.h, level, out.data_ptr(), channels)
         return out
 
+    def set_keypoint_first(self, mode: int):
+        check(self.lib.egonn_debug_set_keypoint_first(self.h, int(mode)))
+
     def select_keypoints(self, sigma: torch.Tensor, keypoints: torch.Tensor, descriptors: torch.Tensor, n_k: int):
         B = self.batch_size
         dev = self.device
diff --git a/egonn_amd/csrc/common.h b/egonn_amd/csrc/common.h
--- a/egonn_amd/csrc/common.h
+++ b/egonn_amd/csrc/common.h
@@ -203,6 +203,7 @@
   bool no_gated_k2s2;
   bool no_fused_ghead;
   bool no_split_heads;
+  bool keypoint_first;
   bool no_tail_split;
   bool no_task_order;
   bool flat_sort, sort_pairs;
diff --git a/egonn_amd/csrc/coords.hip b/egonn_amd/csrc/coords.hip
--- a/egonn_amd/csrc/coords.hip
+++ b/egonn_amd/csrc/coords.hip
@@ -22,6 +22,7 @@
     return Switches{.debug_sync = ds && ds[0] == '1', .no_presplit = on("EGONN_NO_PRESPLIT"), .no_fused_down = on("EGONN_NO_FUSED_DOWN"),
                     .no_fused_lateral = on("EGONN_NO_FUSED_LATERAL"), .no_gated_k2s2 = on("EGONN_NO_GATED_K2S2"),
                     .no_fused_ghead = on("EGONN_NO_FUSED_GHEAD"), .no_split_heads = on("EGONN_NO_SPLIT_HEADS"),
+                    .keypoint_first = on("EGONN_KEYPOINT_FIRST"),
                     .no_tail_split = on("EGONN_NO_TAIL_SPLIT"), .no_task_order = on("EGONN_NO_TASK_ORDER"),
                     .flat_sort = on("EGONN_FLAT_SORT"), .sort_pairs = on("EGONN_SORT_PAIRS"), .no_search67 = on("EGONN_NO_SEARCH67"),
                     .no_dense_stream = on("EGONN_NO_DENSE_STREAM"),
diff --git a/egonn_amd/csrc/heads.hip b/egonn_amd/csrc/heads.hip
--- a/egonn_amd/csrc/heads.hip
+++ b/egonn_amd/csrc/heads.hip
@@ -94,6 +94,7 @@
 template <int CIN, int NT>
 __device__ static inline void stage_frags_t(const float* __restrict__ W, int cout, f32x4* __restrict__ dst, int tid, int nthreads) {
   constexpr int T = CIN / 16;
+#pragma unroll 4
   for (int i = tid; i < NT * T * 64; i += nthreads) {
     const int lane = i & 63, ft = i >> 6;
     const int nt = ft / T, t = ft - nt * T;
@@ -294,26 +295,51 @@
   const void* pack;
   int32_t* flags;
 };
-__global__ __launch_bounds__(LH_WAVES * 64) void local_heads_split_kernel(const LocalHeadsSplitArgs q) {
+constexpr int LH_DESC = 1, LH_KP = 2, LH_SIGMA = 4, LH_ALL = LH_DESC | LH_KP | LH_SIGMA;
+template <int HEADS>
+struct LhsSpan {
+  static_assert(HEADS == LH_ALL || HEADS == LH_SIGMA || HEADS == (LH_DESC | LH_KP), "the heads of a kernel are one span of the pack");
+  static constexpr int first = (HEADS & LH_DESC) ? LHS_DW0 : LHS_SW0;
+  static constexpr int last = (HEADS & LH_SIGMA) ? LHS_FRAGS : LHS_SW0;
+  static constexpr int lds_f32x4 = (last - first) * 2 * 64;
+};
+struct LhsWinv { float w[6]; };
+template <int HEADS, int THREADS>
+__device__ static inline f32x4* lhs_stage(const LocalHeadsSplitArgs& q, f32x4* __restrict__ lds, int tid, LhsWinv* wi) {
+  constexpr int N = LhsSpan<HEADS>::lds_f32x4, U = 8;
+  const f32x4* src = reinterpret_cast<const f32x4*>(q.pack) + LhsSpan<HEADS>::first * 2 * 64;
+  int i = tid;
+  for (; i + (U - 1) * THREADS < N; i += U * THREADS) {
+    f32x4 v[U];
+#pragma unroll
+    for (int u = 0; u < U; ++u) v[u] = src[i + u * THREADS];
+#pragma unroll
+    for (int u = 0; u < U; ++u) lds[i + u * THREADS] = v[u];
+  }
+  {
+    f32x4 v[U];
+#pragma unroll
+    for (int u = 0; u < U; ++u)
+      if (i + u * THREADS < N) v[u] = src[i + u * THREADS];
+#pragma unroll
+    for (int u = 0; u < U; ++u)
+      if (i + u * THREADS < N) lds[i + u * THREADS] = v[u];
+  }
+  f32x4* const lat = lds + N;
+  if (q.a.lw) stage_frags_t<64, 4>(q.a.lw, 64, lat, tid, THREADS);
+  const float* winv = reinterpret_cast<const float*>(reinterpret_cast<const char*>(q.pack) + (size_t)LHS_FRAGS * 2048);
+#pragma unroll
+  for (int i = 0; i < 6; ++i) wi->w[i] = winv[i];
+  return lat;
+}
+template <int HEADS>
+__device__ static inline void lhs_tile(const LocalHeadsSplitArgs& q, const f32x4* __restrict__ frags, const f32x4* __restrict__ lat,
+                                       const LhsWinv& wi, int lane, int64_t row, bool ok, float* __restrict__ out_desc,
+                                       float* __restrict__ out_kp, float* __restrict__ out_sigma) {
   const LocalHeadsArgs& p = q.a;
-  extern __shared__ __attribute__((aligned(16))) f32x4 lh_frags[];
-  const int tid = threadIdx.x, lane = tid & 63, wave = tid >> 6;
-  const int l15 = lane & 15, g4 = lane >> 4;
+  constexpr int F0 = LhsSpan<HEADS>::first;
+  const int g4 = lane >> 4;
   {
-    const f32x4* src = reinterpret_cast<const f32x4*>(q.pack);
-    for (int i = tid; i < LHS_FRAGS * 2 * 64; i += LH_WAVES * 64) lh_frags[i] = src[i];
-  }
-  f32x4* const lat = lh_frags + LHS_FRAGS * 2 * 64;
-  if (p.lw) stage_frags_t<64, 4>(p.lw, 64, lat, tid, LH_WAVES * 64);
-  const float* winv = reinterpret_cast<const float*>(reinterpret_cast<const char*>(q.pack) + (size_t)LHS_FRAGS * 2048);
-  const float wi0 = winv[0], wi1 = winv[1], wi2 = winv[2], wi3 = winv[3], wi4 = winv[4], wi5 = winv[5];
-  __syncthreads();
-  int64_t n = p.n;
-  if (p.n_dev) n = min((int64_t)*p.n_dev, n);
-  const int64_t ntiles = (n + 15) >> 4;
-  for (int64_t tile = (int64_t)blockIdx.x * LH_WAVES + wave; tile < ntiles; tile += (int64_t)gridDim.x * LH_WAVES) {
-    const int64_t row = tile * 16 + l15;
-    const bool ok = row < n;
     f32x4 x[4];
     auto load4 = [&](const float* base, int t) -> f32x4 {
       if (!ok) return (f32x4){0.f, 0.f, 0.f, 0.f};
@@ -339,16 +365,16 @@
     for (int t = 0; t < 4; ++t)
 #pragma unroll
       for (int r = 0; r < 4; ++r) outside |= !(fabsf(x[t][r]) < 65520.f);
-    {
+    if constexpr ((HEADS & LH_DESC) != 0) {
       f32x4 h[6], o[8];
-      lhs_layer<64, 6>(lh_frags + LHS_DW0 * 2 * 64, x, lane, wi0, h);
+      lhs_layer<64, 6>(frags + (LHS_DW0 - F0) * 2 * 64, x, lane, wi.w[0], h);
 #pragma unroll
       for (int nt = 0; nt < 6; ++nt) {
         const f32x4 b = *reinterpret_cast<const f32x4*>(p.db0 + 16 * nt + 4 * g4);
 #pragma unroll
         for (int r = 0; r < 4; ++r) h[nt][r] = fmaxf(h[nt][r] + b[r], 0.f);
       }
-      lhs_layer<96, 8>(lh_frags + LHS_DW1 * 2 * 64, h, lane, wi1, o);
+      lhs_layer<96, 8>(frags + (LHS_DW1 - F0) * 2 * 64, h, lane, wi.w[1], o);
       float ss = 0.f;
 #pragma unroll
       for (int nt = 0; nt < 8; ++nt) {
@@ -366,85 +392,180 @@
       if (ok) {
 #pragma unroll
         for (int nt = 0; nt < 8; ++nt)
-          *reinterpret_cast<f32x4*>(p.out_desc + row * 128 + 16 * nt + 4 * g4) = o[nt] * inv;
-      }
-    }
-    {
+          *reinterpret_cast<f32x4*>(out_desc + 16 * nt + 4 * g4) = o[nt] * inv;
+      }
+    }
+    if constexpr ((HEADS & LH_KP) != 0) {
       f32x4 h[2], o[1];
-      lhs_layer<64, 2>(lh_frags + LHS_KW0 * 2 * 64, x, lane, wi2, h);
+      lhs_layer<64, 2>(frags + (LHS_KW0 - F0) * 2 * 64, x, lane, wi.w[2], h);
 #pragma unroll
       for (int nt = 0; nt < 2; ++nt) {
         const f32x4 b = *reinterpret_cast<const f32x4*>(p.kb0 + 16 * nt + 4 * g4);
 #pragma unroll
         for (int r = 0; r < 4; ++r) h[nt][r] = fmaxf(h[nt][r] + b[r], 0.f);
       }
-      lhs_layer<32, 1>(lh_frags + LHS_KW1 * 2 * 64, h, lane, wi3, o);
+      lhs_layer<32, 1>(frags + (LHS_KW1 - F0) * 2 * 64, h, lane, wi.w[3], o);
       if (ok && g4 == 0) {
         guard += (o[0][0] - o[0][0]) + (o[0][1] - o[0][1]) + (o[0][2] - o[0][2]);
         const float ox = p.ignore_offsets ? 0.f : tanhf(o[0][0] + p.kb1[0]);
         const float oy = p.ignore_offsets ? 0.f : tanhf(o[0][1] + p.kb1[1]);
         const float oz = p.ignore_offsets ? 0.f : tanhf(o[0][2] + p.kb1[2]);
-        keypoint_position(p.keys[row], p.level, p.cb, ox, oy, oz, p.mode, p.s0, p.s1, p.s2, p.out_kp + row * 3);
-      }
-    }
-    {
+        keypoint_position(p.keys[row], p.level, p.cb, ox, oy, oz, p.mode, p.s0, p.s1, p.s2, out_kp);
+      }
+    }
+    if constexpr ((HEADS & LH_SIGMA) != 0) {
       f32x4 h[2], o[1];
-      lhs_layer<64, 2>(lh_frags + LHS_SW0 * 2 * 64, x, lane, wi4, h);
+      lhs_layer<64, 2>(frags + (LHS_SW0 - F0) * 2 * 64, x, lane, wi.w[4], h);
 #pragma unroll
       for (int nt = 0; nt < 2; ++nt) {
         const f32x4 b = *reinterpret_cast<const f32x4*>(p.sb0 + 16 * nt + 4 * g4);
 #pragma unroll
         for (int r = 0; r < 4; ++r) h[nt][r] = fmaxf(h[nt][r] + b[r], 0.f);
       }
-      lhs_layer<32, 1>(lh_frags + LHS_SW1 * 2 * 64, h, lane, wi5, o);
+      lhs_layer<32, 1>(frags + (LHS_SW1 - F0) * 2 * 64, h, lane, wi.w[5], o);
       if (ok && g4 == 0) {
         guard += o[0][0] - o[0][0];
-        p.out_sigma[row] = apply_act(o[0][0] + p.sb1[0], ACT_SOFTPLUS);
+        *out_sigma = apply_act(o[0][0] + p.sb1[0], ACT_SOFTPLUS);
       }
     }
     if (ok && (outside || guard != 0.f) && q.flags) atomicOr(q.flags, 8);
   }
 }
-
-int local_heads_forward(const float* x, int64_t n, const int32_t* n_dev, const float* const* w ,
-                        const uint64_t* keys, int level, int cb, int mode, const float* step, int ignore_offsets,
-                        float* out_desc, float* out_kp, float* out_sigma, hipStream_t stream, const float* lateral_w,
-                        const float* lateral_res, int in_bf16, const void* split_pack, int32_t* flags) {
-  if (n == 0) return EGONN_OK;
-  EGONN_REQUIRE((lateral_w == nullptr) == (lateral_res == nullptr), EGONN_ERR_INVALID, "local heads: lateral kernel and residual go together");
+template <int HEADS, int WAVES>
+__device__ static inline void lhs_rows_kernel(const LocalHeadsSplitArgs& q) {
+  const LocalHeadsArgs& p = q.a;
+  extern __shared__ __attribute__((aligned(16))) f32x4 lh_frags[];
+  const int tid = threadIdx.x, lane = tid & 63, wave = tid >> 6;
+  LhsWinv wi;
+  const f32x4* lat = lhs_stage<HEADS, WAVES * 64>(q, lh_frags, tid, &wi);
+  __syncthreads();
+  int64_t n = p.n;
+  if (p.n_dev) n = min((int64_t)*p.n_dev, n);
+  const int64_t ntiles = (n + 15) >> 4;
+  for (int64_t tile = (int64_t)blockIdx.x * WAVES + wave; tile < ntiles; tile += (int64_t)gridDim.x * WAVES) {
+    const int64_t row = tile * 16 + (lane & 15);
+    lhs_tile<HEADS>(q, lh_frags, lat, wi, lane, row, row < n, (HEADS & LH_DESC) ? p.out_desc + row * 128 : nullptr,
+                    (HEADS & LH_KP) ? p.out_kp + row * 3 : nullptr, p.out_sigma + row);
+  }
+}
+__global__ __launch_bounds__(LH_WAVES * 64) void local_heads_split_kernel(const LocalHeadsSplitArgs q) {
+  lhs_rows_kernel<LH_ALL, LH_WAVES>(q);
+}
+constexpr int LSG_WAVES = 4, LDC_WAVES = 4;
+__global__ __launch_bounds__(LSG_WAVES * 64) void local_sigma_kernel(const LocalHeadsSplitArgs q) {
+  lhs_rows_kernel<LH_SIGMA, LSG_WAVES>(q);
+}
+__global__ __launch_bounds__(LDC_WAVES * 64) void local_decode_kernel(const LocalHeadsSplitArgs q, const int32_t* __restrict__ sel_rows,
+                                                                      int64_t slots, float* __restrict__ sel_desc,
+                                                                      float* __restrict__ sel_kp) {
+  const LocalHeadsArgs& p = q.a;
+  extern __shared__ __attribute__((aligned(16))) f32x4 lh_frags[];
+  const int tid = threadIdx.x, lane = tid & 63, wave = tid >> 6;
+  LhsWinv wi;
+  const f32x4* lat = lhs_stage<LH_DESC | LH_KP, LDC_WAVES * 64>(q, lh_frags, tid, &wi);
+  __syncthreads();
+  int64_t n = p.n;
+  if (p.n_dev) n = min((int64_t)*p.n_dev, n);
+  const int64_t ntiles = (slots + 15) >> 4;
+  for (int64_t tile = (int64_t)blockIdx.x * LDC_WAVES + wave; tile < ntiles; tile += (int64_t)gridDim.x * LDC_WAVES) {
+    const int64_t slot = tile * 16 + (lane & 15);
+    const bool live = slot < slots;
+    const int64_t row = live ? (int64_t)sel_rows[slot] : -1;
+    const bool ok = row >= 0 && row < n;
+    float* const od = sel_desc + slot * 128;
+    float* const ok3 = sel_kp + slot * 3;
+    lhs_tile<LH_DESC | LH_KP>(q, lh_frags, lat, wi, lane, row, ok, od, ok3, nullptr);
+    if (live && !ok) {
+      const int g4 = lane >> 4;
+#pragma unroll
+      for (int nt = 0; nt < 8; ++nt) *reinterpret_cast<f32x4*>(od + 16 * nt + 4 * g4) = (f32x4){0.f, 0.f, 0.f, 0.f};
+      if (g4 == 0) ok3[0] = ok3[1] = ok3[2] = 0.f;
+    }
+  }
+}
+
+namespace {
+int lh_args(const LocalHeadsIn& in, LocalHeadsArgs* a) {
+  EGONN_REQUIRE((in.lateral_w == nullptr) == (in.lateral_res == nullptr), EGONN_ERR_INVALID, "local heads: lateral kernel and residual go together");
+  EGONN_REQUIRE(!in.in_bf16 || in.lateral_w, EGONN_ERR_INVALID, "local heads: bf16 input rows only through the fused lateral");
+  const float* const* w = in.w;
+  a->x = in.x; a->n = in.n; a->n_dev = in.n_dev;
+  a->lw = in.lateral_w; a->lres = in.lateral_res;
+  a->in_bf16 = in.in_bf16 ? 1 : 0;
+  a->dw0 = w[0]; a->db0 = w[1]; a->dw1 = w[2]; a->db1 = w[3];
+  a->kw0 = w[4]; a->kb0 = w[5]; a->kw1 = w[6]; a->kb1 = w[7];
+  a->sw0 = w[8]; a->sb0 = w[9]; a->sw1 = w[10]; a->sb1 = w[11];
+  a->keys = in.keys; a->level = in.level; a->cb = in.cb; a->mode = in.mode; a->ignore_offsets = in.ignore_offsets;
+  a->s0 = in.step[0]; a->s1 = in.mode ? in.step[1] : in.step[0]; a->s2 = in.mode ? in.step[2] : in.step[0];
+  a->out_desc = a->out_kp = a->out_sigma = nullptr;
+  return EGONN_OK;
+}
+template <int HEADS>
+constexpr size_t lhs_lds_bytes() { return (size_t)(LhsSpan<HEADS>::lds_f32x4 + 16 * 64) * sizeof(f32x4); }
+}
+
+int local_heads_forward(const LocalHeadsIn& in, float* out_desc, float* out_kp, float* out_sigma, hipStream_t stream) {
+  if (in.n == 0) return EGONN_OK;
   LocalHeadsArgs a;
-  a.x = x; a.n = n; a.n_dev = n_dev;
-  a.lw = lateral_w; a.lres = lateral_res;
-  a.in_bf16 = in_bf16 ? 1 : 0;
-  EGONN_REQUIRE(!in_bf16 || lateral_w, EGONN_ERR_INVALID, "local heads: bf16 input rows only through the fused lateral");
-  a.dw0 = w[0]; a.db0 = w[1]; a.dw1 = w[2]; a.db1 = w[3];
-  a.kw0 = w[4]; a.kb0 = w[5]; a.kw1 = w[6]; a.kb1 = w[7];
-  a.sw0 = w[8]; a.sb0 = w[9]; a.sw1 = w[10]; a.sb1 = w[11];
-  a.keys = keys; a.level = level; a.cb = cb; a.mode = mode; a.ignore_offsets = ignore_offsets;
-  a.s0 = step[0]; a.s1 = mode ? step[1] : step[0]; a.s2 = mode ? step[2] : step[0];
+  EGONN_TRY(lh_args(in, &a));
   a.out_desc = out_desc; a.out_kp = out_kp; a.out_sigma = out_sigma;
-  const int64_t tiles = cdiv(n, 16);
-  const size_t lds = (size_t)(LH_FRAGS + (lateral_w ? 16 : 0)) * 64 * sizeof(f32x4);
+  const int64_t tiles = cdiv(in.n, 16);
+  const size_t lds = (size_t)(LH_FRAGS + (in.lateral_w ? 16 : 0)) * 64 * sizeof(f32x4);
   static AttrOnce attr_done;
   if (attr_done.need()) {
     HIP_CHECK(hipFuncSetAttribute(reinterpret_cast<const void*>(&local_heads_kernel), hipFuncAttributeMaxDynamicSharedMemorySize, 160 * 1024));
-    attr_done.mark(); 
+    attr_done.mark();
   }
   const unsigned grid = (unsigned)std::min<int64_t>(cdiv(tiles, LH_WAVES), 256);
-  if (split_pack) {
+  if (in.split_pack) {
     static AttrOnce attr2;
     if (attr2.need()) {
       HIP_CHECK(hipFuncSetAttribute(reinterpret_cast<const void*>(&local_heads_split_kernel), hipFuncAttributeMaxDynamicSharedMemorySize, 160 * 1024));
       attr2.mark();
     }
     LocalHeadsSplitArgs q;
-    q.a = a; q.pack = split_pack; q.flags = flags;
-    const size_t lds2 = (size_t)(LHS_FRAGS * 2 + (lateral_w ? 16 : 0)) * 64 * sizeof(f32x4);
+    q.a = a; q.pack = in.split_pack; q.flags = in.flags;
+    const size_t lds2 = (size_t)(LHS_FRAGS * 2 + (in.lateral_w ? 16 : 0)) * 64 * sizeof(f32x4);
     hipLaunchKernelGGL(local_heads_split_kernel, dim3(grid), dim3(LH_WAVES * 64), lds2, stream, q);
     HIP_CHECK(hipGetLastError());
     return EGONN_OK;
   }
   hipLaunchKernelGGL(local_heads_kernel, dim3(grid), dim3(LH_WAVES * 64), lds, stream, a);
+  HIP_CHECK(hipGetLastError());
+  return EGONN_OK;
+}
+
+bool local_heads_keypoint_first(const LocalHeadsIn& in) { return in.split_pack && in.lateral_w; }
+
+int local_sigma_forward(const LocalHeadsIn& in, float* out_sigma, hipStream_t stream) {
+  EGONN_REQUIRE(local_heads_keypoint_first(in) && out_sigma, EGONN_ERR_INVALID, "local sigma: needs the split pack, the fused lateral and an output");
+  if (in.n == 0) return EGONN_OK;
+  LocalHeadsSplitArgs q;
+  EGONN_TRY(lh_args(in, &q.a));
+  q.a.out_sigma = out_sigma;
+  q.pack = in.split_pack; q.flags = in.flags;
+  const unsigned grid = (unsigned)std::min<int64_t>(cdiv(cdiv(in.n, 16), LSG_WAVES), 4 * 256);
+  hipLaunchKernelGGL(local_sigma_kernel, dim3(grid), dim3(LSG_WAVES * 64), lhs_lds_bytes<LH_SIGMA>(), stream, q);
+  HIP_CHECK(hipGetLastError());
+  return EGONN_OK;
+}
+
+int local_decode_forward(const LocalHeadsIn& in, const int32_t* sel_rows, int64_t slots, float* sel_desc, float* sel_kp,
+                         hipStream_t stream) {
+  EGONN_REQUIRE(local_heads_keypoint_first(in) && sel_rows && sel_desc && sel_kp && in.keys && slots >= 0, EGONN_ERR_INVALID,
+                "local decode: needs the split pack, the fused lateral, the selected rows and both outputs");
+  if (slots == 0) return EGONN_OK;
+  LocalHeadsSplitArgs q;
+  EGONN_TRY(lh_args(in, &q.a));
+  q.pack = in.split_pack; q.flags = in.flags;
+  static AttrOnce attr_done;
+  if (attr_done.need()) {
+    HIP_CHECK(hipFuncSetAttribute(reinterpret_cast<const void*>(&local_decode_kernel), hipFuncAttributeMaxDynamicSharedMemorySize, 160 * 1024));
+    attr_done.mark();
+  }
+  const unsigned grid = (unsigned)std::min<int64_t>(cdiv(cdiv(slots, 16), LDC_WAVES), 256);
+  hipLaunchKernelGGL(local_decode_kernel, dim3(grid), dim3(LDC_WAVES * 64), lhs_lds_bytes<LH_DESC | LH_KP>(), stream, q, sel_rows, slots,
+                     sel_desc, sel_kp);
   HIP_CHECK(hipGetLastError());
   return EGONN_OK;
 }
diff --git a/egonn_amd/csrc/kernels.h b/egonn_amd/csrc/kernels.h
--- a/egonn_amd/csrc/kernels.h
+++ b/egonn_amd/csrc/kernels.h
@@ -138,10 +138,25 @@
 constexpr int LH_WAVES = 8;
 int keypoint_positions(const uint64_t* keys, int64_t n, int level, int cb, const float* offsets, int mode,
                        const float* step, int ignore_offsets, float* out, hipStream_t stream, const int32_t* n_dev = nullptr);
-int local_heads_forward(const float* x, int64_t n, const int32_t* n_dev, const float* const* w, const uint64_t* keys,
-                        int level, int cb, int mode, const float* step, int ignore_offsets, float* out_desc, float* out_kp,
-                        float* out_sigma, hipStream_t stream, const float* lateral_w = nullptr, const float* lateral_res = nullptr,
-                        int in_bf16 = 0, const void* split_pack = nullptr, int32_t* flags = nullptr);
+struct LocalHeadsIn {
+  const float* x = nullptr;
+  int64_t n = 0;
+  const int32_t* n_dev = nullptr;
+  const float* const* w = nullptr;
+  const uint64_t* keys = nullptr;
+  int level = 0, cb = 0, mode = 0;
+  const float* step = nullptr;
+  int ignore_offsets = 0;
+  const float *lateral_w = nullptr, *lateral_res = nullptr;
+  int in_bf16 = 0;
+  const void* split_pack = nullptr;
+  int32_t* flags = nullptr;
+};
+int local_heads_forward(const LocalHeadsIn& in, float* out_desc, float* out_kp, float* out_sigma, hipStream_t stream);
+bool local_heads_keypoint_first(const LocalHeadsIn& in);
+int local_sigma_forward(const LocalHeadsIn& in, float* out_sigma, hipStream_t stream);
+int local_decode_forward(const LocalHeadsIn& in, const int32_t* sel_rows, int64_t slots, float* sel_desc, float* sel_kp,
+                         hipStream_t stream);
 size_t local_heads_pack_bytes();
 int local_heads_pack(const float* const* w6_dev, void* out, hipStream_t stream);
 int select_topk(const float* sigma, const int32_t* boff_dev, int B, int k, const float* kp, const float* desc, int dc,
diff --git a/egonn_amd/csrc/model.h b/egonn_amd/csrc/model.h
--- a/egonn_amd/csrc/model.h
+++ b/egonn_amd/csrc/model.h
@@ -14,6 +14,7 @@
   int level_ch[EGONN_NUM_LEVELS] = {};
   int level_bf16 = 0;
   bool from_points = false;
+  int keypoint_first = -1;
 };
 
 #define REQUIRE_PLAN(c)                                                                               \
diff --git a/egonn_amd/csrc/model.hip b/egonn_amd/csrc/model.hip
--- a/egonn_amd/csrc/model.hip
+++ b/egonn_amd/csrc/model.hip
@@ -773,13 +773,17 @@
 
 }
 
-API int egonn_forward(egonn_ctx* c, egonn_model* m, const float* features, int quant_mode, const float* step, int flags,
-                      float* out_global, float* out_desc, float* out_kp, float* out_sigma, void* stream) {
-  REQUIRE_PLAN(c);
-  EGONN_REQUIRE(m && m->ready, EGONN_ERR_STATE, "model not finalized (call egonn_model_finalize)");
-  EGONN_REQUIRE(step, EGONN_ERR_INVALID, "forward: null argument");
-  HIP_CHECK(hipSetDevice(c->device));
-  hipStream_t st = (hipStream_t)stream;
+namespace {
+
+struct SelectOut {
+  int n_k;
+  float *kp, *desc;
+  int32_t *rows, *count;
+};
+
+int forward_graph(egonn_ctx* c, egonn_model* m, const float* features, int quant_mode, const float* step, int flags, float* out_global,
+                  float* out_desc, float* out_kp, float* out_sigma, const SelectOut* sel, hipStream_t st) {
+  HIP_CHECK(hipSetDevice(c->device));
   Plan& P = c->plan;
   const int B = P.batch;
   const int32_t* cnt = c->dev_counts;
@@ -787,8 +791,6 @@
   const size_t es = bf16 ? 2 : 4;
   const bool do_global = !(flags & EGONN_FLAG_DISABLE_GLOBAL);
   const bool do_local = !(flags & EGONN_FLAG_DISABLE_LOCAL);
-  EGONN_REQUIRE(!do_global || out_global, EGONN_ERR_INVALID, "forward: out_global is null");
-  EGONN_REQUIRE(!do_local || (out_desc && out_kp && out_sigma), EGONN_ERR_INVALID, "forward: local outputs are null");
   HIP_CHECK(hipMemsetAsync(c->dev_fp16_flag, 0, sizeof(int32_t), st));
 
   {
@@ -802,8 +804,23 @@
   need += (size_t)P.cap[5] * (192 + 256 + 128 * 2) * 4 + (size_t)P.cap[3] * (96 + 32 + 32 + 3 + 64 * 2) * 4;
   need += (size_t)B * SEG_CHUNKS * 256 * 4 * 10 + (size_t)P.cap[3] * 32 + (4u << 20);
   need += sconv_ksplit_scratch_floats(c) * 4 + 4096;
+  const void* lh_pack = (!switches().no_split_heads && sconv_split_arithmetic(c)) ? m->lh_pack : nullptr;
+  const bool fused_lateral = !switches().no_fused_lateral && LOCAL_CH == 64;
+  const bool want_first = c->keypoint_first < 0 ? switches().keypoint_first : c->keypoint_first == 1;
+  const bool kp_first = sel && do_local && lh_pack && fused_lateral && want_first;
+  if (sel) need += (size_t)P.cap[3] * (1 + (kp_first ? 0 : LOCAL_DIM + 3)) * 4 + 3 * 256;
   Arena* A;
   EGONN_TRY(claim_work(c, need, true, &A));
+  if (sel) {
+    WALLOC(float, sg, P.cap[3]);
+    out_sigma = sg;
+    if (!kp_first) {
+      WALLOC(float, ad, (size_t)P.cap[3] * LOCAL_DIM);
+      WALLOC(float, ak, (size_t)P.cap[3] * 3);
+      out_desc = ad;
+      out_kp = ak;
+    }
+  }
 
   const int64_t n0 = P.cap[0];
   const float* f0 = features;
@@ -834,21 +851,37 @@
                   EGONN_ERR_STATE, "local heads: unexpected layer sizes");
     const float* hw[12] = {m->ldec.w0, m->ldec.b0, m->ldec.w1, m->ldec.b1, m->kp.w0, m->kp.b0, m->kp.w1, m->kp.b1,
                            m->sg.w0, m->sg.b0, m->sg.w1, m->sg.b1};
-    const void* lh_pack = (!switches().no_split_heads && sconv_split_arithmetic(c)) ? m->lh_pack : nullptr;
-    if (!switches().no_fused_lateral && LOCAL_CH == 64) {
-      EGONN_TRY(local_heads_forward(reinterpret_cast<const float*>(x[3]), n3, cnt + 3, hw, P.lv[3].keys, 3, P.coord_bits, quant_mode,
-                                    step, (flags & EGONN_FLAG_IGNORE_KP_REGRESSOR) ? 1 : 0, out_desc, out_kp, out_sigma, st,
-                                    m->l1x1[3], reinterpret_cast<const float*>(u3), bf16, lh_pack, c->dev_fp16_flag));
-      return EGONN_OK;
+    LocalHeadsIn hin{.n = n3, .n_dev = cnt + 3, .w = hw, .keys = P.lv[3].keys, .level = 3, .cb = P.coord_bits, .mode = quant_mode,
+                     .step = step, .ignore_offsets = (flags & EGONN_FLAG_IGNORE_KP_REGRESSOR) ? 1 : 0, .split_pack = lh_pack,
+                     .flags = c->dev_fp16_flag};
+    if (fused_lateral) {
+      hin.x = reinterpret_cast<const float*>(x[3]);
+      hin.lateral_w = m->l1x1[3];
+      hin.lateral_res = reinterpret_cast<const float*>(u3);
+      hin.in_bf16 = bf16;
+    } else {
+      WALLOC(float, l3, n3 * LOCAL_CH);
+      EGONN_TRY(dense_forward({.in = x[3], .in_bf16 = bf16, .n = n3, .n_dev = cnt + 3, .cin = 64, .cout = LOCAL_CH, .W = m->l1x1[3],
+                               .wfrag = static_cast<const float*>(m->pk_l1x1[3]), .residual = u3, .res_bf16 = bf16, .out = l3},
+                              st));
+      hin.x = l3;
     }
-    WALLOC(float, l3, n3 * LOCAL_CH);
-    EGONN_TRY(dense_forward({.in = x[3], .in_bf16 = bf16, .n = n3, .n_dev = cnt + 3, .cin = 64, .cout = LOCAL_CH, .W = m->l1x1[3],
-                             .wfrag = static_cast<const float*>(m->pk_l1x1[3]), .residual = u3, .res_bf16 = bf16, .out = l3},
-                            st));
-    EGONN_TRY(local_heads_forward(l3, n3, cnt + 3, hw, P.lv[3].keys, 3, P.coord_bits, quant_mode, step,
-                                  (flags & EGONN_FLAG_IGNORE_KP_REGRESSOR) ? 1 : 0, out_desc, out_kp, out_sigma, st, nullptr, nullptr, 0,
-                                  lh_pack, c->dev_fp16_flag));
-    return EGONN_OK;
+    if (kp_first) {
+      {
+        ProfScope ps(c, st, "local_sigma_kernel/L3", PK_OTHER, 3, 1, 64, 1, (int)es);
+        EGONN_TRY(local_sigma_forward(hin, out_sigma, st));
+      }
+      EGONN_TRY(select_topk(out_sigma, P.lv[3].boff, B, sel->n_k, nullptr, nullptr, 0, sel->rows, sel->count, nullptr, nullptr, st));
+      ProfScope ps(c, st, "local_decode_kernel/L3", PK_OTHER, 3, 1, 64, LOCAL_DIM + 3, (int)es);
+      return local_decode_forward(hin, sel->rows, (int64_t)B * sel->n_k, sel->desc, sel->kp, st);
+    }
+    if (!sel) return local_heads_forward(hin, out_desc, out_kp, out_sigma, st);
+    {
+      ProfScope ps(c, st, lh_pack ? "local_heads_split_kernel/L3" : "local_heads_kernel/L3", PK_OTHER, 3, 1, 64, LOCAL_DIM + 4, (int)es);
+      EGONN_TRY(local_heads_forward(hin, out_desc, out_kp, out_sigma, st));
+    }
+    return select_topk(out_sigma, P.lv[3].boff, B, sel->n_k, out_kp, out_desc, LOCAL_DIM, sel->rows, sel->count, sel->kp, sel->desc,
+                       st);
   };
   const float *gated_t2 = nullptr, *gated_res = nullptr, *gated_gate = nullptr;
   for (int i = 1; i <= 7; ++i) {
@@ -966,6 +999,39 @@
   return EGONN_OK;
 }
 
+}
+
+API int egonn_forward(egonn_ctx* c, egonn_model* m, const float* features, int quant_mode, const float* step, int flags,
+                      float* out_global, float* out_desc, float* out_kp, float* out_sigma, void* stream) {
+  REQUIRE_PLAN(c);
+  EGONN_REQUIRE(m && m->ready, EGONN_ERR_STATE, "model not finalized (call egonn_model_finalize)");
+  EGONN_REQUIRE(step, EGONN_ERR_INVALID, "forward: null argument");
+  EGONN_REQUIRE((flags & EGONN_FLAG_DISABLE_GLOBAL) || out_global, EGONN_ERR_INVALID, "forward: out_global is null");
+  EGONN_REQUIRE((flags & EGONN_FLAG_DISABLE_LOCAL) || (out_desc && out_kp && out_sigma), EGONN_ERR_INVALID,
+                "forward: local outputs are null");
+  return forward_graph(c, m, features, quant_mode, step, flags, out_global, out_desc, out_kp, out_sigma, nullptr, (hipStream_t)stream);
+}
+
+API int egonn_extract(egonn_ctx* c, egonn_model* m, const float* features, int quant_mode, const float* step, int flags,
+                      float* out_global, int n_k, float* sel_kp, float* sel_desc, int32_t* sel_rows, int32_t* sel_count,
+                      void* stream) {
+  REQUIRE_PLAN(c);
+  EGONN_REQUIRE(m && m->ready, EGONN_ERR_STATE, "model not finalized (call egonn_model_finalize)");
+  EGONN_REQUIRE(step, EGONN_ERR_INVALID, "extract: null argument");
+  EGONN_REQUIRE(!(flags & EGONN_FLAG_DISABLE_LOCAL), EGONN_ERR_INVALID, "extract: the local head selects the keypoints");
+  EGONN_REQUIRE((flags & EGONN_FLAG_DISABLE_GLOBAL) || out_global, EGONN_ERR_INVALID, "extract: out_global is null");
+  EGONN_REQUIRE(sel_kp && sel_desc && sel_rows && sel_count, EGONN_ERR_INVALID, "extract: selected outputs are null");
+  EGONN_REQUIRE(n_k >= 1 && n_k <= 8192, EGONN_ERR_INVALID, "extract: n_k=%d outside [1, 8192]", n_k);
+  const SelectOut sel{.n_k = n_k, .kp = sel_kp, .desc = sel_desc, .rows = sel_rows, .count = sel_count};
+  return forward_graph(c, m, features, quant_mode, step, flags, out_global, nullptr, nullptr, nullptr, &sel, (hipStream_t)stream);
+}
+
+API int egonn_debug_set_keypoint_first(egonn_ctx* c, int mode) {
+  EGONN_REQUIRE(c && mode >= -1 && mode <= 1, EGONN_ERR_INVALID, "set_keypoint_first: mode %d outside [-1, 1]", mode);
+  c->keypoint_first = mode;
+  return EGONN_OK;
+}
+
 API int egonn_forward_level_features(egonn_ctx* c, int level, float* out, int channels, void* stream) {
   REQUIRE_PLAN(c);
   EGONN_REQUIRE(level >= 0 && level < EGONN_NUM_LEVELS && c->level_feat[level], EGONN_ERR_STATE,
diff --git a/egonn_amd/evaluator.py b/egonn_amd/evaluator.py
--- a/egonn_amd/evaluator.py
+++ b/egonn_amd/evaluator.py
@@ -8,6 +8,16 @@
 from . import _lib
 from .model import MinkGL
 from .minkloc import _MinkLocBase
+
+
+def _selected_outputs(model, dev, B, n_k, make):
+    return {
+        'global': make((B, model.global_descriptor_size), dtype=torch.float32, device=dev),
+        'keypoints': make((B, n_k, 3), dtype=torch.float32, device=dev),
+        'descriptors': make((B, n_k, model.local_descriptor_size), dtype=torch.float32, device=dev),
+        'rows': make((B, n_k), dtype=torch.int32, device=dev),
+        'count': make((B,), dtype=torch.int32, device=dev),
+    }
 
 
 class DescriptorExtractor:
@@ -67,11 +77,19 @@
         return out
 
     @torch.no_grad()
-    def extract_packed(self, points: torch.Tensor, offsets: List[int], model: MinkGL = None, slot: int = 0):
+    def extract_packed(self, points: torch.Tensor, offsets: List[int], model: MinkGL = None, slot: int = 0,
+                       all_rows: bool = True):
         model = model or self.model
         ctx = model.context(slot)
         q = self.quantizer
         ctx.voxelize(points, offsets, q.mode, q.step)
+        if not all_rows:
+            if self.ignore_keypoint_saliency:
+                raise ValueError("ignore_keypoint_saliency draws its keypoints from every row: all_rows=True")
+            model._sync_weights()
+            out = _selected_outputs(model, ctx.device, ctx.batch_size, self.n_k, torch.empty)
+            model._egonn_extract(ctx, self.n_k, out)
+            return out
         y = model._forward_on_plan(ctx, None)
         d, k, s = model._last_local
         if self.ignore_keypoint_saliency:
@@ -100,7 +118,7 @@
         for i, (points, offsets) in enumerate(batches):
             slot = i % n_streams
             with torch.cuda.stream(self._streams[slot]):
-                yield self.extract_packed(points, offsets, model, slot=slot)
+                yield self.extract_packed(points, offsets, model, slot=slot, all_rows=self.ignore_keypoint_saliency)
 
     def _ones(self, n, dev):
         buf = getattr(self, '_ones_buf', None)
@@ -136,24 +154,9 @@
         ctx, model, q = self.ctx, self.model, self.ex.quantizer
         ctx.voxelize_device(self.points, self.offsets, self.B, q.mode, q.step)
         if self.out is None:
-            dev = ctx.device
-            cap3 = ctx.level_capacity(3)
-            n_k = self.ex.n_k
-            self.out = {
-                'global': torch.zeros((self.B, model.global_descriptor_size), dtype=torch.float32, device=dev),
-                'all_descriptors': torch.zeros((cap3, model.local_descriptor_size), dtype=torch.float32, device=dev),
-                'all_keypoints': torch.zeros((cap3, 3), dtype=torch.float32, device=dev),
-                'all_sigma': torch.zeros((cap3, 1), dtype=torch.float32, device=dev),
-                'keypoints': torch.zeros((self.B, n_k, 3), dtype=torch.float32, device=dev),
-                'descriptors': torch.zeros((self.B, n_k, model.local_descriptor_size), dtype=torch.float32, device=dev),
-                'rows': torch.zeros((self.B, n_k), dtype=torch.int32, device=dev),
-                'count': torch.zeros((self.B,), dtype=torch.int32, device=dev),
-            }
-        o = self.out
-        model._forward_on_plan(ctx, None, outputs=(o['global'], o['all_descriptors'], o['all_keypoints'], o['all_sigma']))
-        _lib.call(ctx.device, ctx.lib.egonn_select_keypoints, ctx.h, o['all_sigma'].data_ptr(), o['all_keypoints'].data_ptr(),
-                  o['all_descriptors'].data_ptr(), self.ex.n_k, o['keypoints'].data_ptr(), o['descriptors'].data_ptr(),
-                  o['rows'].data_ptr(), o['count'].data_ptr())
+            self.out = _selected_outputs(model, ctx.device, self.B, self.ex.n_k, torch.zeros)
+        model._sync_weights()
+        model._egonn_extract(ctx, self.ex.n_k, self.out)
 
     def _load(self, points: torch.Tensor, offsets):
         n = int(offsets[-1])
diff --git a/egonn_amd/model.py b/egonn_amd/model.py
--- a/egonn_amd/model.py
+++ b/egonn_amd/model.py
@@ -408,6 +408,13 @@
         _lib.call(ctx.device, ctx.lib.egonn_forward, ctx.h, self._handle.h, _lib._ptr(feats), q.mode, step,
                   self._flags(disable_global_head, disable_local_head), *[_lib._ptr(t) for t in outputs])
 
+    def _egonn_extract(self, ctx, n_k, out):
+        q = self.quantizer
+        step = (_lib.C.c_float * 3)(*([float(s) for s in q.step] + [0.0, 0.0])[:3])
+        _lib.call(ctx.device, ctx.lib.egonn_extract, ctx.h, self._handle.h, None, q.mode, step, self._flags(False, False),
+                  out['global'].data_ptr(), n_k, out['keypoints'].data_ptr(), out['descriptors'].data_ptr(),
+                  out['rows'].data_ptr(), out['count'].data_ptr())
+
     def keypoint_coords(self) -> List[torch.Tensor]:
         ctx = self.context()
         lvl = min(LOCAL_LEVELS)
diff --git a/include/egonn_hip.h b/include/egonn_hip.h
--- a/include/egonn_hip.h
+++ b/include/egonn_hip.h
@@ -120,6 +120,12 @@
 int egonn_select_keypoints(egonn_ctx* ctx, const float* sigma, const float* keypoints, const float* descriptors,
                            int n_k, float* sel_keypoints, float* sel_descriptors, int32_t* sel_rows,
                            int32_t* sel_count, void* stream);
+
+int egonn_extract(egonn_ctx* ctx, egonn_model* model, const float* features, int quant_mode, const float* step, int flags,
+                  float* out_global, int n_k, float* sel_keypoints, float* sel_descriptors, int32_t* sel_rows,
+                  int32_t* sel_count, void* stream);
+
+int egonn_debug_set_keypoint_first(egonn_ctx* ctx, int mode);
 
 int egonn_topk_rows(const float* sigma, const int32_t* row_offsets, int batch_size, int n_k, int32_t* sel_rows,
                     int32_t* sel_count, void* stream);
```
